# bernardomig/torch_semantic_segmentation

Hardware: AMD Instinct MI355X
Metric: images/sec (train step) fastscnn 1024x2048 bs=8 (higher is better)
Workload: dtype bf16; 1 GPU; fastscnn train step (zero_grad+fwd+CE(ignore 255)+bwd+AdamW), 8 x 3 x 1024 x 2048 per GPU, 19 classes, random-init weights; global_batch=8, parallelism=dp1, hip_graph=True, syncbn=False

## Files before the change

### include/tss_hip.h

```cpp
#ifndef TSS_HIP_H
#define TSS_HIP_H

#ifdef __cplusplus
extern "C" {
#endif

#define TSS_OK 0
#define TSS_ERR_DTYPE (-1)
#define TSS_ERR_SHAPE (-2)
#define TSS_ERR_ALIGN (-3)
#define TSS_ERR_HIP (-4)

#define TSS_F32 0
#define TSS_BF16 1

typedef struct tss_bn_bwd_job {
  const double* bstats; double count; const float* invstd; const float* gamma; int training; int accumulate;
  float* dgamma; float* dbeta; float* ga; float* gb; float* gce; int C;
  int xchg_world; int xchg_rank; void* xchg_peers[8]; void* xchg_counters;
} tss_bn_bwd_job;

enum {
  TSS_K_PWCONV_FWD = 0, TSS_K_PWCONV_BWD_DATA, TSS_K_PWCONV_BWD_WEIGHT,
  TSS_K_CONV3X3_FWD, TSS_K_CONV3X3_BWD_DATA, TSS_K_CONV3X3_BWD_WEIGHT,
  TSS_K_STEM_FWD, TSS_K_STEM_BWD_WEIGHT,
  TSS_K_DWCONV_FWD, TSS_K_DWCONV_BWD_DATA, TSS_K_DWCONV_BWD_WEIGHT,
  TSS_K_BN_FINALIZE, TSS_K_BN_BWD_FINALIZE, TSS_K_JOIN_FWD, TSS_K_JOIN_BWD,
  TSS_K_DROPOUT, TSS_K_BIAS_GRAD, TSS_K_ADAMW,
  TSS_K_BILINEAR_FWD, TSS_K_BILINEAR_BWD, TSS_K_BILINEAR_BWD_COLS, TSS_K_BILINEAR_PLANAR_FWD,
  TSS_K_UPSAMPLE_HEAD_FWD, TSS_K_UPSAMPLE_HEAD_BWD_ROWS, TSS_K_UPSAMPLE_HEAD_BWD_COLS,
  TSS_K_POOL_FWD, TSS_K_POOL_BWD, TSS_K_COPY,
  TSS_K_CE_FWD, TSS_K_CE_BWD, TSS_K_ARGMAX, TSS_K_UPSAMPLE_CE_FWD, TSS_K_UPSAMPLE_CE_BWD,
  TSS_K_RESIZE_FLIP_PLANAR, TSS_K_MULTISCALE_ARGMAX,
  TSS_K_SGD, TSS_K_GRAD_NORM,
  TSS_K_WIDE_CE_FWD, TSS_K_WIDE_CE_BWD, TSS_K_WIDE_ARGMAX, TSS_K_WIDE_MULTISCALE_ARGMAX,
  TSS_K_COUNT
};

int tss_version(void);
int tss_memset_zero(void* p, long bytes, void* stream);
const char* tss_last_error(void);
const char* tss_arch(void);
#define TSS_OPT_DISABLE_FAST_PATHS 1
int tss_set_option(int key, int value);
int tss_get_option(int key);

int tss_prof_enable(int on);
int tss_prof_reset(void);
int tss_prof_collect(void);
int tss_prof_get(int kernel_id, long* launches, double* total_ms, double* alg_bytes, double* flops);
long tss_prof_records(int* kernel_ids, double* ms, double* alg_bytes, long max_records);
const char* tss_prof_name(int kernel_id);
const char* tss_prof_symbol(int kernel_id);

int tss_pwconv_fwd(const void* x, long ldx, const float* in_mean, const float* in_scale, const float* in_bias, int in_relu,
                   const float* w, const void* w_bf16, const float* bias, void* y, long ldy, double* stats,
                   long P, int K, int N, int dtype, void* stream);
int tss_pwconv_fwd_joined(const void* x, long ldx, const float* in_mean, const float* in_scale, const float* in_bias, int in_relu,
                          const float* w, const void* w_bf16, const float* bias,
                          const float* out_mean, const float* out_scale, const float* out_beta,
                          const void* residual, long ldr, int out_relu, void* y, long ldy,
                          long P, int K, int N, int dtype, void* stream);
int tss_bneck_eval_supported(int Cin, int Cmid, int Cout, int stride, int residual, int dtype);
int tss_bneck_eval_fwd(const void* x, long ldx, const float* w1, const void* w1_bf16, const float* mean1, const float* scale1,
                       const float* beta1, const float* wdw, const float* mean2, const float* scale2, const float* beta2,
                       const float* w3, const void* w3_bf16, const float* mean3, const float* scale3, const float* beta3,
                       int residual, void* y, long ldy, int B, int H, int W, int Cin, int Cmid, int Cout, int stride, int dtype,
                       void* stream);
long tss_bn_xchg_bytes(void);
int tss_bn_xchg_counters(void);
int tss_ipc_alloc(long bytes, void** ptr_out, void* handle_out);
int tss_ipc_open(const void* handle, void** ptr_out);
int tss_ipc_close(void* ptr);
int tss_ipc_free(void* ptr);
int tss_bn_xchg_error(const void* mailbox, long* out);
int tss_bn_finalize_xchg(const double* sums, double count, const void* const* peers, int rank, int world, void* counters,
                         const float* gamma, float eps, float momentum, float* running_mean, float* running_var,
                         long long* num_batches_tracked, float* mean_out, float* invstd_out, float* scale, int C, void* stream);
int tss_bn_bwd_finalize_xchg(const double* bstats, double count, const void* const* peers, int rank, int world, void* counters,
                             const float* invstd, const float* gamma, int accumulate, float* dgamma, float* dbeta,
                             float* ga, float* gb, float* gce, int C, void* stream);
int tss_pwconv_bwd_data(const void* e, long lde, const void* yraw, long ldyr,
                        const float* ga, const float* gb, const float* gce, const float* gmu, const float* w, const void* wT_bf16,
                        const void* xraw, long ldx, const float* in_mean, const float* in_scale, const float* in_bias, int in_relu,
                        void* e_in, long ldei, double* bstats, const float* wg_ws, float* wg_dw, long wg_P, int wg_K, int wg_N,
                        long P, int K, int N, int dtype, void* stream);
int tss_pwconv_bwd_weight(const void* e, long lde, const void* yraw, long ldyr,
                          const float* ga, const float* gb, const float* gce, const float* gmu,
                          const void* xraw, long ldx, const float* in_mean, const float* in_scale, const float* in_bias, int in_relu,
                          float* dw, float* ws, int defer_reduce, long P, int K, int N, int dtype, const tss_bn_bwd_job* fin,
                          void* stream);
long tss_pwconv_bwd_weight_ws(long P, int K, int N, int dtype);
int tss_pwconv_fwd_multi(const void* const* srcs, const long* lds, const float* const* means, const float* const* scales,
                         const float* const* biases, int nsrc, int in_relu, const float* w, const void* w_bf16,
                         const float* bias, void* y, long ldy, long P, int N, int dtype, void* stream);
int tss_pwconv_wg_reduce(const float* ws, float* dw, long P, int K, int N, void* stream);

int tss_permute_w3x3(const float* w, float* w_tnc, float* w_tcn, int N, int Cin, void* stream);
int tss_permute_w3x3_bf16(const float* w, void* w_tnc_bf16, void* w_tcn_bf16, int N, int Cin, void* stream);
int tss_conv3x3_fwd(const void* x, long ldx, const float* in_mean, const float* in_scale, const float* in_bias, int in_relu,
                    const float* w_tnc, const void* w_tnc_bf16, void* y, long ldy, double* stats,
                    int B, int Hin, int Win, int Cin, int N, int stride, int dil, int dtype, void* stream);
int tss_conv3x3_bwd_data(const void* e, long lde, const void* yraw, long ldyr,
                         const float* ga, const float* gb, const float* gce, const float* gmu, const float* w_tcn,
                         const void* w_tcn_bf16,
                         const void* xraw, long ldx, const float* in_mean, const float* in_scale, const float* in_bias, int in_relu,
                         void* e_in, long ldei, double* bstats,
                         int B, int H, int W, int Cin, int N, int dil, int dtype, void* stream);
int tss_conv3x3_bwd_weight(const void* e, long lde, const void* yraw, long ldyr,
                           const float* ga, const float* gb, const float* gce, const float* gmu,
                           const void* xraw, long ldx, const float* in_mean, const float* in_scale, const float* in_bias, int in_relu,
                           float* dw, int B, int Hin, int Win, int Cin, int N, int stride, int dil,
                           int dtype, void* stream);
int tss_im2col3x3(const void* x, long ldx, const float* in_mean, const float* in_scale, const float* in_bias, int in_relu,
                  void* col, int B, int H, int W, int C, int dil, int dtype, void* stream);

int tss_permute_wtaps(const float* w , float* w_tnc, float* w_tcn, int N, int Cin, int T, void* stream);
int tss_conv1d3_fwd(const void* x, long ldx, const float* in_mean, const float* in_scale, const float* in_bias, int in_relu,
                    const float* w_tnc, const float* bias, void* y, long ldy, double* stats,
                    int B, int H, int W, int Cin, int N, int axis, int dil, int dtype, void* stream);
int tss_conv1d3_bwd_data(const void* e, long lde, const void* yraw, long ldyr,
                         const float* ga, const float* gb, const float* gce, const float* gmu, const float* w_tcn,
                         const void* xraw, long ldx, const float* in_mean, const float* in_scale, const float* in_bias, int in_relu,
                         void* e_in, long ldei, double* bstats,
                         int B, int H, int W, int Cin, int N, int axis, int dil, int dtype, void* stream);
int tss_conv1d3_bwd_weight(const void* e, long lde, const void* yraw, long ldyr,
                           const float* ga, const float* gb, const float* gce, const float* gmu,
                           const void* xraw, long ldx, const float* in_mean, const float* in_scale, const float* in_bias, int in_relu,
                           float* dw, int B, int H, int W, int Cin, int N, int axis, int dil, int dtype, void* stream);
int tss_conv1d3_lean_supported(int Cin, int N, int dtype);
int tss_conv1d3_fwd_w(const void* x, long ldx, const float* in_mean, const float* in_scale, const float* in_bias, int in_relu,
                      const float* w, const float* bias, void* y, long ldy, double* stats,
                      int B, int H, int W, int Cin, int N, int axis, int dil, int dtype, void* stream);
int tss_conv1d3_bwd_data_w(const void* e, long lde, const void* yraw, long ldyr,
                           const float* ga, const float* gb, const float* gce, const float* gmu, const float* w,
                           const void* xraw, long ldx, const float* in_mean, const float* in_scale, const float* in_bias, int in_relu,
                           void* e_in, long ldei, double* bstats,
                           int B, int H, int W, int Cin, int N, int axis, int dil, int dtype, void* stream);
int tss_conv1d3_bwd_weight_rows(long P, int Cin, int N, int dtype);
int tss_conv1d3_bwd_weight_sweep(const void* e, long lde, const void* yraw, long ldyr,
                                 const float* ga, const float* gb, const float* gce, const float* gmu,
                                 const void* xraw, long ldx, const float* in_mean, const float* in_scale, const float* in_bias,
                                 int in_relu, float* ws, int B, int H, int W, int Cin, int N, int axis, int dil, int dtype, void* stream);
int tss_convtap_bwd_weight_rows(long P, int Cin, int N, int T, int dtype);
int tss_convtap_bwd_weight_sweep(const void* e, long lde, const void* yraw, long ldyr,
                                 const float* ga, const float* gb, const float* gce, const float* gmu,
                                 const void* xraw, long ldx, const float* in_mean, const float* in_scale, const float* in_bias,
                                 int in_relu, float* ws, int B, int H, int W, int Cin, int N, int T, int axis, int dil, int dtype, void* stream);
int tss_sconv_bwd_weight_rows(int B, int Hin, int Win, int Cin, int N, int dtype);
int tss_sconv_bwd_weight_sweep(const void* e, long lde, const void* yraw, long ldyr,
                               const float* ga, const float* gb, const float* gce, const float* gmu,
                               const void* xraw, long ldx, const float* in_mean, const float* in_scale, const float* in_bias,
                               int in_relu, float* ws, int B, int Hin, int Win, int Cin, int N, int dtype, void* stream);
int tss_im2col1d3(const void* x, long ldx, const float* in_mean, const float* in_scale, const float* in_bias, int in_relu,
                  void* col, int B, int H, int W, int C, int axis, int dil, int dtype, void* stream);
int tss_convkxk_fwd(const void* x, long ldx, const float* in_mean, const float* in_scale, const float* in_bias, int in_relu,
                    const float* w_tnc, const float* bias, void* y, long ldy, double* stats,
                    int B, int Hin, int Win, int Cin, int N, int kh, int kw, int stride, int dil, int dtype, void* stream);
int tss_convkxk_bwd_data(const void* e, long lde, const void* yraw, long ldyr,
                         const float* ga, const float* gb, const float* gce, const float* gmu, const float* w_tcn,
                         const void* xraw, long ldx, const float* in_mean, const float* in_scale, const float* in_bias, int in_relu,
                         void* e_in, long ldei, double* bstats,
                         int B, int Hin, int Win, int Cin, int N, int kh, int kw, int stride, int dil, int dtype, void* stream);
int tss_convkxk_bwd_weight(const void* e, long lde, const void* yraw, long ldyr,
                           const float* ga, const float* gb, const float* gce, const float* gmu,
                           const void* xraw, long ldx, const float* in_mean, const float* in_scale, const float* in_bias, int in_relu,
                           float* dw, int B, int Hin, int Win, int Cin, int N, int kh, int kw, int stride, int dil,
                           int dtype, void* stream);

int tss_convkxk_transposed_fwd(const void* x, long ldx, const float* w_tcn, const float* bias, void* y, long ldy,
                               int B, int Hout, int Wout, int Cout, int Cin_t, int kh, int kw, int stride, int dtype, void* stream);

int tss_tensor_stats(const void* z, long ldz, long P, int C, double* stats, int dtype, void* stream);
int tss_bn_bwd_apply(const void* e, long lde, const void* z, long ldz, const float* ga, const float* gb, const float* gce,
                     const float* gmu, void* dz, long lddz, long P, int C, int dtype, void* stream);
int tss_pool_concat_fwd(const void* y1, long ld1, const float* bias, int N1, const void* x, int x_f32, long sxb, long sxc, long sxh,
                        long sxw, int Cin, void* z, long ldz, int B, int Hin, int Win, int dtype, void* stream);
int tss_pool_concat_bwd(const void* dz, long lddz, int N1, const void* x, int x_f32, long sxb, long sxc, long sxh, long sxw, int Cin,
                        void* dx, long lddx, int B, int Hin, int Win, int dtype, void* stream);
int tss_rows_slices(int B, long HW);
int tss_mul_addrows_fwd(const void* u, long ldu, const void* a, long lda, const void* r, long ldr, void* out, long ldo, int B, long HW,
                        int C, int dtype, void* stream);
int tss_mul_addrows_bwd(const void* g, long ldg, const void* u, long ldu, const void* a, long lda, void* du, long lddu, void* da,
                        long ldda, void* dr, long lddr, float* ws, int B, long HW, int C, int dtype, void* stream);
int tss_scale_rows(const void* x, long ldx, const float* m, void* out, long ldo, int B, long HW, int C, int dtype, void* stream);
int tss_cat2_add(const void* gl, long ldl, const void* gr, long ldr, const void* gs, long lds, void* out, long ldo, long P, int half,
                 int dtype, void* stream);
int tss_pad_channels(const void* g, long ldg, int C, void* out, long ldo, int CP, long P, int dtype, void* stream);
int tss_ssnbt_tail_fwd(const void* left, long ldl, const float* mean_l, const float* scale_l, const float* shift_l,
                       const void* right, long ldr, const float* mean_r, const float* scale_r, const float* shift_r,
                       const void* x, long ldx, const float* m, void* out, long ldo, int B, long HW, int C, int dtype, void* stream);
int tss_ssnbt_tail_bwd(const void* dout, long lddo, const void* out, long ldo,
                       const void* left, long ldl, const float* mean_l, const void* right, long ldr, const float* mean_r,
                       const float* m, void* e, long lde, void* gs, long ldgs, double* stats_l, double* stats_r,
                       int B, long HW, int C, int dtype, void* stream);

int tss_channel_shuffle(const void* x, long ldx, void* y, long ldy, long P, int C, int groups, int dtype, void* stream);

int tss_stem3x3_fwd(const void* x_nchw, int x_is_f32, const float* w, void* y, long ldy, double* stats,
                    int B, int Cin, int Hin, int Win, int N, int stride, int dtype, void* stream);
int tss_stem3x3_bwd_weight(const void* e, long lde, const void* yraw, long ldyr,
                           const float* ga, const float* gb, const float* gce, const float* gmu,
                           const void* x_nchw, int x_is_f32, float* dw,
                           float* ws ,
                           int B, int Cin, int Hin, int Win, int N, int stride, int dtype, void* stream);

int tss_dwconv3x3_fwd(const void* x, long ldx, const float* in_mean, const float* in_scale, const float* in_bias, int in_relu,
                      const float* w, void* y, long ldy, double* stats,
                      int B, int Hin, int Win, int C, int stride, int dil, int dtype, void* stream);
int tss_dwconv3x3_bwd_data(const void* e, long lde, const void* yraw, long ldyr,
                           const float* ga, const float* gb, const float* gce, const float* gmu, const float* w,
                           const void* xraw, long ldx, const float* in_mean, const float* in_scale, const float* in_bias, int in_relu,
                           void* e_in, long ldei, double* bstats, const float* wg_ws, float* wg_dw,
                           int B, int Hin, int Win, int C, int stride, int dil, int dtype, void* stream);
int tss_pwconv_bwd_data_radd_supported(long P, int K, int N, int dtype);
int tss_pwconv_bwd_data_joined(const void* e, long lde, const void* yraw, long ldyr,
                               const float* ga, const float* gb, const float* gce, const float* gmu, const float* w, const void* wT_bf16,
                               void* e_in, long ldei, const float* wg_ws, float* wg_dw, long wg_P, int wg_K, int wg_N,
                               const void* radd, long ldr, const void* join_out, long ldjo, const void* join_y, long ldjy,
                               const float* join_mean, double* join_bstats, long P, int K, int N, int dtype, void* stream);
int tss_pwconv_bwd_data_radd(const void* e, long lde, const void* yraw, long ldyr,
                             const float* ga, const float* gb, const float* gce, const float* gmu, const float* w, const void* wT_bf16,
                             void* e_in, long ldei, const float* wg_ws, float* wg_dw, long wg_P, int wg_K, int wg_N,
                             const void* radd, long ldr, long P, int K, int N, int dtype, void* stream);
int tss_pwconv_bwd_fused_preferred(long P, int Cin, int Cout, int dtype);
int tss_pwconv_bwd_fused_rows(long P, int Cin, int Cout);
int tss_pwconv_bwd_fused(const void* e, long lde, const void* yraw, long ldyr, const float* ga, const float* gb, const float* gce,
                         const float* gmu, const float* w, const void* wT_bf16, const void* x, long ldx, const float* in_mean,
                         const float* in_scale, const float* in_bias, int in_relu, int x_pending, void* e_in, long ldei,
                         double* bstats, float* ws, float* bias_ws, long P, int Cin, int Cout, int dtype, void* stream);
int tss_pwconv_bwd_sweep_preferred(long P, int Cin, int Cout, int x_pending, int dtype);
int tss_pwconv_bwd_sweep_rows(long P, int Cin, int Cout);
int tss_pwconv_bwd_sweep(const void* e, long lde, const void* yraw, long ldyr, const float* ga, const float* gb, const float* gce,
                         const float* gmu, const void* wT_bf16, const void* x, long ldx, const float* in_mean,
                         const float* in_scale, const float* in_bias, int in_relu, int x_pending, const void* radd, long ldr,
                         void* e_in, long ldei, double* bstats, float* ws, long P, int Cin, int Cout, int dtype, void* stream);
int tss_dwconv3x3_bwd_fused_supported(int C, int stride, int dil, int dtype);
int tss_dwconv3x3_bwd_fused_sweep(const void* e, long lde, const void* yraw, long ldyr,
                                  const float* ga, const float* gb, const float* gce, const float* gmu, const float* w,
                                  const void* x, long ldx, const float* in_mean, const float* in_scale, const float* in_bias, int in_relu,
                                  int x_pending, void* e_in, long ldei, double* bstats, float* ws,
                                  int B, int Hin, int Win, int C, int stride, int dil, int dtype, void* stream, int* rows_out);
int tss_dw_reduce_many(int njobs, const float* const* ws, float* const* dw, const int* n, const int* rows, void* stream);
int tss_dwconv3x3_bwd_fused_preferred(int C, int stride, int dil, int dtype);
int tss_dwconv3x3_bwd_fused(const void* e, long lde, const void* yraw, long ldyr,
                            const float* ga, const float* gb, const float* gce, const float* gmu, const float* w,
                            const void* x, long ldx, const float* in_mean, const float* in_scale, const float* in_bias, int in_relu,
                            int x_pending, void* e_in, long ldei, double* bstats, float* ws, float* dw,
                            int B, int Hin, int Win, int C, int stride, int dil, int dtype, void* stream);
int tss_dwconv3x3_bwd_weight(const void* e, long lde, const void* yraw, long ldyr,
                             const float* ga, const float* gb, const float* gce, const float* gmu,
                             const void* xraw, long ldx, const float* in_mean, const float* in_scale, const float* in_bias, int in_relu,
                             float* dw, float* ws , int defer_reduce,
                             int B, int Hin, int Win, int C, int stride, int dil, int dtype, void* stream);

int tss_updw_supported(int B, int Hs, int Ws, int Ho, int Wo, int C, int dil, int dtype);
int tss_updw_ws_rows(int B, int Hs, int Ws, int Ho, int Wo, int C, int dil, int dtype);
int tss_updw_fwd(const void* x, long ldx, int Hs, int Ws, const float* w, void* y, long ldy, double* stats,
                 int B, int Ho, int Wo, int C, int dil, int dtype, void* stream);
int tss_updw_bwd(const void* e, long lde, const void* yraw, long ldyr, const float* ga, const float* gb, const float* gce,
                 const float* gmu, const float* w, const void* x, long ldx, int Hs, int Ws, void* e_up, long ldeu, float* ws,
                 int B, int Ho, int Wo, int C, int dil, int dtype, void* stream, int* rows_out);

int tss_stat_slabs(void);

int tss_bn_finalize(const double* sums, double count, const float* gamma, float eps,
                    float momentum, float* running_mean, float* running_var, long long* num_batches_tracked,
                    float* mean_out, float* invstd_out, float* scale, int C, void* stream);
int tss_bn_eval_affine(const float* gamma, const float* running_mean, const float* running_var,
                       float eps, float* mean_out, float* invstd_out, float* scale, int C, void* stream);
int tss_bn_eval_affine_batched(const long long* table, int njobs, int max_channels, void* stream);
int tss_bn_bwd_finalize(const double* bstats, double count, const float* invstd,
                        const float* gamma, int training, int accumulate, float* dgamma, float* dbeta,
                        float* ga, float* gb, float* gce, int C, void* stream);

int tss_slab_reduce(const double* slabs, double count, double* out, int C, void* stream);
int tss_bn_finalize_sync(const double* gsums, const float* gamma, float eps, float momentum, float* running_mean,
                         float* running_var, long long* num_batches_tracked, float* mean_out, float* invstd_out,
                         float* scale, int C, void* stream);
int tss_bn_bwd_finalize_sync(const double* bstats, const double* gsums, const float* invstd, const float* gamma,
                             int accumulate, float* dgamma, float* dbeta, float* ga, float* gb, float* gce, int C,
                             void* stream);

int tss_join_fwd(const void* a, long lda, const float* ma, const float* sa, const float* ba,
                 const void* b, long ldb, const float* mb, const float* sb, const float* bb,
                 void* out, long ldo, int relu, float drop_p, const unsigned long long* seed_slot,
                 long P, int C, int dtype, void* stream);
int tss_join_bwd(const void* dout, long lddo, const void* out, long ldo, int relu,
                 const void* a_raw, long lda, const float* mean_a, double* stats_a,
                 const void* b_raw, long ldb, const float* mean_b, double* stats_b,
                 void* e, long lde, float dout_scale, long P, int C, int dtype, void* stream);

int tss_dropout_tick(unsigned long long* counter, unsigned long long* seed_slot, void* stream);
int tss_dropout(const void* x, long ldx, void* y, long ldy, long P, int C, float p,
                const unsigned long long* seed_slot, int dtype, void* stream);
int tss_bias_grad(const void* e, long lde, long P, int N, float* dbias, int dtype, void* stream);
int tss_dropout_mask(const unsigned long long* counter, void* mask, long P, int C, float p, void* stream);
int tss_pwconv_drop_supported(long P, int K, int N, int dtype);
int tss_pwconv_fwd_drop(const void* x, long ldx, const float* in_mean, const float* in_scale, const float* in_bias, int in_relu,
                        const float* w, const void* w_bf16, const float* bias, void* y, long ldy,
                        const void* mask, float drop_p, unsigned long long* counter,
                        long P, int K, int N, int dtype, void* stream);
int tss_pwconv_bwd_fused_drop_supported(long P, int Cin, int Cout, int dtype);
int tss_pwconv_bwd_fused_drop_rows(long P);
int tss_pwconv_bwd_fused_drop(const void* e, long lde, const void* yraw, long ldyr, const float* ga, const float* gb, const float* gce,
                              const float* gmu, const float* w, const void* x, long ldx, const float* in_mean,
                              const float* in_scale, const float* in_bias, int in_relu, int x_pending, const void* mask, float drop_p,
                              void* e_in, long ldei, double* bstats, float* ws, float* bias_ws, long P, int Cin, int Cout, int dtype,
                              void* stream);
int tss_cast_weights(const long long* table, int njobs, int blocks_per_job, float* zero, long zero_n, void* stream);
int tss_adamw_step(float* params, const float* grads, float* exp_avg, float* exp_avg_sq, long n,
                   const float* lr, float beta1, float beta2, float eps, float weight_decay,
                   float* state, float grad_scale, float lr_host, long step_host, void* stream);

#define TSS_OPT_MAX_GROUPS 8
#define TSS_OPT_NESTEROV 1
typedef struct tss_optgroup { long begin; long end; float lr; float weight_decay; float beta1; float beta2; float eps; int flags; } tss_optgroup;
int tss_adamw_step_groups(float* params, const float* grads, float* exp_avg, float* exp_avg_sq, long n,
                          const tss_optgroup* groups, int ngroups, const float* lr, float* state, const float* scale,
                          float grad_scale, long step_host, void* stream);
int tss_sgd_step_groups(float* params, const float* grads, float* momentum_buf, long n, const tss_optgroup* groups, int ngroups,
                        const float* lr, float* state, const float* scale, float grad_scale, long step_host, void* stream);
long tss_grad_sqnorm_workspace_bytes(long n);
int tss_grad_sqnorm(const float* grads, long n, double* workspace, float grad_scale, float max_norm, float* out, void* stream);

int tss_bilinear_nhwc_fwd(const void* x, long ldx, void* y, long ldy, int B, int Hin, int Win, int Hout, int Wout,
                          int C, int dtype, void* stream);
int tss_bilinear_nhwc_bwd(const void* dy, long lddy, void* dx, long lddx, float* tmp ,
                          int B, int Hin, int Win, int Hout, int Wout, int C, int dtype, void* stream);
int tss_bilinear_planar_fwd(const void* x, int x_dtype, void* y, int y_dtype, long planes, int Hin, int Win,
                            int Hout, int Wout, void* stream);
int tss_upsample_head_fwd(const void* low, long ldl, void* y, int B, int N, int h, int w, int H, int W,
                          int dtype, void* stream);
int tss_upsample_head_bwd(const void* dy, const float* gscale, float* tmp, void* dlow, long ldl,
                          int B, int N, int h, int w, int H, int W, int dtype, void* stream);
int tss_adaptive_pool_fwd(const void* x, long ldx, void* y, long ldy, int B, int H, int W, int C, int bins,
                          int dtype, void* stream);
int tss_adaptive_pool_bwd(const void* dy, long lddy, void* dx, long lddx, int B, int H, int W, int C, int bins,
                          int dtype, void* stream);
int tss_ppm_pool_slices(int B, int ncells);
int tss_ppm_pool_fwd(const void* x, long ldx, void* const* y, const long* ldy, const int* bins, int narms,
                     float* ws ,
                     int B, int H, int W, int C, int dtype, void* stream);
int tss_ppm_pool_bwd(const void* const* dy, const long* lddy, const int* bins, int narms, void* dx, long lddx,
                     const void* radd, long ldr, int B, int H, int W, int C, int dtype, void* stream);
int tss_ppm_concat_fwd(const void* x, long ldx, const void* const* raw, const long* ldr, const int* bins,
                       const float* const* mean, const float* const* scale, const float* const* beta, const int* relu,
                       int narms, void* out, long ldo, int B, int H, int W, int C, int ca, int dtype, void* stream);
int tss_ppm_concat_bwd(const void* dout, long lddo, const void* const* raw, const long* ldr, const int* bins,
                       const float* const* mean, const float* const* scale, const float* const* beta, const int* relu,
                       double* const* bstats, void* const* e, const long* lde, int narms,
                       int B, int H, int W, int C, int ca, int dtype, void* stream);
int tss_ppm_arms_supported(int narms, int C, int Ca, const int* P, int dtype);
int tss_ppm_arms_fwd(const void* const* x, const long* ldx, const float* const* w, const float* const* gamma, float* const* running_mean,
                     float* const* running_var, long long* const* num_batches_tracked, void* const* y, const long* ldy, float* const* vec,
                     const int* P, int narms, int C, int Ca, int training, float eps, float momentum, int dtype, void* stream);
int tss_ppm_arms_bwd(const void* const* e, const long* lde, const void* const* y, const long* ldy, const void* const* x, const long* ldx,
                     const float* const* w, const float* const* gamma, float* const* vec, float* const* dw, float* const* dgamma,
                     float* const* dbeta, int accumulate, void* const* e_in, const long* ldei, const int* P, int narms, int C, int Ca,
                     int training, int dtype, void* stream);
int tss_copy_nhwc(const void* x, long ldx, void* y, long ldy, long P, int C, int dtype, void* stream);

int tss_gate_slices(int B, long HW);
int tss_gate_fwd(const void* x, long ldx, const void* a, long lda, void* out, long ldo, int B, long HW, int C, float add_one,
                 int dtype, void* stream);
int tss_gate_bwd(const void* g, long ldg, const void* x, long ldx, const void* a, long lda, void* dx, long lddx, void* da, long ldda,
                 float* ws, int B, long HW, int C, float add_one, int dtype, void* stream);

int tss_cross_entropy_fwd(const void* logits, const long long* target, float* lse, double* acc,
                          float* loss, float* inv_count, long B, int C, long HW, int ignore_index,
                          int dtype, void* stream);
int tss_cross_entropy_bwd(const void* logits, const long long* target, const float* lse, const float* inv_count,
                          const float* grad_out, void* dlogits, long B, int C, long HW, int ignore_index,
                          int dtype, void* stream);
long tss_cross_entropy_ex_rows(long B, long HW);
int tss_cross_entropy_fwd_ex(const void* logits, const long long* target, const float* weight, float label_smoothing,
                             float* lse, double* rows, float* loss, float* inv_count, long B, int C, long HW, int ignore_index,
                             int dtype, void* stream);
int tss_cross_entropy_bwd_ex(const void* logits, const long long* target, const float* weight, float label_smoothing,
                             const float* lse, const float* inv_count, const float* grad_out, void* dlogits, long B, int C, long HW,
                             int ignore_index, int dtype, void* stream);
long tss_ohem_workspace_bytes(void);
int tss_ohem_select(const float* pixel_loss, void* workspace, float* loss, float* params, long n, float thresh_loss, long n_top,
                    void* stream);
int tss_ohem_fwd(const void* logits, const long long* target, float* lse, float* pixel_loss, void* workspace,
                 float* loss, float* params, long B, int C, long HW, int ignore_index, float thresh_loss,
                 long n_top, int dtype, void* stream);
int tss_ohem_bwd(const void* logits, const long long* target, const float* lse, const float* pixel_loss,
                 const float* params, const float* grad_out, void* dlogits, long B, int C, long HW, int ignore_index,
                 int dtype, void* stream);
long tss_lovasz_workspace_bytes(long n_pixels, int C, int chunk_classes);
int tss_lovasz_fwd(const void* logits, const long long* target, void* workspace, float* loss, float* n_present,
                   long B, int C, long HW, int ignore_index, int has_ignore, int variant, int chunk_classes, int dtype,
                   void* stream);
int tss_lovasz_bwd(const void* logits, const long long* target, const void* workspace, const float* n_present,
                   const float* grad_out, void* dlogits, long B, int C, long HW, int chunk_classes, int dtype, void* stream);
long tss_focal_workspace_bytes(long B, long HW, int max_blocks);
int tss_focal_fwd(const void* logits, const long long* target, float* lse, float* pixel_coef, void* workspace, float* loss,
                  float* scale, long B, int C, long HW, int ignore_index, int has_ignore, float alpha, float gamma, int variant,
                  int max_blocks, int dtype, void* stream);
int tss_focal_bwd(const void* logits, const long long* target, const float* lse, const float* pixel_coef, const float* scale,
                  const float* grad_out, void* dlogits, long B, int C, long HW, int max_blocks, int dtype, void* stream);
long tss_dice_workspace_bytes(long B, int C, long HW, int max_blocks);
int tss_dice_fwd(const void* logits, const long long* target, float* lse, void* workspace, float* loss, long B, int C, long HW,
                 int ignore_index, int has_ignore, float smooth, int max_blocks, int dtype, void* stream);
int tss_dice_bwd(const void* logits, const long long* target, const float* lse, const void* workspace, const float* grad_out,
                 void* dlogits, long B, int C, long HW, int ignore_index, int has_ignore, int max_blocks, int dtype, void* stream);
// ... 91 lines not shown
```

### torch_semantic_segmentation_amd/_native.py

```python
import ctypes
import os

import torch

_HERE = os.path.dirname(os.path.abspath(__file__))
LIB_PATH = os.environ.get('TSS_HIP_LIB') or os.path.join(_HERE, 'libtss_hip.so')

TSS_F32, TSS_BF16 = 0, 1
ERRORS = {-1: 'TSS_ERR_DTYPE (unsupported dtype)', -2: 'TSS_ERR_SHAPE (unsupported shape or pitch)',
          -3: 'TSS_ERR_ALIGN (pointer not 16-byte aligned)', -4: 'TSS_ERR_HIP (HIP launch error)'}

_P, _L, _I, _F, _D = ctypes.c_void_p, ctypes.c_long, ctypes.c_int, ctypes.c_float, ctypes.c_double

HEADER_PATH = os.path.join(os.path.dirname(_HERE), 'include', 'tss_hip.h')


def parse_header(path=HEADER_PATH):
    import re
    text = open(path).read()
    text = re.sub(r'/\*.*?\*/', ' ', text, flags=re.S)
    scalars = {'int': _I, 'long': _L, 'float': _F, 'double': _D}
    decls = {}
    for m in re.finditer(r'\b(int|long|const\s+char\s*\*)\s*(tss_\w+)\s*\(([^)]*)\)\s*;', text):
        ret, name, params = m.group(1), m.group(2), m.group(3).strip()
        types = []
        if params and params != 'void':
            for prm in params.split(','):
                prm = prm.strip()
                if '*' in prm:
                    types.append(_P)
                else:
                    words = prm.split()[:-1]
                    types.append(scalars[' '.join(w for w in words if w != 'const')])
        decls[name] = (scalars.get(ret, ctypes.c_char_p), types)
    return decls


_lib = None


def lib():
    global _lib
    if _lib is None:
        if not os.path.exists(LIB_PATH):
            raise RuntimeError(
                'libtss_hip.so is not built (%s). Run `python -m torch_semantic_segmentation_amd.build`; '
                'this package has no non-HIP fallback.' % LIB_PATH)
        handle = ctypes.CDLL(LIB_PATH)
        for name, (restype, argtypes) in parse_header().items():
            fn = getattr(handle, name)
            fn.argtypes = argtypes
            fn.restype = restype
        _lib = handle
    return _lib


def call(name, *args):
    rc = getattr(lib(), name)(*args)
    if rc != 0:
        detail = lib().tss_last_error().decode() if rc == -4 else ''
        raise RuntimeError('%s failed: %s %s' % (name, ERRORS.get(rc, rc), detail))


def fast_paths_disabled():
    return lib().tss_get_option(1) == 1


def ptr(t):
    return None if t is None else t.data_ptr()


def stream():
    return torch.cuda.current_stream().cuda_stream


_slabs = None


def stat_slabs():
    global _slabs
    if _slabs is None:
        _slabs = lib().tss_stat_slabs()
    return _slabs


def dtype_code(dtype):
    if dtype == torch.float32:
        return TSS_F32
    if dtype == torch.bfloat16:
        return TSS_BF16
    raise TypeError('the HIP path computes in float32 or bfloat16 activations, got %s' % dtype)



K_COUNT = 41


def prof_enable(on=True):
    call('tss_prof_enable', 1 if on else 0)


def prof_reset():
    call('tss_prof_reset')


def prof_records(limit=100000):
    h = lib()
    ids = (ctypes.c_int * limit)()
    ms = (ctypes.c_double * limit)()
    by = (ctypes.c_double * limit)()
    n = min(h.tss_prof_records(ids, ms, by, limit), limit)
    return [(h.tss_prof_name(ids[i]).decode(), ms[i], by[i]) for i in range(n)]


def prof_table():
    call('tss_prof_collect')
    out = {}
    h = lib()
    for k in range(K_COUNT):
        n, ms, by, fl = ctypes.c_long(), ctypes.c_double(), ctypes.c_double(), ctypes.c_double()
        h.tss_prof_get(k, ctypes.byref(n), ctypes.byref(ms), ctypes.byref(by), ctypes.byref(fl))
        if n.value:
            out[h.tss_prof_name(k).decode()] = dict(symbol=h.tss_prof_symbol(k).decode(), launches=n.value,
                                                    ms=ms.value, bytes=by.value, flops=fl.value)
    return out
```

### torch_semantic_segmentation_amd/build.py

```python
import os
import subprocess
import sys
from concurrent.futures import ThreadPoolExecutor

HERE = os.path.dirname(os.path.abspath(__file__))
CSRC = os.path.join(HERE, 'csrc')
INCLUDE = os.path.join(os.path.dirname(HERE), 'include')
LIB = os.path.join(HERE, 'libtss_hip.so')
SOURCES = ['convgemm.hip', 'pwfast.hip', 'pwbwd.hip', 'pwsweep.hip', 'bneck.hip', 'conv3x3.hip', 'fc1d.hip', 'fcg.hip', 'sconv.hip', 'atrous.hip', 'wstat.hip', 'stem.hip', 'wgrad.hip', 'dwconv.hip', 'dwroll.hip', 'updw.hip', 'pointwise.hip', 'optim.hip', 'xchg.hip', 'resample.hip', 'ppm.hip', 'loss.hip', 'ohem.hip', 'lovasz.hip', 'softloss.hip', 'distill.hip', 'labelhist.hip', 'hostio.hip', 'augment.hip', 'msflip.hip', 'widehead.hip', 'softhead.hip', 'gate.hip', 'zoo.hip', 'ssnbt.hip', 'prof.cpp']
HIPCC = os.environ.get('HIPCC', '/opt/rocm/bin/hipcc')
FLAGS = ['--offload-arch=gfx950', '-O3', '-fPIC', '-std=c++17', '-Wall', '-Wno-unused-function',
         '-I' + INCLUDE, '-I' + CSRC]


def _deps_mtime():
    files = [os.path.join(CSRC, f) for f in os.listdir(CSRC) if f.endswith('.h')]
    files.append(os.path.join(INCLUDE, 'tss_hip.h'))
    return max(os.path.getmtime(f) for f in files)


def _compile(src, force):
    path = os.path.join(CSRC, src)
    timing = os.environ.get('TSS_TIMING') == '1'
    obj = os.path.join(CSRC, os.path.splitext(src)[0] + ('.timing.o' if timing else '.o'))
    if (not force and os.path.exists(obj)
            and os.path.getmtime(obj) >= max(os.path.getmtime(path), _deps_mtime())):
        return obj, False
    extra = ['-DTSS_TIMING'] if timing else []
    cmd = [HIPCC] + FLAGS + extra + (['-x', 'hip'] if src.endswith('.cpp') else []) + ['-c', path, '-o', obj]
    res = subprocess.run(cmd, capture_output=True, text=True)
    if res.returncode != 0:
        raise RuntimeError('hipcc failed for %s:\n%s\n%s' % (src, res.stdout, res.stderr))
    if res.stderr.strip():
        sys.stderr.write(res.stderr)
    return obj, True


def build(force=False, verbose=True):
    with ThreadPoolExecutor(max_workers=4) as pool:
        results = list(pool.map(lambda s: _compile(s, force), SOURCES))
    objs = [o for o, _ in results]
    variant = 'timing' if os.environ.get('TSS_TIMING') == '1' else 'release'
    stamp = os.path.join(CSRC, '.variant')
    same = os.path.exists(stamp) and open(stamp).read().strip() == variant
    if any(changed for _, changed in results) or not os.path.exists(LIB) or not same:
        cmd = [HIPCC, '--offload-arch=gfx950', '-shared', '-fPIC', '-o', LIB] + objs
        res = subprocess.run(cmd, capture_output=True, text=True)
        if res.returncode != 0:
            raise RuntimeError('link failed:\n%s\n%s' % (res.stdout, res.stderr))
        open(stamp, 'w').write(variant)
        if verbose:
            print('built', LIB, '(%s)' % variant)
    elif verbose:
        print('up to date', LIB)
    return LIB


if __name__ == '__main__':
    build(force='--force' in sys.argv)
```

### torch_semantic_segmentation_amd/csrc/dwroll.hip

```cpp
#include "dwroll.h"

#include <cstdlib>

#include "common.h"

namespace {

constexpr int NT = 256;
constexpr int ENT = NT + 16;

struct RollArgs {
  const bf16_t* x; long ldx; const float* xm; const float* xs; const float* xb; int x_relu;
  const float* w; bf16_t* y; long ldy; double* stats;
  int B, Hin, Win, C, CV, Hout, Wout;
  int CVS, PXL, nsl, nstrips, RS, nseg, rows_used;
  int dseg, dstrip, db;
  long units;
};

struct Cursor { int it, b, strip, seg, x0, o0; };

__device__ __forceinline__ void advance(Cursor& c, const RollArgs& g, int n_iter) {
  if (++c.it == n_iter) {
    c.it = 0;
    c.seg += g.dseg;
    int carry = c.seg >= g.nseg ? 1 : 0;
    c.seg -= carry * g.nseg;
    c.strip += g.dstrip + carry;
    carry = c.strip >= g.nstrips ? 1 : 0;
    c.strip -= carry * g.nstrips;
    c.b += g.db + carry;
    c.x0 = c.strip * g.PXL;
    c.o0 = c.seg * g.RS;
  }
}

__device__ __forceinline__ int clampi(int v, int lo, int hi) { return v < lo ? lo : (v > hi ? hi : v); }

typedef unsigned int u32x4 __attribute__((ext_vector_type(4)));
__device__ __forceinline__ void request(u32x4& dst, const bf16_t* uniform_base, int elem_offset) {
  asm volatile("global_load_dwordx4 %0, %1, %2" : "=v"(dst) : "v"(elem_offset * 2), "s"(uniform_base));
}
template <int N> __device__ __forceinline__ void arrived(u32x4& a, u32x4& b) {
  asm volatile("s_waitcnt vmcnt(%2)" : "+v"(a), "+v"(b) : "n"(N));
}
template <int N> __device__ __forceinline__ void arrived(u32x4& a, u32x4& b, u32x4& c, u32x4& d, u32x4& e, u32x4& f) {
  asm volatile("s_waitcnt vmcnt(%6)" : "+v"(a), "+v"(b), "+v"(c), "+v"(d), "+v"(e), "+v"(f) : "n"(N));
}

__device__ __forceinline__ void park(float4* lo4, float4* hi4, int e, const u32x4& raw, bool valid, const float sc[8],
                                     const float sh[8], float relu_lo) {
  float v[8];
  V8<bf16_t>::unpack(make_uint4(raw[0], raw[1], raw[2], raw[3]), v);
  const float lo = valid ? relu_lo : 0.f, hi = valid ? TSS_INF : 0.f;
#pragma unroll
  for (int j = 0; j < 8; ++j) v[j] = clamp3(v[j] * sc[j] + sh[j], lo, hi);
  lo4[e] = make_float4(v[0], v[1], v[2], v[3]);
  hi4[e] = make_float4(v[4], v[5], v[6], v[7]);
}
__device__ __forceinline__ void fetch(const float4* lo4, const float4* hi4, int e, float v[8]) {
  const float4 a = lo4[e], b = hi4[e];
  v[0] = a.x; v[1] = a.y; v[2] = a.z; v[3] = a.w; v[4] = b.x; v[5] = b.y; v[6] = b.z; v[7] = b.w;
}

template <int NC>
__device__ __forceinline__ void flush_slab(const float (&s1)[NC], const float (&s2)[NC], double* stats, int C, int CVS, int PXL,
                                           int sl, int brow, int rows_used, int p, int cg, bool lane_on, float* red) {
  const int tid = threadIdx.x;
  const int cw = CVS * NC;
  __syncthreads();
  if (p < PXL) {
#pragma unroll
    for (int j = 0; j < NC; ++j) {
      red[(p * 2 + 0) * cw + cg * NC + j] = lane_on ? s1[j] : 0.f;
      red[(p * 2 + 1) * cw + cg * NC + j] = lane_on ? s2[j] : 0.f;
    }
  }
  __syncthreads();
  const int ncol = 2 * cw, share = NT / ncol;
  float part = 0.f;
  const int col = tid % ncol, sub = tid / ncol;
  if (sub < share) {
#pragma unroll 8
    for (int q = sub; q < PXL; q += share) part += red[(q * 2 + col / cw) * cw + col % cw];
  }
  float* part_s = red + NT * 16;
  if (sub < share) part_s[sub * ncol + col] = part;
  __syncthreads();
  if (tid < ncol) {
    const int which = tid / cw, c = tid - which * cw;
    const int ch = sl * 64 + c;
    if (ch < C) {
      double a = 0.0;
      for (int q = 0; q < share; ++q) a += (double)part_s[q * ncol + tid];
      stats[(long)brow * 2 * C + which * C + ch] = a;
      for (int r = brow + rows_used; r < TSS_STAT_SLABS; r += rows_used) stats[(long)r * 2 * C + which * C + ch] = 0.0;
    }
  }
}

template <int S> struct RollCfg;
#ifndef TSS_ROLL_PF1
#define TSS_ROLL_PF1 6
#endif
#ifndef TSS_ROLL_PF2
#define TSS_ROLL_PF2 2
#endif
#ifndef TSS_ROLL_BPF1
#define TSS_ROLL_BPF1 4
#endif
#ifndef TSS_ROLL_BPF2
#define TSS_ROLL_BPF2 2
#endif
template <> struct RollCfg<1> { static constexpr int PF = TSS_ROLL_PF1, NRAW = 2, ROWS = 1, ARRS = 1; };
template <> struct RollCfg<2> { static constexpr int PF = TSS_ROLL_PF2, NRAW = 6, ROWS = 2, ARRS = 2; };

template <int S>
__global__ __launch_bounds__(NT, 2) void dw_fwd_roll_kernel(const RollArgs g) {
  typedef RollCfg<S> K;
  constexpr int PF = K::PF;
  extern __shared__ __align__(16) unsigned char dyn_smem[];
  typedef float4 (*Ring)[K::ROWS][K::ARRS][2][ENT];
  Ring ring = reinterpret_cast<Ring>(dyn_smem);
  const int tid = threadIdx.x;
  const int p = tid / g.CVS, cg = tid - p * g.CVS;
  const int sl = (int)blockIdx.x % g.nsl, brow = (int)blockIdx.x / g.nsl;
  const int cv = sl * 8 + cg;
  const bool lane_on = p < g.PXL && cv < g.CV;
  const int c0 = lane_on ? cv * 8 : 0;
  const bool halo_l = lane_on && p == 0, halo_r = lane_on && p == g.PXL - 1;
  const int ldx = (int)g.ldx;

  const int n_iter = (S == 1) ? g.RS + 2 : g.RS + 1;
  Cursor ci, cc;
  ci.it = 0;
  ci.seg = brow % g.nseg;
  ci.strip = (brow / g.nseg) % g.nstrips;
  ci.b = brow / (g.nseg * g.nstrips);
  ci.x0 = ci.strip * g.PXL;
  ci.o0 = ci.seg * g.RS;
  cc = ci;

  u32x4 raw[PF][K::NRAW];
  const int halo_dx = halo_l ? -1 : (halo_r ? g.PXL : p);
  auto issue = [&](const Cursor& c, u32x4 (&r)[K::NRAW]) {
    const int b = c.b < g.B ? c.b : g.B - 1;
    if (S == 1) {
      const int iy = clampi(c.o0 - 1 + c.it, 0, g.Hin - 1);
      const bf16_t* row = g.x + ((long)b * g.Hin + iy) * g.Win * g.ldx;
      request(r[0], row, clampi(c.x0 + p, 0, g.Win - 1) * ldx + c0);
      request(r[1], row, clampi(c.x0 + halo_dx, 0, g.Win - 1) * ldx + c0);
    } else {
#pragma unroll
      for (int ry = 0; ry < 2; ++ry) {
        const int iy = clampi(2 * (c.o0 + c.it) - 1 + ry, 0, g.Hin - 1);
        const bf16_t* row = g.x + ((long)b * g.Hin + iy) * g.Win * g.ldx;
        const int ix = 2 * (c.x0 + p);
        request(r[3 * ry + 0], row, clampi(ix, 0, g.Win - 1) * ldx + c0);
        request(r[3 * ry + 1], row, clampi(ix + 1, 0, g.Win - 1) * ldx + c0);
        request(r[3 * ry + 2], row, clampi(halo_l ? 2 * c.x0 - 1 : ix, 0, g.Win - 1) * ldx + c0);
      }
    }
  };
#pragma unroll
  for (int k = 0; k < PF; ++k) {
    issue(ci, raw[k]);
    advance(ci, g, n_iter);
  }

  float sc[8], sh[8];
  {
    float mu[8];
    const bool has = g.xs != nullptr, has_b = has && g.xb != nullptr, has_m = has && g.xm != nullptr;
    const float* safe = g.w;
#pragma unroll
    for (int h = 0; h < 2; ++h) {
      float a[4], b[4], m[4];
      V4<float>::load(has ? g.xs + c0 + 4 * h : safe, a);
      V4<float>::load(has_b ? g.xb + c0 + 4 * h : safe, b);
      V4<float>::load(has_m ? g.xm + c0 + 4 * h : safe, m);
#pragma unroll
      for (int j = 0; j < 4; ++j) {
        sc[4 * h + j] = has ? a[j] : 1.f;
        sh[4 * h + j] = has_b ? b[j] : 0.f;
        mu[4 * h + j] = has_m ? m[j] : 0.f;
      }
    }
#pragma unroll
    for (int j = 0; j < 8; ++j) sh[j] = __builtin_fmaf(-mu[j], sc[j], sh[j]);
  }
  float wr[9][8];
  {
    float wf[72];
#pragma unroll
    for (int q = 0; q < 18; ++q) V4<float>::load(g.w + (long)c0 * 9 + 4 * q, wf + 4 * q);
#pragma unroll
    for (int j = 0; j < 8; ++j)
#pragma unroll
      for (int t = 0; t < 9; ++t) wr[t][j] = wf[j * 9 + t];
  }
  const float relu_lo = g.x_relu ? 0.f : -TSS_INF;
  float s1[8], s2[8];
#pragma unroll
  for (int j = 0; j < 8; ++j) { s1[j] = 0.f; s2[j] = 0.f; }

  auto write = [&](const Cursor& c, const u32x4 (&r)[K::NRAW], int slot) {
    if (S == 1) {
      const int iy = c.o0 - 1 + c.it;
      const bool vy = iy >= 0 && iy < g.Hin;
      float4* lo4 = ring[slot][0][0][0];
      float4* hi4 = ring[slot][0][0][1];
      if (p < g.PXL) park(lo4, hi4, tid + g.CVS, r[0], vy && c.x0 + p < g.Win, sc, sh, relu_lo);
      if (halo_l) park(lo4, hi4, tid, r[1], vy && c.x0 - 1 >= 0, sc, sh, relu_lo);
      if (halo_r) park(lo4, hi4, tid + 2 * g.CVS, r[1], vy && c.x0 + g.PXL < g.Win, sc, sh, relu_lo);
    } else {
#pragma unroll
      for (int ry = 0; ry < 2; ++ry) {
        const int iy = 2 * (c.o0 + c.it) - 1 + ry;
        const bool vy = iy >= 0 && iy < g.Hin;
        const int ix = 2 * (c.x0 + p);
        if (p < g.PXL) {
          park(ring[slot][ry][1][0], ring[slot][ry][1][1], tid, r[3 * ry + 0], vy && ix < g.Win, sc, sh, relu_lo);
          park(ring[slot][ry][0][0], ring[slot][ry][0][1], tid + g.CVS, r[3 * ry + 1], vy && ix + 1 < g.Win, sc, sh, relu_lo);
        }
        if (halo_l) park(ring[slot][ry][0][0], ring[slot][ry][0][1], tid, r[3 * ry + 2], vy && 2 * c.x0 - 1 >= 0, sc, sh, relu_lo);
      }
    }
  };

  float accA[8], accB[8];
#pragma unroll
  for (int j = 0; j < 8; ++j) { accA[j] = 0.f; accB[j] = 0.f; }

  auto emit = [&](const Cursor& c, int orow, float (&acc)[8]) {
    if (lane_on && orow < g.Hout && c.x0 + p < g.Wout) {
#pragma unroll
      for (int j = 0; j < 8; ++j) {
        acc[j] = V8<bf16_t>::round(acc[j]);
        s1[j] += acc[j];
        s2[j] += acc[j] * acc[j];
      }
      V8<bf16_t>::store(g.y + ((long)c.b * g.Hout + orow) * g.Wout * g.ldy + ((c.x0 + p) * (int)g.ldy + c0), acc);
    }
  };
  auto compute = [&](const Cursor& c, int slot) {
    if (!lane_on) return;
    if (S == 1) {
      float accC[8];
      if (c.it == 0) {
#pragma unroll
        for (int j = 0; j < 8; ++j) { accA[j] = 0.f; accB[j] = 0.f; }
      }
#pragma unroll
      for (int kx = 0; kx < 3; ++kx) {
        float a[8];
        fetch(ring[slot][0][0][0], ring[slot][0][0][1], tid + kx * g.CVS, a);
#pragma unroll
        for (int j = 0; j < 8; ++j) {
          accA[j] += a[j] * wr[6 + kx][j];
          accB[j] += a[j] * wr[3 + kx][j];
          accC[j] = kx == 0 ? a[j] * wr[0][j] : accC[j] + a[j] * wr[kx][j];
        }
      }
      if (c.it >= 2) emit(c, c.o0 + c.it - 2, accA);
#pragma unroll
      for (int j = 0; j < 8; ++j) { accA[j] = accB[j]; accB[j] = accC[j]; }
    } else {
      if (c.it == 0) {
#pragma unroll
        for (int j = 0; j < 8; ++j) accA[j] = 0.f;
      }
#pragma unroll
      for (int kx = 0; kx < 3; ++kx) {
        float a[8];
        fetch(ring[slot][0][kx & 1][0], ring[slot][0][kx & 1][1], tid + (kx >> 1) * g.CVS, a);
#pragma unroll
        for (int j = 0; j < 8; ++j) {
          accA[j] += a[j] * wr[6 + kx][j];
          accB[j] = kx == 0 ? a[j] * wr[0][j] : accB[j] + a[j] * wr[kx][j];
        }
      }
      if (c.it >= 1) emit(c, c.o0 + c.it - 1, accA);
#pragma unroll
      for (int kx = 0; kx < 3; ++kx) {
        float a[8];
        fetch(ring[slot][1][kx & 1][0], ring[slot][1][kx & 1][1], tid + (kx >> 1) * g.CVS, a);
#pragma unroll
        for (int j = 0; j < 8; ++j) accB[j] += a[j] * wr[3 + kx][j];
      }
#pragma unroll
      for (int j = 0; j < 8; ++j) accA[j] = accB[j];
    }
  };

  int slot = 0;
  while (cc.b < g.B) {
#pragma unroll
    for (int k = 0; k < PF; ++k) {
      if (cc.b >= g.B) break;
      if (S == 1) arrived<K::NRAW * (PF - 1)>(raw[k][0], raw[k][1]);
      else arrived<K::NRAW * (PF - 1)>(raw[k][0], raw[k][1], raw[k][2], raw[k][3 % K::NRAW], raw[k][4 % K::NRAW], raw[k][5 % K::NRAW]);
      write(cc, raw[k], slot);
      asm volatile("" ::: "memory");
      issue(ci, raw[k]);
      advance(ci, g, n_iter);
      __syncthreads();
      compute(cc, slot);
      advance(cc, g, n_iter);
      slot ^= 1;
    }
  }
#pragma unroll
  for (int k = 0; k < PF; ++k) {
    if (S == 1) arrived<0>(raw[k][0], raw[k][1]);
    else arrived<0>(raw[k][0], raw[k][1], raw[k][2], raw[k][3 % K::NRAW], raw[k][4 % K::NRAW], raw[k][5 % K::NRAW]);
  }

  if (g.stats) flush_slab<8>(s1, s2, g.stats, g.C, g.CVS, g.PXL, sl, brow, g.rows_used, p, cg, lane_on, reinterpret_cast<float*>(dyn_smem));
}

void plan(RollArgs& g, int S) {
  g.CV = g.C / 8;
  g.nsl = (g.CV + 7) / 8;
  g.CVS = g.CV < 8 ? g.CV : 8;
  g.PXL = NT / g.CVS;
  g.nstrips = (g.Wout + g.PXL - 1) / g.PXL;
  const int cap = TSS_STAT_SLABS / g.nsl > 0 ? TSS_STAT_SLABS / g.nsl : 1;
  const int halo = S == 1 ? 2 : 1;
  long best_cost = -1;
  for (int nseg = 1; nseg <= g.Hout; ++nseg) {
    const int RS = (g.Hout + nseg - 1) / nseg;
    if (RS < 4 && nseg > 1) break;
    const int segs = (g.Hout + RS - 1) / RS;
    const long units = (long)g.B * g.nstrips * segs;
    const long k = (units + cap - 1) / cap;
    const long cost = k * (RS + halo) + 6;
    if (best_cost < 0 || cost < best_cost) {
      best_cost = cost;
      g.RS = RS; g.nseg = segs; g.units = units;
      g.rows_used = (int)((units + k - 1) / k);
    }
  }
  g.dseg = g.rows_used % g.nseg;
  g.dstrip = (g.rows_used / g.nseg) % g.nstrips;
  g.db = g.rows_used / (g.nseg * g.nstrips);
}


typedef unsigned int u32x2 __attribute__((ext_vector_type(2)));
__device__ __forceinline__ void request2(u32x2& dst, const bf16_t* uniform_base, int elem_offset) {
  asm volatile("global_load_dwordx2 %0, %1, %2" : "=v"(dst) : "v"(elem_offset * 2), "s"(uniform_base));
}
template <int N> __device__ __forceinline__ void arrived2(u32x2& a, u32x2& b, u32x2& c, u32x2& d, u32x2& e, u32x2& f) {
  asm volatile("s_waitcnt vmcnt(%6)" : "+v"(a), "+v"(b), "+v"(c), "+v"(d), "+v"(e), "+v"(f) : "n"(N));
}
__device__ __forceinline__ void settle(float (&a)[4]) { asm volatile("" : "+v"(a[0]), "+v"(a[1]), "+v"(a[2]), "+v"(a[3])); }
__device__ __forceinline__ void settle(float4& a) { asm volatile("" : "+v"(a.x), "+v"(a.y), "+v"(a.z), "+v"(a.w)); }
__device__ __forceinline__ u32x2 keep2(const u32x2& r) {
  u32x2 o;
  asm volatile("v_mov_b32 %0, %2\n\tv_mov_b32 %1, %3" : "=&v"(o[0]), "=&v"(o[1]) : "v"(r[0]), "v"(r[1]));
  return o;
}
__device__ __forceinline__ void unpack4(const u32x2& r, float v[4]) {
  v[0] = __uint_as_float(r[0] << 16); v[1] = __uint_as_float(r[0] & 0xffff0000u);
  v[2] = __uint_as_float(r[1] << 16); v[3] = __uint_as_float(r[1] & 0xffff0000u);
}
__device__ __forceinline__ float4 ld4(const float* p) { return *reinterpret_cast<const float4*>(p); }

struct RollBwdArgs {
  const bf16_t* e; long lde; const bf16_t* yr; long ldyr; const float* ga; const float* gb; const float* gce; const float* gmu;
  const float* w;
  const bf16_t* x; long ldx; const float* xm; const float* xs; const float* xb; int x_relu, x_mask;
  bf16_t* ein; long ldei; double* stats; float* ws;
  int B, H, W, C;
  int CVS, PXL, nsl, nstrips, RS, nseg, rows_used, dseg, dstrip, db;
};
#ifdef TSS_ROLL_TIMING
__device__ unsigned long long g_roll_timing[8];
#define TSS_RT(var) unsigned long long var; asm volatile("s_memtime %0\n s_waitcnt lgkmcnt(0)" : "=s"(var) :: "memory")
#else
#define TSS_RT(var)
#endif
constexpr int BENT = NT + 32;
constexpr int BPF = TSS_ROLL_BPF1;

struct BCursor { int it, b, strip, seg, x0, o0; };
__device__ __forceinline__ void advance(BCursor& c, const RollBwdArgs& g, int n_iter) {
  if (++c.it == n_iter) {
    c.it = 0;
    c.seg += g.dseg;
    int carry = c.seg >= g.nseg ? 1 : 0;
    c.seg -= carry * g.nseg;
    c.strip += g.dstrip + carry;
    carry = c.strip >= g.nstrips ? 1 : 0;
    c.strip -= carry * g.nstrips;
    c.b += g.db + carry;
    c.x0 = c.strip * g.PXL;
    c.o0 = c.seg * g.RS;
  }
}

template <int RPJ>
__global__ __launch_bounds__(NT, 2) void dw_bwd_roll_s1_kernel(const RollBwdArgs g) {
  constexpr int PFB = RPJ == 1 ? BPF : 2;
  TSS_RT(rt_begin);
#ifdef TSS_ROLL_TIMING
  unsigned long long rt_ph[4] = {0, 0, 0, 0}, rt_ph4 = 0;
#endif
  __shared__ __align__(16) float4 rows_s[4 * RPJ][BENT];
  auto Gs = [&](int slot_, int jr) -> float4* { return rows_s[slot_ * RPJ + jr]; };
  auto As = [&](int slot_, int jr) -> float4* { return rows_s[2 * RPJ + slot_ * RPJ + jr]; };
  static_assert(sizeof(float4) * 4 * BENT >= sizeof(float) * (NT * 16 + NT), "flush_slab scratch");
  const int tid = threadIdx.x;
  const int p = tid / g.CVS, cg = tid - p * g.CVS;
  const int sl = (int)blockIdx.x % g.nsl, brow = (int)blockIdx.x / g.nsl;
  const int ch = sl * 64 + cg * 4;
  const bool lane_on = p < g.PXL && ch < g.C;
  const int c0 = lane_on ? ch : 0;
  const bool halo_l = lane_on && p == 0, halo_r = lane_on && p == g.PXL - 1;
  const int halo_dx = halo_l ? -1 : (halo_r ? g.PXL : p);
  const int lde = (int)g.lde, ldy = (int)g.ldyr, ldx = (int)g.ldx;
  const bf16_t* ysrc = g.yr ? g.yr : g.e;

  const int n_iter = (g.RS + 2 + RPJ - 1) / RPJ;
  BCursor ci, cc;
  ci.it = 0;
  ci.seg = brow % g.nseg;
  ci.strip = (brow / g.nseg) % g.nstrips;
  ci.b = brow / (g.nseg * g.nstrips);
  ci.x0 = ci.strip * g.PXL;
  ci.o0 = ci.seg * g.RS;
  cc = ci;

  u32x2 raw[PFB][6 * RPJ];
  auto issue = [&](const BCursor& c, u32x2 (&r)[6 * RPJ]) {
    const int b = c.b < g.B ? c.b : g.B - 1;
#pragma unroll
   for (int jr = 0; jr < RPJ; ++jr) {
    const int iy = clampi(c.o0 - 1 + c.it * RPJ + jr, 0, g.H - 1);
    const long rowpix = ((long)b * g.H + iy) * g.W;
    const int xm_ = clampi(c.x0 + p, 0, g.W - 1), xh_ = clampi(c.x0 + halo_dx, 0, g.W - 1);
    const bf16_t* re = g.e + rowpix * g.lde;
    const bf16_t* ry = ysrc + rowpix * (g.yr ? g.ldyr : g.lde);
    const bf16_t* rx = g.x + rowpix * g.ldx;
    const int ldyy = g.yr ? ldy : lde;
    request2(r[6 * jr + 0], re, xm_ * lde + c0);
    request2(r[6 * jr + 1], ry, xm_ * ldyy + c0);
    request2(r[6 * jr + 2], rx, xm_ * ldx + c0);
    request2(r[6 * jr + 3], re, xh_ * lde + c0);
    request2(r[6 * jr + 4], ry, xh_ * ldyy + c0);
    request2(r[6 * jr + 5], rx, xh_ * ldx + c0);
   }
  };
#pragma unroll
  for (int k = 0; k < PFB; ++k) {
    issue(ci, raw[k]);
    advance(ci, g, n_iter);
  }

  float ca[4], cb[4], kd[4], sc[4], sh[4], mu[4];
  {
    const float* safe = g.w;
    float t0[4], t1[4], t2[4], t3[4];
    V4<float>::load(g.ga ? g.ga + c0 : safe, t0);
    V4<float>::load(g.yr ? g.gb + c0 : safe, t1);
    V4<float>::load(g.yr ? g.gce + c0 : safe, t2);
    V4<float>::load(g.yr ? g.gmu + c0 : safe, t3);
#pragma unroll
    for (int j = 0; j < 4; ++j) {
      ca[j] = g.ga ? t0[j] : 1.f;
      cb[j] = g.yr ? t1[j] : 0.f;
      kd[j] = g.yr ? -(ca[j] * t2[j]) - cb[j] * t3[j] : 0.f;
    }
    const bool has = g.xs != nullptr;
    V4<float>::load(has ? g.xs + c0 : safe, t0);
    V4<float>::load(has && g.xb ? g.xb + c0 : safe, t1);
    V4<float>::load(g.xm ? g.xm + c0 : safe, t2);
#pragma unroll
    for (int j = 0; j < 4; ++j) {
      sc[j] = has ? t0[j] : 1.f;
      mu[j] = g.xm ? t2[j] : 0.f;
      sh[j] = __builtin_fmaf(-(has ? mu[j] : 0.f), sc[j], (has && g.xb) ? t1[j] : 0.f);
    }
  }
  float wr[9][4];
  {
    float wf[36];
#pragma unroll
    for (int q = 0; q < 9; ++q) V4<float>::load(g.w + (long)c0 * 9 + 4 * q, wf + 4 * q);
#pragma unroll
    for (int j = 0; j < 4; ++j)
#pragma unroll
      for (int t = 0; t < 9; ++t) wr[t][j] = wf[j * 9 + t];
  }
  const float relu_lo = g.x_relu ? 0.f : -TSS_INF;
  float dwa[9][4], accA[4], accB[4], gprev[4], aprev[3][4], s1[4], s2[4];
#pragma unroll
  for (int j = 0; j < 4; ++j) {
    accA[j] = accB[j] = gprev[j] = s1[j] = s2[j] = 0.f;
#pragma unroll
    for (int t = 0; t < 9; ++t) dwa[t][j] = 0.f;
#pragma unroll
    for (int t = 0; t < 3; ++t) aprev[t][j] = 0.f;
  }
  u32x2 xprev = {0u, 0u};

  auto ga_of = [&](const u32x2& re, const u32x2& ry, const u32x2& rx, bool valid, float4& gv, float4& av) {
    float ev[4], yv[4], xv[4], go[4], ao[4];
    unpack4(re, ev); unpack4(ry, yv); unpack4(rx, xv);
    const float lo = valid ? relu_lo : 0.f, hi = valid ? TSS_INF : 0.f;
#pragma unroll
    for (int j = 0; j < 4; ++j) {
      const float gj = ca[j] * ev[j] + (cb[j] * yv[j] + kd[j]);
      go[j] = valid ? gj : 0.f;
      ao[j] = clamp3(xv[j] * sc[j] + sh[j], lo, hi);
    }
    gv = make_float4(go[0], go[1], go[2], go[3]);
    av = make_float4(ao[0], ao[1], ao[2], ao[3]);
  };

  TSS_RT(rt_loop);
  int slot = 0;
  while (cc.b < g.B) {
#pragma unroll
    for (int k = 0; k < PFB; ++k) {
      if (cc.b >= g.B) break;
      TSS_RT(rt0);
#pragma unroll
      for (int jr = 0; jr < RPJ; ++jr)
        arrived2<6 * RPJ * (PFB - 1)>(raw[k][6 * jr], raw[k][6 * jr + 1], raw[k][6 * jr + 2], raw[k][6 * jr + 3], raw[k][6 * jr + 4], raw[k][6 * jr + 5]);
      TSS_RT(rt1);
      float4 gown[RPJ], aown[RPJ];
      u32x2 xcur[RPJ];
#pragma unroll
      for (int jr = 0; jr < RPJ; ++jr) {
        const int r = cc.o0 - 1 + cc.it * RPJ + jr;
        const bool vy = r >= 0 && r < g.H;
        ga_of(raw[k][6 * jr], raw[k][6 * jr + 1], raw[k][6 * jr + 2], vy && cc.x0 + p < g.W, gown[jr], aown[jr]);
        if (p < g.PXL) { Gs(slot, jr)[tid + g.CVS] = gown[jr]; As(slot, jr)[tid + g.CVS] = aown[jr]; }
        if (halo_l || halo_r) {
          float4 gh, ah;
          ga_of(raw[k][6 * jr + 3], raw[k][6 * jr + 4], raw[k][6 * jr + 5], vy && (halo_l ? cc.x0 - 1 >= 0 : cc.x0 + g.PXL < g.W), gh, ah);
          const int eh = halo_l ? tid : tid + 2 * g.CVS;
          Gs(slot, jr)[eh] = gh; As(slot, jr)[eh] = ah;
        }
        xcur[jr] = keep2(raw[k][6 * jr + 2]);
        settle(gown[jr]); settle(aown[jr]);
      }
      asm volatile("" ::: "memory");
      TSS_RT(rt1a);
      issue(ci, raw[k]);
      advance(ci, g, n_iter);
      TSS_RT(rt2);
      __syncthreads();
      TSS_RT(rt3);
      if (lane_on) {
#pragma unroll
       for (int jr = 0; jr < RPJ; ++jr) {
        const int idx = cc.it * RPJ + jr;
        float G[3][4], A[3][4];
#pragma unroll
        for (int q = 0; q < 3; ++q) {
          const float4 gq = Gs(slot, jr)[tid + q * g.CVS], aq = As(slot, jr)[tid + q * g.CVS];
          G[q][0] = gq.x; G[q][1] = gq.y; G[q][2] = gq.z; G[q][3] = gq.w;
          A[q][0] = aq.x; A[q][1] = aq.y; A[q][2] = aq.z; A[q][3] = aq.w;
        }
        if (idx == 0) {
#pragma unroll
          for (int j = 0; j < 4; ++j) { accA[j] = 0.f; accB[j] = 0.f; }
        }
        float accC[4];
#pragma unroll
        for (int j = 0; j < 4; ++j) {
          accA[j] += wr[0][j] * G[2][j]; accA[j] += wr[1][j] * G[1][j]; accA[j] += wr[2][j] * G[0][j];
          accB[j] += wr[3][j] * G[2][j]; accB[j] += wr[4][j] * G[1][j]; accB[j] += wr[5][j] * G[0][j];
          accC[j] = wr[6][j] * G[2][j]; accC[j] += wr[7][j] * G[1][j]; accC[j] += wr[8][j] * G[0][j];
        }
        const int q = cc.o0 + idx - 2;
        const bool prev_owned = idx >= 2 && idx <= g.RS + 1;
        if (prev_owned && q < g.H && cc.x0 + p < g.W) {
          float out[4];
          if (g.x_mask) {
            float xv[4];
            unpack4(jr == 0 ? xprev : xcur[jr > 0 ? jr - 1 : 0], xv);
#pragma unroll
            for (int j = 0; j < 4; ++j) {
              const bool dead = g.x_relu && !(xv[j] * sc[j] + sh[j] > 0.f);
              out[j] = V8<bf16_t>::round(dead ? 0.f : accA[j]);
              s1[j] += out[j];
              s2[j] += out[j] * (xv[j] - mu[j]);
            }
          } else {
#pragma unroll
            for (int j = 0; j < 4; ++j) out[j] = accA[j];
          }
          V4<bf16_t>::store(g.ein + ((long)cc.b * g.H + q) * g.W * g.ldei + ((cc.x0 + p) * (int)g.ldei + c0), out);
        }
        const bool own_cur = idx >= 1 && idx <= g.RS;
#pragma unroll
        for (int j = 0; j < 4; ++j) {
          const float gc = own_cur ? G[1][j] : 0.f, gp = gprev[j];
#pragma unroll
          for (int kx = 0; kx < 3; ++kx) {
            dwa[6 + kx][j] += gp * A[kx][j];
            dwa[3 + kx][j] += gc * A[kx][j];
            dwa[0 + kx][j] += gc * aprev[kx][j];
          }
          gprev[j] = gc;
#pragma unroll
          for (int kx = 0; kx < 3; ++kx) aprev[kx][j] = A[kx][j];
          accA[j] = accB[j]; accB[j] = accC[j];
        }
       }
        xprev = xcur[RPJ - 1];
      }
#ifdef TSS_ROLL_TIMING
      asm volatile("s_waitcnt vmcnt(%0)" :: "n"(6 * RPJ * PFB));
      TSS_RT(rt4);
      rt_ph[0] += rt1 - rt0; rt_ph[1] += rt2 - rt1a; rt_ph[2] += rt3 - rt2; rt_ph[3] += rt4 - rt3; rt_ph4 += rt1a - rt1;
#endif
      advance(cc, g, n_iter);
      slot ^= 1;
    }
  }
  TSS_RT(rt_tail);
#pragma unroll
  for (int k = 0; k < PFB; ++k)
#pragma unroll
    for (int jr = 0; jr < RPJ; ++jr)
      arrived2<0>(raw[k][6 * jr], raw[k][6 * jr + 1], raw[k][6 * jr + 2], raw[k][6 * jr + 3], raw[k][6 * jr + 4], raw[k][6 * jr + 5]);

  float* red = reinterpret_cast<float*>(&rows_s[0][0]);
  if (g.stats) flush_slab<4>(s1, s2, g.stats, g.C, g.CVS, g.PXL, sl, brow, g.rows_used, p, cg, lane_on, red);
  float* wrow = g.ws + (long)brow * g.C * 9;
  const int cw = g.CVS * 4;
#pragma unroll
  for (int t0 = 0; t0 < 9; t0 += 3) {
    __syncthreads();
#pragma unroll
    for (int tt = 0; tt < 3; ++tt)
      *reinterpret_cast<float4*>(red + tid * 12 + tt * 4) =
          lane_on ? make_float4(dwa[t0 + tt][0], dwa[t0 + tt][1], dwa[t0 + tt][2], dwa[t0 + tt][3]) : make_float4(0.f, 0.f, 0.f, 0.f);
    __syncthreads();
    for (int i = tid; i < cw * 3; i += NT) {
      const int c = i / 3, tt = i - c * 3;
      const int cgc = c >> 2, j = c & 3;
      if (sl * 64 + c < g.C) {
        float sum = 0.f;
        for (int q = 0; q < g.PXL; ++q) sum += red[(q * g.CVS + cgc) * 12 + tt * 4 + j];
        wrow[(long)(sl * 64 + c) * 9 + t0 + tt] = sum;
      }
    }
  }
#ifdef TSS_ROLL_TIMING
  asm volatile("s_waitcnt vmcnt(0)" ::: "memory");
  TSS_RT(rt_end);
  if (threadIdx.x == 0) {
    for (int q = 0; q < 4; ++q) atomicAdd(&g_roll_timing[q], rt_ph[q]);
    atomicAdd(&g_roll_timing[4], rt_loop - rt_begin);
    atomicAdd(&g_roll_timing[5], rt_end - rt_tail);
    atomicAdd(&g_roll_timing[6], rt_ph4);
    atomicAdd(&g_roll_timing[7], 1ull);
  }
#endif
}

constexpr int B2PF = TSS_ROLL_BPF2;

struct B2Cursor { int it, b, strip, seg, x0, o0; };
__device__ __forceinline__ void advance(B2Cursor& c, const RollBwdArgs& g, int n_iter) {
  if (++c.it == n_iter) {
    c.it = 0;
    c.seg += g.dseg;
    int carry = c.seg >= g.nseg ? 1 : 0;
    c.seg -= carry * g.nseg;
    c.strip += g.dstrip + carry;
    carry = c.strip >= g.nstrips ? 1 : 0;
    c.strip -= carry * g.nstrips;
    c.b += g.db + carry;
    c.x0 = c.strip * g.PXL;
    c.o0 = c.seg * g.RS;
  }
}
template <int N>
__device__ __forceinline__ void arrived10(u32x2 (&r)[10]) {
  asm volatile("s_waitcnt vmcnt(%10)"
               : "+v"(r[0]), "+v"(r[1]), "+v"(r[2]), "+v"(r[3]), "+v"(r[4]), "+v"(r[5]), "+v"(r[6]), "+v"(r[7]), "+v"(r[8]), "+v"(r[9])
               : "n"(N));
}

__global__ __launch_bounds__(NT, 2) void dw_bwd_roll_s2_kernel(const RollBwdArgs g, const int Ho, const int Wo) {
  __shared__ __align__(16) float4 rows_s[6][BENT];
  static_assert(sizeof(float4) * 6 * BENT >= sizeof(float) * (NT * 16 + NT), "flush_slab scratch");
  const int tid = threadIdx.x;
  const int p = tid / g.CVS, cg = tid - p * g.CVS;
  const int sl = (int)blockIdx.x % g.nsl, brow = (int)blockIdx.x / g.nsl;
  const int ch = sl * 64 + cg * 4;
  const bool lane_on = p < g.PXL && ch < g.C;
  const int c0 = lane_on ? ch : 0;
  const bool halo_l = lane_on && p == 0, halo_r = lane_on && p == g.PXL - 1;
  const int lde = (int)g.lde, ldx = (int)g.ldx;
  const bf16_t* ysrc = g.yr ? g.yr : g.e;
  const int ldyy = g.yr ? (int)g.ldyr : lde;
  const long ldyl = g.yr ? g.ldyr : g.lde;

  const int n_iter = g.RS + 1;
  B2Cursor ci, cc;
  ci.it = 0;
  ci.seg = brow % g.nseg;
  ci.strip = (brow / g.nseg) % g.nstrips;
  ci.b = brow / (g.nseg * g.nstrips);
  ci.x0 = ci.strip * g.PXL;
  ci.o0 = ci.seg * g.RS;
  cc = ci;

  u32x2 raw[B2PF][10];
  auto issue = [&](const B2Cursor& c, u32x2 (&r)[10]) {
    const int b = c.b < g.B ? c.b : g.B - 1;
    const int o = c.o0 + c.it;
    const long orow = ((long)b * Ho + clampi(o, 0, Ho - 1)) * Wo;
    const bf16_t* re = g.e + orow * g.lde;
    const bf16_t* ry = ysrc + orow * ldyl;
    const int po = clampi(c.x0 + p, 0, Wo - 1), pr = clampi(c.x0 + (halo_r ? p + 1 : p), 0, Wo - 1);
    request2(r[0], re, po * lde + c0);
    request2(r[1], ry, po * ldyy + c0);
    request2(r[2], re, pr * lde + c0);
    request2(r[3], ry, pr * ldyy + c0);
    const int ix = 2 * (c.x0 + p);
    const int x0c = clampi(ix, 0, g.W - 1), x1c = clampi(ix + 1, 0, g.W - 1), xlc = clampi(halo_l ? ix - 1 : ix, 0, g.W - 1);
#pragma unroll
    for (int ry2 = 0; ry2 < 2; ++ry2) {
      const int iy = clampi(2 * o - 1 + ry2, 0, g.H - 1);
      const bf16_t* rx = g.x + ((long)b * g.H + iy) * g.W * g.ldx;
      request2(r[4 + 3 * ry2], rx, x0c * ldx + c0);
      request2(r[5 + 3 * ry2], rx, x1c * ldx + c0);
      request2(r[6 + 3 * ry2], rx, xlc * ldx + c0);
    }
  };
#pragma unroll
  for (int k = 0; k < B2PF; ++k) {
    issue(ci, raw[k]);
    advance(ci, g, n_iter);
  }

  float ca[4], cb[4], kd[4], sc[4], sh[4], mu[4];
  {
    const float* safe = g.w;
    float t0[4], t1[4], t2[4], t3[4];
    V4<float>::load(g.ga ? g.ga + c0 : safe, t0);
    V4<float>::load(g.yr ? g.gb + c0 : safe, t1);
    V4<float>::load(g.yr ? g.gce + c0 : safe, t2);
    V4<float>::load(g.yr ? g.gmu + c0 : safe, t3);
#pragma unroll
    for (int j = 0; j < 4; ++j) {
      ca[j] = g.ga ? t0[j] : 1.f;
      cb[j] = g.yr ? t1[j] : 0.f;
      kd[j] = g.yr ? -(ca[j] * t2[j]) - cb[j] * t3[j] : 0.f;
    }
    const bool has = g.xs != nullptr;
    V4<float>::load(has ? g.xs + c0 : safe, t0);
    V4<float>::load(has && g.xb ? g.xb + c0 : safe, t1);
    V4<float>::load(g.xm ? g.xm + c0 : safe, t2);
#pragma unroll
    for (int j = 0; j < 4; ++j) {
      sc[j] = has ? t0[j] : 1.f;
      mu[j] = g.xm ? t2[j] : 0.f;
      sh[j] = __builtin_fmaf(-(has ? mu[j] : 0.f), sc[j], (has && g.xb) ? t1[j] : 0.f);
    }
  }
  float wr[9][4];
  {
    float wf[36];
#pragma unroll
    for (int q = 0; q < 9; ++q) V4<float>::load(g.w + (long)c0 * 9 + 4 * q, wf + 4 * q);
#pragma unroll
    for (int j = 0; j < 4; ++j)
#pragma unroll
      for (int t = 0; t < 9; ++t) wr[t][j] = wf[j * 9 + t];
  }
  const float relu_lo = g.x_relu ? 0.f : -TSS_INF;
  float dwa[9][4], gprev[4], gprev_r[4], s1[4], s2[4];
#pragma unroll
  for (int j = 0; j < 4; ++j) {
    gprev[j] = gprev_r[j] = s1[j] = s2[j] = 0.f;
#pragma unroll
    for (int t = 0; t < 9; ++t) dwa[t][j] = 0.f;
  }

  auto g_of = [&](const u32x2& re, const u32x2& ry, bool valid, float (&go)[4]) {
    float ev[4], yv[4];
    unpack4(re, ev); unpack4(ry, yv);
#pragma unroll
    for (int j = 0; j < 4; ++j) go[j] = valid ? ca[j] * ev[j] + (cb[j] * yv[j] + kd[j]) : 0.f;
  };
  auto a_of = [&](const u32x2& rx, bool valid, float (&ao)[4]) {
    float xv[4];
    unpack4(rx, xv);
    const float lo = valid ? relu_lo : 0.f, hi = valid ? TSS_INF : 0.f;
#pragma unroll
    for (int j = 0; j < 4; ++j) ao[j] = clamp3(xv[j] * sc[j] + sh[j], lo, hi);
  };
  auto put4 = [&](float4* row, int e, const float (&v)[4]) { row[e] = make_float4(v[0], v[1], v[2], v[3]); };
  auto get4 = [&](const float4* row, int e, float (&v)[4]) { const float4 t = row[e]; v[0] = t.x; v[1] = t.y; v[2] = t.z; v[3] = t.w; };
  auto emit = [&](const B2Cursor& c, int q, int px, const u32x2& xraw, float (&acc)[4]) {
    if (q >= 0 && q < g.H && px < g.W) {
      float out[4];
      if (g.x_mask) {
        float xv[4];
        unpack4(xraw, xv);
#pragma unroll
        for (int j = 0; j < 4; ++j) {
          const bool dead = g.x_relu && !(xv[j] * sc[j] + sh[j] > 0.f);
          out[j] = V8<bf16_t>::round(dead ? 0.f : acc[j]);
          s1[j] += out[j];
          s2[j] += out[j] * (xv[j] - mu[j]);
        }
      } else {
#pragma unroll
        for (int j = 0; j < 4; ++j) out[j] = acc[j];
      }
      V4<bf16_t>::store(g.ein + ((long)c.b * g.H + q) * g.W * g.ldei + (px * (int)g.ldei + c0), out);
    }
  };

  int slot = 0;
  while (cc.b < g.B) {
#pragma unroll
    for (int k = 0; k < B2PF; ++k) {
      if (cc.b >= g.B) break;
      arrived10<10 * (B2PF - 1)>(raw[k]);
      const int o = cc.o0 + cc.it;
      const bool vo = o < Ho;
      const int r0 = 2 * o - 1, r1 = 2 * o;
      const bool v0 = r0 >= 0 && r0 < g.H, v1 = r1 < g.H;
      const int ix = 2 * (cc.x0 + p);
      float gown[4], a00[4], a01[4], a10[4], a11[4];
      g_of(raw[k][0], raw[k][1], vo && cc.x0 + p < Wo, gown);
      a_of(raw[k][4], v0 && ix < g.W, a00);
      a_of(raw[k][5], v0 && ix + 1 < g.W, a01);
      a_of(raw[k][7], v1 && ix < g.W, a10);
      a_of(raw[k][8], v1 && ix + 1 < g.W, a11);
      float4* Gs = rows_s[slot];
      float4* A0 = rows_s[2 + 2 * slot];
      float4* A1 = rows_s[3 + 2 * slot];
      if (p < g.PXL) { put4(Gs, tid, gown); put4(A0, tid + g.CVS, a01); put4(A1, tid + g.CVS, a11); }
      if (halo_r) {
        float gh[4];
        g_of(raw[k][2], raw[k][3], vo && cc.x0 + g.PXL < Wo, gh);
        put4(Gs, tid + g.CVS, gh);
      }
      if (halo_l) {
        float ah[4];
        a_of(raw[k][6], v0 && ix - 1 >= 0, ah);
        put4(A0, tid, ah);
        a_of(raw[k][9], v1 && ix - 1 >= 0, ah);
        put4(A1, tid, ah);
      }
      const u32x2 x00 = keep2(raw[k][4]), x01 = keep2(raw[k][5]), x10 = keep2(raw[k][7]), x11 = keep2(raw[k][8]);
      settle(gown); settle(a00); settle(a01); settle(a10); settle(a11);
      asm volatile("" ::: "memory");
      issue(ci, raw[k]);
      advance(ci, g, n_iter);
      __syncthreads();
      if (lane_on) {
        float gr[4], al0[4], al1[4];
        get4(Gs, tid + g.CVS, gr);
        get4(A0, tid, al0);
        get4(A1, tid, al1);
        const bool first = cc.it == 0, last = cc.it == g.RS;
        float e0[4], e1[4];
        if (!first) {
#pragma unroll
          for (int j = 0; j < 4; ++j) {
            e0[j] = wr[7][j] * gprev[j]; e0[j] += wr[1][j] * gown[j];
            e1[j] = wr[8][j] * gprev[j]; e1[j] += wr[6][j] * gprev_r[j]; e1[j] += wr[2][j] * gown[j]; e1[j] += wr[0][j] * gr[j];
          }
          emit(cc, r0, ix, x00, e0);
          emit(cc, r0, ix + 1, x01, e1);
        }
        if (!last) {
#pragma unroll
          for (int j = 0; j < 4; ++j) {
            e0[j] = wr[4][j] * gown[j];
            e1[j] = wr[5][j] * gown[j]; e1[j] += wr[3][j] * gr[j];
          }
          emit(cc, r1, ix, x10, e0);
          emit(cc, r1, ix + 1, x11, e1);
        }
#pragma unroll
        for (int j = 0; j < 4; ++j) {
          const float gc = last ? 0.f : gown[j], gp = first ? 0.f : gprev[j];
          dwa[0][j] += gc * al0[j]; dwa[1][j] += gc * a00[j]; dwa[2][j] += gc * a01[j];
          dwa[3][j] += gc * al1[j]; dwa[4][j] += gc * a10[j]; dwa[5][j] += gc * a11[j];
          dwa[6][j] += gp * al0[j]; dwa[7][j] += gp * a00[j]; dwa[8][j] += gp * a01[j];
          gprev[j] = gown[j]; gprev_r[j] = gr[j];
        }
      }
      advance(cc, g, n_iter);
      slot ^= 1;
    }
  }
#pragma unroll
  for (int k = 0; k < B2PF; ++k) arrived10<0>(raw[k]);

  float* red = reinterpret_cast<float*>(&rows_s[0][0]);
  if (g.stats) flush_slab<4>(s1, s2, g.stats, g.C, g.CVS, g.PXL, sl, brow, g.rows_used, p, cg, lane_on, red);
  float* wrow = g.ws + (long)brow * g.C * 9;
  const int cw = g.CVS * 4;
#pragma unroll
  for (int t0 = 0; t0 < 9; t0 += 3) {
    __syncthreads();
#pragma unroll
    for (int tt = 0; tt < 3; ++tt)
      *reinterpret_cast<float4*>(red + tid * 12 + tt * 4) =
          lane_on ? make_float4(dwa[t0 + tt][0], dwa[t0 + tt][1], dwa[t0 + tt][2], dwa[t0 + tt][3]) : make_float4(0.f, 0.f, 0.f, 0.f);
    __syncthreads();
    for (int i = tid; i < cw * 3; i += NT) {
      const int c = i / 3, tt = i - c * 3;
      const int cgc = c >> 2, j = c & 3;
      if (sl * 64 + c < g.C) {
        float sum = 0.f;
        for (int q = 0; q < g.PXL; ++q) sum += red[(q * g.CVS + cgc) * 12 + tt * 4 + j];
        wrow[(long)(sl * 64 + c) * 9 + t0 + tt] = sum;
      }
    }
  }
}

void plan_bwd(RollBwdArgs& g, int S, int Ho, int Wo, int rpj = 1) {
  const int cv4 = g.C / 4;
  g.nsl = (g.C + 63) / 64;
  g.CVS = cv4 < 16 ? cv4 : 16;
  g.PXL = NT / g.CVS;
  g.nstrips = (Wo + g.PXL - 1) / g.PXL;
  const int cap = TSS_STAT_SLABS / g.nsl > 0 ? TSS_STAT_SLABS / g.nsl : 1;
  const int halo = S == 1 ? 2 : 1;
  long best_cost = -1;
  for (int nseg = 1; nseg <= Ho; ++nseg) {
    const int RS = (Ho + nseg - 1) / nseg;
    if (RS < 4 && nseg > 1) break;
    const int segs = (Ho + RS - 1) / RS;
    const long units = (long)g.B * g.nstrips * segs;
    const long k = (units + cap - 1) / cap;
    const long cost = k * ((RS + halo + rpj - 1) / rpj) * rpj + 6;
    if (best_cost < 0 || cost < best_cost) {
      best_cost = cost;
      g.RS = RS; g.nseg = segs;
      g.rows_used = (int)((units + k - 1) / k);
    }
  }
  g.dseg = g.rows_used % g.nseg;
  g.dstrip = (g.rows_used / g.nseg) % g.nstrips;
  g.db = g.rows_used / (g.nseg * g.nstrips);
}

inline size_t ring_bytes(int S) { return (size_t)2 * S * S * 2 * ENT * sizeof(float4); }

}

namespace tss {

bool dwroll_supported(int C, int stride, int dil, int dtype) {
  const char* sw = getenv("TSS_DW_ROLL");
  const bool on = !(sw && atoi(sw) == 0);
  return on && dtype == TSS_BF16 && dil == 1 && (stride == 1 || stride == 2) && C >= 8 && (C % 8) == 0 && C <= 768;
}

void dwroll_fwd(const void* x, long ldx, const float* in_mean, const float* in_scale, const float* in_bias, int in_relu,
                const float* w, void* y, long ldy, double* stats,
                int B, int Hin, int Win, int C, int stride, hipStream_t stream) {
  RollArgs g = {};
  g.x = (const bf16_t*)x; g.ldx = ldx; g.xm = in_mean; g.xs = in_scale; g.xb = in_bias; g.x_relu = in_relu;
  g.w = w; g.y = (bf16_t*)y; g.ldy = ldy; g.stats = stats;
  g.B = B; g.Hin = Hin; g.Win = Win; g.C = C;
  g.Hout = (Hin - 1) / stride + 1; g.Wout = (Win - 1) / stride + 1;
  plan(g, stride);
  const int grid = g.nsl * g.rows_used;
  static tss::DevOnce once;
  if (once.first())
    (void)hipFuncSetAttribute(reinterpret_cast<const void*>(dw_fwd_roll_kernel<2>), hipFuncAttributeMaxDynamicSharedMemorySize, (int)ring_bytes(2));
  if (stride == 1) hipLaunchKernelGGL(dw_fwd_roll_kernel<1>, dim3(grid), dim3(NT), ring_bytes(1), stream, g);
  else hipLaunchKernelGGL(dw_fwd_roll_kernel<2>, dim3(grid), dim3(NT), ring_bytes(2), stream, g);
}


bool dwroll_bwd_fused_supported(int C, int stride, int dil, int dtype) {
  const char* sw = getenv("TSS_DW_ROLL_BWD");
  const bool on = !(sw && atoi(sw) == 0);
  return on && dtype == TSS_BF16 && dil == 1 && (stride == 1 || stride == 2) && C >= 8 && (C % 8) == 0 && C <= 768;
}

int dwroll_bwd_fused(const void* e, long lde, const void* yraw, long ldyr, const float* ga, const float* gb, const float* gce,
                     const float* gmu, const float* w, const void* x, long ldx, const float* in_mean, const float* in_scale,
                     const float* in_bias, int in_relu, int x_pending, void* e_in, long ldei, double* bstats, float* ws,
                     int B, int H, int W, int C, int stride, hipStream_t stream) {
  RollBwdArgs g = {};
  g.e = (const bf16_t*)e; g.lde = lde; g.yr = (const bf16_t*)yraw; g.ldyr = ldyr; g.ga = ga; g.gb = gb; g.gce = gce; g.gmu = gmu;
  g.w = w; g.x = (const bf16_t*)x; g.ldx = ldx; g.xm = in_mean; g.xs = in_scale; g.xb = in_bias; g.x_relu = in_relu;
  g.x_mask = x_pending; g.ein = (bf16_t*)e_in; g.ldei = ldei; g.stats = bstats; g.ws = ws;
  g.B = B; g.H = H; g.W = W; g.C = C;
  const int Ho = (H - 1) / stride + 1, Wo = (W - 1) / stride + 1;
  const char* sw = getenv("TSS_ROLL_RPJ");
  const int rpj = (stride == 1 && !(sw && atoi(sw) == 1)) ? 2 : 1;
  plan_bwd(g, stride, Ho, Wo, rpj);
  if (stride == 1 && rpj == 2) hipLaunchKernelGGL(dw_bwd_roll_s1_kernel<2>, dim3(g.nsl * g.rows_used), dim3(NT), 0, stream, g);
  else if (stride == 1) hipLaunchKernelGGL(dw_bwd_roll_s1_kernel<1>, dim3(g.nsl * g.rows_used), dim3(NT), 0, stream, g);
  else hipLaunchKernelGGL(dw_bwd_roll_s2_kernel, dim3(g.nsl * g.rows_used), dim3(NT), 0, stream, g, Ho, Wo);
  return g.rows_used;
}

}

#ifdef TSS_ROLL_TIMING
extern "C" int tss_debug_roll_timing(unsigned long long* out8, int reset) {
  if (hipMemcpyFromSymbol(out8, HIP_SYMBOL(g_roll_timing), sizeof(unsigned long long) * 8) != hipSuccess) return -1;
  if (reset) { unsigned long long z[8] = {0}; (void)hipMemcpyToSymbol(HIP_SYMBOL(g_roll_timing), z, sizeof(z)); }
  return 0;
}
#endif
```

### torch_semantic_segmentation_amd/csrc/prof.cpp

```cpp
#include <mutex>
#include <vector>

#include "common.h"

namespace {

struct KernelInfo { const char* name; const char* symbol; };
const KernelInfo kInfo[TSS_K_COUNT] = {
    {"pwconv_fwd", "pwfast_kernel<false>|pwfast_mc_kernel<false>|convgemm_kernel"},
    {"pwconv_bwd_data", "pwfast_kernel<true>|pwfast_mc_kernel<true>|pwbwd_kernel|pwsweep_kernel|convgemm_kernel"},
    {"pwconv_bwd_weight", "wgfast_kernel|wgrad_kernel"},
    {"conv3x3_fwd", "conv3x3_wstat_kernel|conv3x3_stream_kernel|conv3x3_lean_kernel<false>|fc1d_kernel|convgemm_kernel<fwd>"}, {"conv3x3_bwd_data", "conv3x3_lean_kernel<true>|fc1d_kernel|convgemm_kernel<bwd>"}, {"conv3x3_bwd_weight", "fc1d_wgrad_kernel|wgrad_kernel"},
    {"stem3x3_fwd", "stem_fwd_mfma_kernel|convgemm_kernel"}, {"stem3x3_bwd_weight", "stem_wgrad_mfma_kernel|stem_wgrad_kernel"},
    {"dwconv3x3_fwd", "dw_fwd_roll_kernel|dw_fwd_strip_kernel"}, {"dwconv3x3_bwd_data", "dw_bwd_roll_s1_kernel|dw_bwd_roll_s2_kernel|dw_bwd_data_strip_kernel"},
    {"dwconv3x3_bwd_weight", "dw_bwd_weight_strip_kernel"},
    {"bn_finalize", "bn_finalize_kernel"}, {"bn_bwd_finalize", "bn_bwd_finalize_kernel"},
    {"join_fwd", "join_fwd_kernel"}, {"join_bwd", "join_bwd_kernel"},
    {"dropout", "dropout_kernel"}, {"bias_grad", "colsum_kernel"}, {"adamw", "adamw_kernel"},
    {"bilinear_nhwc_fwd", "bilinear_nhwc_fwd_kernel|ppm_concat_fwd_kernel"}, {"bilinear_nhwc_bwd_rows", "bilinear_nhwc_bwd_rows_kernel|ppm_concat_bwd_kernel"},
    {"bilinear_nhwc_bwd_cols", "bilinear_nhwc_bwd_cols_kernel"},
    {"bilinear_planar_fwd", "bilinear_planar_fwd_kernel"},
    {"upsample_head_fwd", "upsample_head_fwd_kernel"}, {"upsample_head_bwd_rows", "upsample_head_bwd_rows_kernel"},
    {"upsample_head_bwd_cols", "upsample_head_bwd_cols_kernel"},
    {"adaptive_pool_fwd", "adaptive_pool_fwd_kernel|ppm_pool_fwd_kernel"}, {"adaptive_pool_bwd", "adaptive_pool_bwd_kernel|ppm_pool_bwd_kernel"},
    {"copy_nhwc", "copy_nhwc_kernel"},
    {"cross_entropy_fwd", "ce_fwd_kernel"}, {"cross_entropy_bwd", "ce_bwd_kernel"}, {"argmax_confusion", "argmax_confusion_kernel"},
    {"upsample_ce_fwd", "upsample_ce_onepass_kernel"}, {"upsample_ce_bwd", "upsample_ce_gather_kernel"},
    {"resize_flip_planar", "resize_flip_planar_kernel"}, {"multiscale_argmax_confusion", "multiscale_argmax_kernel"},
    {"sgd", "sgd_kernel"}, {"grad_norm", "grad_sqnorm_kernel|grad_sqnorm_final_kernel"},
    {"upsample_ce_wide_fwd", "wide_ce_kernel"}, {"upsample_ce_wide_bwd", "wide_ce_gather_kernel"},
    {"argmax_confusion_wide", "wide_upsample_argmax_kernel|wide_planar_argmax_kernel"},
    {"multiscale_argmax_confusion_wide", "wide_multiscale_argmax_kernel"},
};

struct Rec { int kid; hipEvent_t a, b; double bytes, flops; };
struct Total { long launches; double ms, bytes, flops; };
struct Done { int kid; double ms, bytes; };
std::vector<Done> g_done;

std::mutex g_mu;
bool g_enabled = false;
std::vector<Rec> g_recs;
std::vector<hipEvent_t> g_pool;
Total g_tot[TSS_K_COUNT];
thread_local char g_err[256] = "";

hipEvent_t get_event() {
  if (!g_pool.empty()) { hipEvent_t e = g_pool.back(); g_pool.pop_back(); return e; }
  hipEvent_t e;
  (void)hipEventCreate(&e);
  return e;
}

}

namespace tss {

int check_last(const char* what) {
  const hipError_t err = hipGetLastError();
  if (err == hipSuccess) return TSS_OK;
  snprintf(g_err, sizeof(g_err), "%s: %s", what, hipGetErrorString(err));
  return TSS_ERR_HIP;
}

ProfScope::ProfScope(int kernel_id, hipStream_t s, double alg_bytes, double flops) : slot(-1), stream(s) {
  if (!g_enabled) return;
  std::lock_guard<std::mutex> lk(g_mu);
  Rec r;
  r.kid = kernel_id; r.bytes = alg_bytes; r.flops = flops;
  r.a = get_event(); r.b = get_event();
  (void)hipEventRecord(r.a, stream);
  g_recs.push_back(r);
  slot = (int)g_recs.size() - 1;
}

ProfScope::~ProfScope() {
  if (slot < 0) return;
  std::lock_guard<std::mutex> lk(g_mu);
  (void)hipEventRecord(g_recs[slot].b, stream);
}

}

extern "C" {

int tss_version(void) { return 1; }

int tss_memset_zero(void* p, long bytes, void* stream) {
  if (!p || bytes <= 0) return TSS_OK;
  if (hipMemsetAsync(p, 0, (size_t)bytes, (hipStream_t)stream) != hipSuccess) return TSS_ERR_HIP;
  return tss::check_last("memset_zero");
}
const char* tss_last_error(void) { return g_err; }
const char* tss_arch(void) { return "gfx950"; }

int tss_prof_enable(int on) {
  std::lock_guard<std::mutex> lk(g_mu);
  g_enabled = on != 0;
  return TSS_OK;
}

int tss_prof_reset(void) {
  std::lock_guard<std::mutex> lk(g_mu);
  for (Rec& r : g_recs) { g_pool.push_back(r.a); g_pool.push_back(r.b); }
  g_recs.clear();
  for (int i = 0; i < TSS_K_COUNT; ++i) g_tot[i] = Total{0, 0.0, 0.0, 0.0};
  g_done.clear();
  return TSS_OK;
}

int tss_prof_collect(void) {
  std::lock_guard<std::mutex> lk(g_mu);
  for (Rec& r : g_recs) {
    if (hipEventSynchronize(r.b) != hipSuccess) return TSS_ERR_HIP;
    float ms = 0.f;
    if (hipEventElapsedTime(&ms, r.a, r.b) != hipSuccess) return TSS_ERR_HIP;
    Total& t = g_tot[r.kid];
    t.launches += 1; t.ms += ms; t.bytes += r.bytes; t.flops += r.flops;
    g_done.push_back(Done{r.kid, (double)ms, r.bytes});
    g_pool.push_back(r.a); g_pool.push_back(r.b);
  }
  g_recs.clear();
  return TSS_OK;
}

int tss_prof_get(int kernel_id, long* launches, double* total_ms, double* alg_bytes, double* flops) {
  if (kernel_id < 0 || kernel_id >= TSS_K_COUNT) return TSS_ERR_SHAPE;
  std::lock_guard<std::mutex> lk(g_mu);
  const Total& t = g_tot[kernel_id];
  if (launches) *launches = t.launches;
  if (total_ms) *total_ms = t.ms;
  if (alg_bytes) *alg_bytes = t.bytes;
  if (flops) *flops = t.flops;
  return TSS_OK;
}

long tss_prof_records(int* kernel_ids, double* ms, double* alg_bytes, long max_records) {
  std::lock_guard<std::mutex> lk(g_mu);
  long n = (long)g_done.size() < max_records ? (long)g_done.size() : max_records;
  for (long i = 0; i < n; ++i) { kernel_ids[i] = g_done[i].kid; ms[i] = g_done[i].ms; alg_bytes[i] = g_done[i].bytes; }
  return (long)g_done.size();
}

const char* tss_prof_name(int kernel_id) {
  return (kernel_id >= 0 && kernel_id < TSS_K_COUNT) ? kInfo[kernel_id].name : "";
}
const char* tss_prof_symbol(int kernel_id) {
  return (kernel_id >= 0 && kernel_id < TSS_K_COUNT) ? kInfo[kernel_id].symbol : "";
}

}
```

### torch_semantic_segmentation_amd/csrc/stem.hip

```cpp
#include "common.h"

namespace {

constexpr int NT = 256;

struct StemArgs {
  const void* x; int x_f32;
  const float* w; void* y; long ldy; double* stats;
  int B, Cin, Hin, Win, Hout, Wout, N, stride;
};

struct __attribute__((packed, aligned(4))) F4u { float x, y, z, w; };
template <typename TX>
__device__ __forceinline__ void stem_taps(const TX* x, long b, int oy, int ox, bool in, int Cin, int Hin, int Win,
                                          int stride, long plane, float v[27]) {
  if (sizeof(TX) == 4 && stride == 2 && Win >= 4) {
    const int ix0 = 2 * ox - 1;
    const int base = ix0 < 0 ? 0 : (ix0 > Win - 4 ? Win - 4 : ix0);
    const int sh = ix0 - base;
#pragma unroll
    for (int c = 0; c < 3; ++c)
#pragma unroll
      for (int ky = 0; ky < 3; ++ky) {
        const int iy = 2 * oy + ky - 1;
        const bool vy = in && c < Cin && iy >= 0 && iy < Hin;
        const float* row = reinterpret_cast<const float*>(x) + (b * Cin + (c < Cin ? c : 0)) * plane + (long)(vy ? iy : 0) * Win + base;
        const F4u f = *reinterpret_cast<const F4u*>(row);
#pragma unroll
        for (int kx = 0; kx < 3; ++kx) {
          const int idx = kx + sh;
          const float t = idx <= 0 ? f.x : (idx == 1 ? f.y : (idx == 2 ? f.z : f.w));
          v[c * 9 + ky * 3 + kx] = (vy && idx >= 0 && ix0 + kx < Win) ? t : 0.f;
        }
      }
    return;
  }
#pragma unroll
  for (int c = 0; c < 3; ++c)
#pragma unroll
    for (int ky = 0; ky < 3; ++ky) {
      const int iy = oy * stride + ky - 1;
      const bool vy = iy >= 0 && iy < Hin;
#pragma unroll
      for (int kx = 0; kx < 3; ++kx) {
        const int ix = ox * stride + kx - 1;
        const bool ok = in && c < Cin && vy && ix >= 0 && ix < Win;
        const long off = (b * Cin + (c < Cin ? c : 0)) * plane + (vy ? iy : 0) * (long)Win + (ix < 0 ? 0 : (ix >= Win ? Win - 1 : ix));
        const float t = (float)x[off];
        v[c * 9 + ky * 3 + kx] = ok ? t : 0.f;
      }
    }
}

template <typename TX>
__global__ __launch_bounds__(NT, 2) void stem_fwd_mfma_kernel(const StemArgs g) {
  typedef bf16_t T;
  constexpr int N = 32, TP = 256, PITCH = 40;
  __shared__ __align__(16) T Xp[TP * PITCH];
  __shared__ float red[NT / 64][2][N];
  const int tid = threadIdx.x, lane = tid & 63, wave = tid >> 6;
  const int fr = lane & 15, fq = lane >> 4;
  const int K = g.Cin * 9;
  bf16x8 wf[2];
#pragma unroll
  for (int i = 0; i < 2; ++i)
#pragma unroll
    for (int j = 0; j < 8; ++j) {
      const int k = fq * 8 + j;
      wf[i][j] = (T)(g.w[(i * 16 + fr) * K + (k < K ? k : 0)] * (k < K ? 1.f : 0.f));
    }
  const TX* x = reinterpret_cast<const TX*>(g.x);
  T* y = reinterpret_cast<T*>(g.y);
  float st1[2][4], st2[2][4];
#pragma unroll
  for (int i = 0; i < 2; ++i)
#pragma unroll
    for (int q = 0; q < 4; ++q) { st1[i][q] = 0.f; st2[i][q] = 0.f; }
  const long P = (long)g.B * g.Hout * g.Wout;
  const long HWo = (long)g.Hout * g.Wout;
  const long plane = (long)g.Hin * g.Win;
  const long ntiles = (P + TP - 1) / TP;
  for (long tile = blockIdx.x; tile < ntiles; tile += gridDim.x) {
    const long p0 = tile * TP;
    {
      const long p = p0 + tid;
      const bool in = p < P;
      const long pc = in ? p : 0;
      const long b = pc / HWo; const long rem = pc - b * HWo;
      const int oy = (int)(rem / g.Wout), ox = (int)(rem - (long)oy * g.Wout);
      float v[32];
      stem_taps<TX>(x, b, oy, ox, in, g.Cin, g.Hin, g.Win, g.stride, plane, v);
#pragma unroll
      for (int k = 27; k < 32; ++k) v[k] = 0.f;
      __syncthreads();
#pragma unroll
      for (int h = 0; h < 4; ++h) V8<T>::store(Xp + tid * PITCH + h * 8, v + h * 8);
    }
    __syncthreads();
#pragma unroll
    for (int m = 0; m < 4; ++m) {
      const int prow = wave * 64 + m * 16 + fr;
      const bf16x8 xf = *reinterpret_cast<const bf16x8*>(Xp + prow * PITCH + fq * 8);
      const long p = p0 + prow;
#pragma unroll
      for (int i = 0; i < 2; ++i) {
        const f32x4 d = __builtin_amdgcn_mfma_f32_16x16x32_bf16(wf[i], xf, (f32x4){0.f, 0.f, 0.f, 0.f}, 0, 0, 0);
        if (p < P) {
          bf16x4 o;
#pragma unroll
          for (int q = 0; q < 4; ++q) o[q] = (T)d[q];
#pragma unroll
          for (int q = 0; q < 4; ++q) { const float rq = (float)o[q]; st1[i][q] += rq; st2[i][q] += rq * rq; }
          *reinterpret_cast<bf16x4*>(y + p * g.ldy + i * 16 + fq * 4) = o;
        }
      }
    }
  }
  if (g.stats) {
#pragma unroll
    for (int i = 0; i < 2; ++i)
#pragma unroll
      for (int q = 0; q < 4; ++q) {
        const float a = row16_sum(st1[i][q]), b = row16_sum(st2[i][q]);
        if (fr == 0) { red[wave][0][i * 16 + fq * 4 + q] = a; red[wave][1][i * 16 + fq * 4 + q] = b; }
      }
    __syncthreads();
    for (int i = tid; i < 2 * N; i += NT) {
      const int which = i / N, n = i - which * N;
      double s = 0.0;
      for (int wv = 0; wv < NT / 64; ++wv) s += (double)red[wv][which][n];
      g.stats[(long)blockIdx.x * 2 * N + i] = s;
      for (int r = blockIdx.x + gridDim.x; r < TSS_STAT_SLABS; r += gridDim.x) g.stats[(long)r * 2 * N + i] = 0.0;
    }
  }
}

struct StemWgradArgs {
  const void* e; long lde; const void* yraw; long ldyr; const float* ga; const float* gb; const float* gce; const float* gmu;
  const void* x; float* ws; float* dw;
  int B, Cin, Hin, Win, Hout, Wout, stride;
};

template <typename T, typename TX>
__global__ __launch_bounds__(NT, 2) void stem_wgrad_kernel(const StemWgradArgs g) {
  constexpr int N = 32, TP = 256, KP = 28;
  __shared__ __align__(16) float Gs[TP * N];
  __shared__ __align__(16) float Xs[TP * KP];
  const int tid = threadIdx.x;
  const T* e = reinterpret_cast<const T*>(g.e);
  const T* yr = reinterpret_cast<const T*>(g.yraw);
  const TX* x = reinterpret_cast<const TX*>(g.x);
  const int K = g.Cin * 9;
  const long P = (long)g.B * g.Hout * g.Wout;
  const long HWo = (long)g.Hout * g.Wout;
  const long plane = (long)g.Hin * g.Win;
  const long ntiles = (P + TP - 1) / TP;
  const int gcv = tid & 3;
  float ca[8], cb[8], cc[8], cm[8];
#pragma unroll
  for (int j = 0; j < 8; ++j) {
    ca[j] = g.ga ? g.ga[gcv * 8 + j] : 1.f;
    cb[j] = g.yraw ? g.gb[gcv * 8 + j] : 0.f;
    cc[j] = g.yraw ? g.gce[gcv * 8 + j] : 0.f;
    cm[j] = g.yraw ? g.gmu[gcv * 8 + j] : 0.f;
  }
  const int n = tid & 31, jg = tid >> 5;
  float acc[4] = {0.f, 0.f, 0.f, 0.f};
  for (long tile = blockIdx.x; tile < ntiles; tile += gridDim.x) {
    const long p0 = tile * TP;
    __syncthreads();
    {
      const long p = p0 + tid;
      const bool in = p < P;
      const long pc = in ? p : 0;
      const long b = pc / HWo; const long rem = pc - b * HWo;
      const int oy = (int)(rem / g.Wout), ox = (int)(rem - (long)oy * g.Wout);
      float* xr = Xs + tid * KP;
#pragma unroll
      for (int c = 0; c < 3; ++c) {
#pragma unroll
        for (int ky = 0; ky < 3; ++ky) {
          const int iy = oy * g.stride + ky - 1;
          const bool vy = iy >= 0 && iy < g.Hin;
#pragma unroll
          for (int kx = 0; kx < 3; ++kx) {
            const int ix = ox * g.stride + kx - 1;
            const bool ok = in && c < g.Cin && vy && ix >= 0 && ix < g.Win;
            const long off = (b * g.Cin + (c < g.Cin ? c : 0)) * plane + (vy ? iy : 0) * (long)g.Win +
                             (ix < 0 ? 0 : (ix >= g.Win ? g.Win - 1 : ix));
            const float v = (float)x[off];
            xr[c * 9 + ky * 3 + kx] = ok ? v : 0.f;
          }
        }
      }
      xr[27] = 0.f;
    }
#pragma unroll
    for (int i = 0; i < 4; ++i) {
      const int px = (tid >> 2) + 64 * i;
      const long p = p0 + px;
      const bool in = p < P;
      const long pc = in ? p : 0;
      float ev[8], gv[8];
      V8<T>::load(e + pc * g.lde + gcv * 8, ev);
      if (yr) {
// ... 197 lines not shown
```

### torch_semantic_segmentation_amd/ops.py

```python
import collections
import ctypes
import math
import os
import threading

import torch
from torch.autograd import Function
from torch.nn.modules.batchnorm import _BatchNorm

from . import _native as N

call, ptr, stream = N.call, N.ptr, N.stream



_DIRECT = [False]


class direct_grads:

    def __init__(self, enabled=True):
        self.enabled = bool(enabled)

    def __enter__(self):
# ... 390 lines not shown
class Dense3x3Shadows(_Scoped):
    _table = _W3X3

    def __init__(self, module):
        self.items = []
        for m in module.modules():
            if (isinstance(m, torch.nn.Conv2d) and m.kernel_size == (3, 3) and m.groups == 1 and m.weight.is_cuda
                    and m.weight.dtype == torch.float32 and m.in_channels % 8 == 0 and m.out_channels % 8 == 0):
                w = m.weight
                self.items.append((w, w.data_ptr(), torch.empty((9, m.out_channels, m.in_channels), dtype=torch.bfloat16, device=w.device)))
        self.entries = {p: t for _, p, t in self.items}

    def refresh(self):
        for w, p, t in self.items:
            if w.data_ptr() != p:
                raise RuntimeError('Dense3x3Shadows: a parameter was reallocated; rebuild the shadows')
            call('tss_permute_w3x3_bf16', ptr(w), ptr(t), None, w.shape[0], w.shape[1], stream())


_EVAL_AFFINES = {}


class EvalAffines(_Scoped):
    _table = _EVAL_AFFINES

    def __init__(self, module):
        import struct
        bns = [m for m in module.modules() if isinstance(m, torch.nn.modules.batchnorm._BatchNorm)
               and m.running_mean is not None and m.running_var is not None and m.running_mean.is_cuda
               and m.running_mean.dtype == torch.float32 and (m.weight is None or m.weight.dtype == torch.float32)]
        self.bns, self.table, self.entries = bns, None, {}
        if not bns:
            return
        dev = bns[0].running_mean.device
        total = sum(3 * m.num_features for m in bns)
        self.flat = torch.empty(total, dtype=torch.float32, device=dev)
        rows, off = [], 0
        for m in bns:
            C = m.num_features
            out = self.flat[off:off + 3 * C].view(3, C)
            off += 3 * C
            self.entries[id(m)] = out
            eps_bits = struct.unpack('<i', struct.pack('<f', float(m.eps)))[0]
            rows.append([m.weight.data_ptr() if m.weight is not None else 0, m.running_mean.data_ptr(),
                         m.running_var.data_ptr(), out.data_ptr(), C, eps_bits])
        self.ptrs = [(r[0], r[1], r[2]) for r in rows]
        self.table = torch.tensor(rows, dtype=torch.int64, device=dev)
        self.max_c = max(m.num_features for m in bns)

    def refresh(self):
        if self.table is None:
            return
        for m, (g, rm, rv) in zip(self.bns, self.ptrs):
            if (m.weight.data_ptr() if m.weight is not None else 0) != g or m.running_mean.data_ptr() != rm \
                    or m.running_var.data_ptr() != rv:
                raise RuntimeError('EvalAffines: a BatchNorm tensor was reallocated; rebuild the affines')
        call('tss_bn_eval_affine_batched', ptr(self.table), self.table.shape[0], self.max_c, stream())


conv3x3_lean_max_dilation = int(os.environ.get('TSS_CONV3X3_LEAN_MAXDIL', '1'))


def _conv3x3_lean(dtype, k, n, stride, dil):
    return (dtype == torch.bfloat16 and stride == 1 and 1 <= dil <= conv3x3_lean_max_dilation and k in (32, 64, 128) and n % 16 == 0 and 16 <= n <= 128
            and not N.fast_paths_disabled())


conv3x3_stream = os.environ.get('TSS_CONV3X3_STREAM', '1') != '0'


def _conv3x3_stream(dtype, k, n, stride, in_link, in_relu):
    return (conv3x3_stream and dtype == torch.bfloat16 and stride == 1 and in_link is None and not in_relu and k % 32 == 0
            and 32 <= k <= 128 and n % 16 == 0 and 16 <= n <= 128 and not N.fast_paths_disabled())


def _shadow(weight, which):
    ent = _SHADOWS.get(weight.data_ptr()) if _SHADOWS else None
    return ptr(ent[which]) if ent is not None else None


def _aff(link):
    if link is None:
        return None, None, None
    return ptr(link.mean), ptr(link.scale), ptr(link.beta)


def _direct_target(param):
    g = param.grad if (param is not None and param.is_leaf) else None
    if _DIRECT[0] and g is not None and g.dtype == torch.float32 and g.is_contiguous() and g.is_cuda:
        return g
    return None


def _grad_target(param, like, shape=None):
    g = _direct_target(param)
    if g is not None:
        return g, None
    g = torch.zeros_like(like) if shape is None else torch.zeros(shape, dtype=torch.float32, device=like.device)
    return g, g



def round_up(v, m):
    return (v + m - 1) // m * m


def new_nhwc(b, c, h, w, dtype, device, ld=None):
    ld = round_up(c, 8) if ld is None else ld
    base = torch.empty((b, h, w, ld), dtype=dtype, device=device)
    t = base.permute(0, 3, 1, 2)
    return t if ld == c else t[:, :c]


def is_nhwc(t):
    if t.dim() != 4 or not t.is_cuda:
        return False
    b, c, h, w = t.shape
    ld = t.stride(3)
    return (t.stride() == (h * w * ld, 1, w * ld, ld) and ld % 8 == 0 and ld >= c
            and t.data_ptr() % 16 == 0)


def to_nhwc(t):
    if is_nhwc(t):
        return t
    _check_device(t)
    out = new_nhwc(*t.shape, t.dtype, t.device)
    out.copy_(t)
    return out


def _check_device(t):
    if not t.is_cuda:
        raise RuntimeError('torch_semantic_segmentation_amd runs on the MI355X HIP path only: got a %s tensor. '
                           'There is no CPU fallback (the CPU oracle lives in oracle/, for tests).' % t.device)
    if t.device.index is not None and t.device.index != torch.cuda.current_device():
        raise RuntimeError('tensor lives on cuda:%d but the current device is cuda:%d; wrap the call in '
                           'torch.cuda.device(%d) (one process per GPU is the supported layout)'
                           % (t.device.index, torch.cuda.current_device(), t.device.index))
    N.lib()


def ld(t):
    return t.stride(3)


def npix(t):
    return t.shape[0] * t.shape[2] * t.shape[3]



class BNLink:
    __slots__ = ('C', 'count', 'training', 'gamma', 'beta', 'vec', 'scale', 'mean', 'invstd',
                 'ga', 'gb', 'gce', 'stats', 'bstats', 'consumed', 'sync')

    def __init__(self, C, count, training, gamma, beta, device, slabs=True):
        self.C, self.count, self.training, self.gamma, self.beta = C, count, training, gamma, beta
        self.vec = torch.empty((6, C), dtype=torch.float32, device=device)
        self.mean, self.invstd, self.scale, self.ga, self.gb, self.gce = self.vec.unbind(0)
        if slabs:
            both = torch.empty((2, N.stat_slabs(), 2 * C), dtype=torch.float64, device=device)
            self.stats, self.bstats = both[0], both[1]
        else:
            self.stats = self.bstats = None
        self.consumed = False
        self.sync = None


class Deferred:
    __slots__ = ('raw', 'link', 'relu')

    def __init__(self, raw, link=None, relu=False):
        self.raw, self.link, self.relu = raw, link, relu

    @property
    def shape(self):
        return self.raw.shape


    def take(self):
        if self.link is not None:
            if self.link.consumed:
                raise RuntimeError('a deferred BatchNorm output may feed exactly one consumer; materialize it first')
            self.link.consumed = True
        return self


class SyncBatchNorm(torch.nn.BatchNorm2d):
    process_group = None


def convert_syncbn_model(module, process_group=None):
    for m in module.modules():
        if isinstance(m, torch.nn.BatchNorm2d) and not isinstance(m, SyncBatchNorm):
            m.__class__ = SyncBatchNorm
            m.process_group = process_group
    return module


def _sync_group(bn, any_mode=False):
    import torch.distributed as dist
    if not isinstance(bn, (SyncBatchNorm, torch.nn.SyncBatchNorm)) or not (bn.training or any_mode):
        return None
    if not (dist.is_available() and dist.is_initialized()):
        return None
    group = getattr(bn, 'process_group', None) or dist.group.WORLD
    return group if (dist.get_world_size(group) > 1 or os.environ.get('TSS_SYNCBN_FORCE') == '1') else None


syncbn_ipc = os.environ.get('TSS_SYNCBN_IPC', '1') != '0'
_XCHG = {}


class _Exchange:

    def __init__(self, group, device):
        import socket
        import torch.distributed as dist
        self.rank, self.world = dist.get_rank(group), dist.get_world_size(group)
        self.device = device
        if self.world > 8:
            raise RuntimeError('more than 8 ranks')
        nbytes = N.lib().tss_bn_xchg_bytes()
        own, handle = ctypes.c_void_p(), (ctypes.c_char * 64)()
        with torch.cuda.device(device):
            call('tss_ipc_alloc', nbytes, ctypes.byref(own), handle)
            self.own = own.value
            me = (socket.gethostname(), os.getpid(), bytes(handle.raw))
            everyone = [None] * self.world
            if self.world > 1:
                dist.all_gather_object(everyone, me, group=group)
            else:
                everyone[0] = me
            if len({h for h, _, _ in everyone}) != 1:
                call('tss_ipc_free', self.own)
                raise RuntimeError('the ranks of the group are not on one node')
            self.mapped = []
            ptrs = []
            for r, (_, pid, hb) in enumerate(everyone):
                if r == self.rank:
                    ptrs.append(self.own)
                    continue
                if pid == os.getpid():
                    raise RuntimeError('two ranks in one process')
                p_ = ctypes.c_void_p()
                call('tss_ipc_open', ctypes.create_string_buffer(hb, 64), ctypes.byref(p_))
                self.mapped.append(p_.value)
                ptrs.append(p_.value)
        self.peers = (ctypes.c_void_p * self.world)(*ptrs)
        self.counters = torch.zeros(N.lib().tss_bn_xchg_counters(), dtype=torch.int64, device=device)
        if self.world > 1:
            dist.barrier(group=group)

    def error(self):
        out = ctypes.c_long(0)
        with torch.cuda.device(self.device):
            call('tss_bn_xchg_error', self.own, ctypes.byref(out))
        return out.value


def _exchange(group, device):
    if not syncbn_ipc:
        return None
    key = (group, device.index)
    if key not in _XCHG:
        try:
            _XCHG[key] = _Exchange(group, device)
        except Exception as exc:
            import warnings
            warnings.warn('SyncBatchNorm: HIP IPC exchange unavailable (%s); using dist.all_reduce' % (exc,))
            _XCHG[key] = None
    return _XCHG[key]


def _allreduce_stats(slabs, count, C, group, st):
    import torch.distributed as dist
    vec = torch.empty(2 * C + 1, dtype=torch.float64, device=slabs.device)
    call('tss_slab_reduce', ptr(slabs), float(count), ptr(vec), C, st)
    dist.all_reduce(vec, op=dist.ReduceOp.SUM, group=group)
    return vec


def as_deferred(x):
    if isinstance(x, Deferred):
        return x
    _check_device(x)
    N.dtype_code(x.dtype)
    return Deferred(to_nhwc(x))


def materialize(d, relu_override=None):
    if not isinstance(d, Deferred):
        return d
    if d.link is None and not d.relu:
        return d.raw
    return join(d, None, d.relu)



class UnitCfg:
    __slots__ = ('kind', 'stride', 'dil', 'in_link', 'in_relu', 'bn', 'training', 'out_dtype', 'out_link',
                 'image_f32', 'cin', 'cout', 'params', 'res_fork', 'stash_fork', 'overlapped', 'kh', 'kw', 'drop_p', 'prev_join')


def _classify(conv, x_is_image):
    k = conv.kernel_size
    if tuple(k) in ((1, 3), (3, 1)):
        ax = 0 if tuple(k) == (1, 3) else 1
        d = conv.dilation[1 - ax]
        want_pad, want_dil = ((0, d), (1, d)) if ax == 0 else ((d, 0), (d, 1))
        if (conv.padding_mode != 'zeros' or conv.groups != 1 or tuple(conv.stride) != (1, 1) or tuple(conv.padding) != want_pad
                or tuple(conv.dilation) != want_dil or x_is_image):
            raise NotImplementedError('HIP path: 1x3 / 3x1 convolutions must be dense, stride 1, padding = dilation on the '
                                      'kernel axis: %r' % conv)
        return 'dense1d_w' if ax == 0 else 'dense1d_h', 1, d
    kh, kw = k
    if conv.groups == 1 and not x_is_image and kh % 2 == 1 and kw % 2 == 1 and (kh != kw or kh > 3):
        dd = [conv.dilation[i] for i in (0, 1) if k[i] > 1]
        d = dd[0]
# ... 403 lines not shown

def _res_grad(cfg):
    fork = cfg.res_fork
    return fork, (fork.g2 if fork is not None else None)


def _bwd_stem(c):
    ws = c.tmp((N.stat_slabs(), c.Cout * 28))
    call('tss_stem3x3_bwd_weight', *c.gargs, ptr(c.x), int(c.cfg.image_f32), ptr(c.dw), ptr(ws),
         c.B, c.Cin, c.Hin, c.Win, c.Cout, c.s, c.dt, c.st)
    if c.need_dx:
        raise NotImplementedError('HIP path: gradient with respect to the input image is not implemented')
    return None, _NO_EXTRAS



def _bwd_pw(c):
    P, Cin, Cout, dt = c.P, c.Cin, c.Cout, c.dt
    fused = bool(fuse_pw_backward and c.need_dx and c.side is None and c.e.dtype == torch.bfloat16
                 and not N.fast_paths_disabled() and N.lib().tss_pwconv_bwd_fused_preferred(P, Cin, Cout, dt))
    if c.drop_mask is not None:
        fused = True
    if fused:
        return _bwd_pw_fused(c)
    radd_s = _res_grad(c.cfg)[1]
    sweep = bool(sweep_pw_backward and c.need_dx and c.side is None and c.e.dtype == torch.bfloat16 and c.x.dtype == torch.bfloat16
                 and not N.fast_paths_disabled()
                 and N.lib().tss_pwconv_bwd_sweep_preferred(P, Cin, Cout, int(bool(c.deferred_in)), dt)
                 and (radd_s is None or (not c.deferred_in and radd_s.dtype == c.e.dtype and tuple(radd_s.shape) == tuple(c.x.shape)
                                         and is_nhwc(radd_s))))
    if sweep:
        return _bwd_pw_sweep(c)
    return _bwd_pw_split(c)


def _bwd_pw_fused(c):
    e_in = _new_e_in(c)
    if e_in is None:
        return None, _NO_EXTRAS
    P, Cin, Cout, weight, drop_mask = c.P, c.Cin, c.Cout, c.weight, c.drop_mask
    rows = (N.lib().tss_pwconv_bwd_fused_drop_rows(P) if drop_mask is not None
            else N.lib().tss_pwconv_bwd_fused_rows(P, Cin, Cout))
    ws = c.tmp((rows, Cout * Cin))
    bws = dbias = dbias_ret = None
    if c.has_bias:
        bws = c.tmp((rows, Cout))
        dbias, dbias_ret = _grad_target(c.p_bias, weight, Cout)
    if drop_mask is not None:
        call('tss_pwconv_bwd_fused_drop', *c.gargs, ptr(weight), *c.xargs, int(bool(c.deferred_in)), ptr(drop_mask),
             c.cfg.drop_p, ptr(e_in), ld(e_in), c.bst, ptr(ws), ptr(bws), P, Cin, Cout, c.dt, c.st)
    else:
        call('tss_pwconv_bwd_fused', *c.gargs, ptr(weight), _shadow(weight, 1), *c.xargs, int(bool(c.deferred_in)),
             ptr(e_in), ld(e_in), c.bst, ptr(ws), ptr(bws), P, Cin, Cout, c.dt, c.st)
    returned = c.dw_ret if c.dw_ret is not None else dbias_ret
    _add_rows(ws, c.dw, Cout * Cin, rows, c.p_weight, returned)
    if bws is not None:
        _add_rows(bws, dbias, Cout, rows, c.p_bias, returned)
    return e_in, (None, True, dbias_ret)


def _bwd_pw_sweep(c):
    e_in = _new_e_in(c)
    if e_in is None:
        return None, _NO_EXTRAS
    P, Cin, Cout, weight = c.P, c.Cin, c.Cout, c.weight
    fork, radd_s = _res_grad(c.cfg)
    rows = N.lib().tss_pwconv_bwd_sweep_rows(P, Cin, Cout)
    ws = c.tmp((rows, Cout * Cin))
    wT = _shadow(weight, 1)
    hold_wT = None
    if wT is None:
        hold_wT = weight.detach().reshape(Cout, Cin).t().contiguous().to(torch.bfloat16)
        wT = ptr(hold_wT)
    call('tss_pwconv_bwd_sweep', *c.gargs, wT, *c.xargs, int(bool(c.deferred_in)), ptr(radd_s),
         ld(radd_s) if radd_s is not None else 0, ptr(e_in), ld(e_in), c.bst, ptr(ws), P, Cin, Cout, c.dt, c.st)
    del hold_wT
    if radd_s is not None:
        fork.consumed = True
    _add_rows(ws, c.dw, Cout * Cin, rows, c.p_weight, c.dw_ret)
    return e_in, _NO_EXTRAS


def _bwd_pw_split(c):
    P, Cin, Cout, dt = c.P, c.Cin, c.Cout, c.dt
    nws = N.lib().tss_pwconv_bwd_weight_ws(P, Cin, Cout, dt) if c.y is not None else 0
    ws = c.tmp(nws) if nws else None
    defer = 1 if (ws is not None and c.need_dx and c.side is None) else 0
    postponed = bool(defer and postpone_wgrad and c.dw_ret is None and not c.cfg.overlapped
                     and _backward_task() != -1 and not _param_observed(c.p_weight))
    if not postponed:
        _flush_wg(c.st)
        _flush_red(c.st)
        call('tss_pwconv_bwd_weight', *c.gargs, *c.xargs, ptr(c.dw), ptr(ws), defer, P, Cin, Cout, dt, None, c.wst)
    e_in = _new_e_in(c)
    if e_in is None:
        return None, _NO_EXTRAS
    if postponed:
        red, hold = _take_red(c.dev)
    else:
        red, hold = ((ptr(ws), ptr(c.dw), 0, 0, 0) if defer else (None, None, 0, 0, 0)), None
    _pw_data_grad(c, e_in, red)
    del hold
    if postponed:
        _postpone_pw_wgrad(c, ws)
    return e_in, _NO_EXTRAS


def _pw_data_grad(c, e_in, red):
    e, x, y, weight, P, Cin, Cout, dt, st = c.e, c.x, c.y, c.weight, c.P, c.Cin, c.Cout, c.dt, c.st
    deferred_in = c.deferred_in
    fork, radd = _res_grad(c.cfg)
    radd_ok = (radd is not None and not deferred_in and y is not None and e.dtype == torch.bfloat16 and radd.dtype == e.dtype
               and tuple(radd.shape) == tuple(e_in.shape) and N.lib().tss_pwconv_bwd_data_radd_supported(P, Cin, Cout, dt))
    pj = c.cfg.prev_join
    if (pj is not None and (radd is None or radd_ok) and not deferred_in and y is not None and e.dtype == torch.bfloat16
            and P * Cin <= fuse_join_backward_max
            and pj.j_a is not None and tuple(pj.j_a.shape) == tuple(x.shape)
            and is_nhwc(pj.j_a) and N.lib().tss_pwconv_bwd_data_radd_supported(P, Cin, Cout, dt)):
        jl = pj.a_link
        call('tss_pwconv_bwd_data_joined', *c.gargs, ptr(weight), _shadow(weight, 1), ptr(e_in), ld(e_in), *red,
             ptr(radd), ld(radd) if radd is not None else 0, ptr(x), ld(x), ptr(pj.j_a), ld(pj.j_a), ptr(jl.mean),
             ptr(jl.bstats), P, Cin, Cout, dt, st)
        pj.fused_e = e_in
        if radd is not None:
            fork.consumed = True
    elif radd_ok:
        call('tss_pwconv_bwd_data_radd', *c.gargs, ptr(weight), _shadow(weight, 1), ptr(e_in), ld(e_in),
             *red, ptr(radd), ld(radd), P, Cin, Cout, dt, st)
        fork.consumed = True
    else:
        call('tss_pwconv_bwd_data', *c.gargs, ptr(weight), _shadow(weight, 1), *c.margs, ptr(e_in), ld(e_in), c.bst,
             *red, P, Cin, Cout, dt, st)


def _postpone_pw_wgrad(c, ws):
    st = c.st
    _flush_wg(st)
    own = torch.cuda.current_stream(c.dev)
    ps = _cur_pass()

    def launch_wg(fin, _keep=(c.e, c.y, c.x, c.link, c.il, ws, c.dw), _args=(c.gargs, c.xargs, ptr(c.dw), ptr(ws), c.P, c.Cin, c.Cout, c.dt),
                  _sid=st, _own=own, _ps=ps):
        ga_, xa_, dwp, wsp, P_, K_, N_, dt_ = _args
        call('tss_pwconv_bwd_weight', *ga_, *xa_, dwp, wsp, 1, P_, K_, N_, dt_,
             ctypes.byref(fin) if fin is not None else None, _sid)
        _flush_red(_sid, _ps)
        with _lock:
            _ps.red[_sid] = (_keep[5], _keep[6], P_, K_, N_, _keep[0].device, _own)
    with _lock:
        ps.wg[st] = (launch_wg, c.dev, own)



def _bwd_dw(c):
    weight, B, Hin, Win, Cout, s, d, dt, st = c.weight, c.B, c.Hin, c.Win, c.Cout, c.s, c.d, c.dt, c.st
    ws = c.tmp((N.stat_slabs(), Cout * 9))
    defer = 1 if (c.need_dx and c.side is None) else 0
    fused = bool(defer and ((fuse_dw_backward and N.lib().tss_dwconv3x3_bwd_fused_supported(Cout, s, d, dt))
                            or N.lib().tss_dwconv3x3_bwd_fused_preferred(Cout, s, d, dt)))
    if not fused:
        call('tss_dwconv3x3_bwd_weight', *c.gargs, *c.xargs, ptr(c.dw), ptr(ws), defer, B, Hin, Win, Cout, s, d, dt, c.wst)
    e_in = _new_e_in(c)
    if e_in is None:
        return None, _NO_EXTRAS
    if fused and c.dw_ret is None and batch_dw_reductions:
        rows = ctypes.c_int(0)
        call('tss_dwconv3x3_bwd_fused_sweep', *c.gargs, ptr(weight), *c.xargs, int(bool(c.deferred_in)), ptr(e_in), ld(e_in),
             c.bst, ptr(ws), B, Hin, Win, Cout, s, d, dt, st, ctypes.byref(rows))
        _add_rows(ws, c.dw, Cout * 9, rows.value, c.p_weight, c.dw_ret)
    elif fused:
        call('tss_dwconv3x3_bwd_fused', *c.gargs, ptr(weight), *c.xargs, int(bool(c.deferred_in)), ptr(e_in), ld(e_in),
             c.bst, ptr(ws), ptr(c.dw), B, Hin, Win, Cout, s, d, dt, st)
    else:
        call('tss_dwconv3x3_bwd_data', *c.gargs, ptr(weight), *c.margs, ptr(e_in), ld(e_in), c.bst,
             ptr(ws) if defer else None, ptr(c.dw) if defer else None, B, Hin, Win, Cout, s, d, dt, st)
    return e_in, _NO_EXTRAS


def _tap_sweep_wgrad(c, entry, rows, taps, *geom):
    ncols = c.Cout * c.Cin * taps
    ws = c.tmp((rows, ncols))
    call(entry, *c.gargs, *c.xargs, ptr(ws), c.B, c.Hin, c.Win, c.Cin, c.Cout, *geom, c.dt, c.wst)
    return ws, rows, ncols


def _pw_wgrad_of_columns(c, gargs, col, K):
    nws = N.lib().tss_pwconv_bwd_weight_ws(c.P, K, c.Cout, c.dt)
    ws = c.tmp(nws) if nws else None
    call('tss_pwconv_bwd_weight', *gargs, ptr(col), K, None, None, None, 0, ptr(c.dw), ptr(ws), 0,
         c.P, K, c.Cout, c.dt, None, c.wst)


def _dense1d_wgrad(c, axis):
    e, y, P, Cin, Cout, d, dt = c.e, c.y, c.P, c.Cin, c.Cout, c.d, c.dt
    rows = N.lib().tss_conv1d3_bwd_weight_rows(P, Cin, Cout, dt)
    rows_w = 0 if rows else N.lib().tss_convtap_bwd_weight_rows(P, Cin, Cout, 3, dt)
    if rows_w:
        return _tap_sweep_wgrad(c, 'tss_convtap_bwd_weight_sweep', rows_w, 3, 3, axis, d)
    if rows:
        return _tap_sweep_wgrad(c, 'tss_conv1d3_bwd_weight_sweep', rows, 3, axis, d)
    if (e.dtype == torch.bfloat16 and Cin % 8 == 0 and Cout % 8 == 0 and unfold_1d_wgrad and not N.fast_paths_disabled()):
        col = c.tmp((P, Cin * 3), torch.bfloat16)
        call('tss_im2col1d3', *c.xargs, ptr(col), c.B, c.Hin, c.Win, Cin, axis, d, dt, c.wst)
        g_ = c.gargs
        if y is None:
            one, zero = _const_rows(c.dev, Cout)
            g_ = (ptr(e), ld(e), ptr(e), ld(e), ptr(c.ga) if c.ga is not None else ptr(one), ptr(zero), ptr(zero), ptr(zero))
        _pw_wgrad_of_columns(c, g_, col, Cin * 3)
    else:
        call('tss_conv1d3_bwd_weight', *c.gargs, *c.xargs, ptr(c.dw), c.B, c.Hin, c.Win, Cin, Cout, axis, d, dt, c.wst)
    return None


def _bwd_dense1d(c):
    weight, B, Hin, Win, Cin, Cout, d, dt, st = c.weight, c.B, c.Hin, c.Win, c.Cin, c.Cout, c.d, c.dt, c.st
    axis = 0 if c.cfg.kind == 'dense1d_w' else 1
    extras = (_dense1d_wgrad(c, axis), False, None)
    e_in = _new_e_in(c)
    if e_in is None:
        return None, extras
    if N.lib().tss_conv1d3_lean_supported(Cin, Cout, dt):
        call('tss_conv1d3_bwd_data_w', *c.gargs, ptr(weight), *c.margs, ptr(e_in), ld(e_in), c.bst,
             B, Hin, Win, Cin, Cout, axis, d, dt, st)
    else:
        w_tcn = c.tmp((3, Cin, Cout))
        call('tss_permute_wtaps', ptr(weight), None, ptr(w_tcn), Cout, Cin, 3, st)
        call('tss_conv1d3_bwd_data', *c.gargs, ptr(w_tcn), *c.margs, ptr(e_in), ld(e_in), c.bst,
             B, Hin, Win, Cin, Cout, axis, d, dt, st)
    return e_in, extras


def _kxk_data_grad(c, e_in):
    cfg, Cin, Cout, st = c.cfg, c.Cin, c.Cout, c.st
    nt = cfg.kh * cfg.kw
    w_tcn = c.tmp((nt, Cin, Cout))
    call('tss_permute_wtaps', ptr(c.weight), None, ptr(w_tcn), Cout, Cin, nt, st)
    call('tss_convkxk_bwd_data', *c.gargs, ptr(w_tcn), *c.margs, ptr(e_in), ld(e_in), c.bst,
         c.B, c.Hin, c.Win, Cin, Cout, cfg.kh, cfg.kw, c.s, c.d, c.dt, st)


def _bwd_ckk(c):
    cfg, P, Cin, Cout, s, d, dt = c.cfg, c.P, c.Cin, c.Cout, c.s, c.d, c.dt
    rows_after_join = None
    if (s == 1 and (cfg.kh, cfg.kw) in ((1, 5), (5, 1)) and N.lib().tss_convtap_bwd_weight_rows(P, Cin, Cout, 5, dt)):
        rows = N.lib().tss_convtap_bwd_weight_rows(P, Cin, Cout, 5, dt)
        rows_after_join = _tap_sweep_wgrad(c, 'tss_convtap_bwd_weight_sweep', rows, 5, 5, 0 if cfg.kh == 1 else 1, d)
    else:
        call('tss_convkxk_bwd_weight', *c.gargs, *c.xargs, ptr(c.dw), c.B, c.Hin, c.Win, Cin, Cout, cfg.kh, cfg.kw, s, d, dt, c.wst)
    e_in = _new_e_in(c)
    if e_in is not None:
        _kxk_data_grad(c, e_in)
    return e_in, (rows_after_join, False, None)


def _dense_wgrad(c):
    e, B, Hin, Win, P, Cin, Cout, s, d, dt = c.e, c.B, c.Hin, c.Win, c.P, c.Cin, c.Cout, c.s, c.d, c.dt
    if (s == 2 and d == 1 and N.lib().tss_sconv_bwd_weight_rows(B, Hin, Win, Cin, Cout, dt)):
        rows = N.lib().tss_sconv_bwd_weight_rows(B, Hin, Win, Cin, Cout, dt)
        return _tap_sweep_wgrad(c, 'tss_sconv_bwd_weight_sweep', rows, 9)
    if (e.dtype == torch.bfloat16 and s == 1 and c.y is not None and (Cin * 9) % 8 == 0 and Cout % 8 == 0
            and not N.fast_paths_disabled()):
        col = c.tmp((P, Cin * 9), torch.bfloat16)
        call('tss_im2col3x3', *c.xargs, ptr(col), B, Hin, Win, Cin, d, dt, c.wst)
        _pw_wgrad_of_columns(c, c.gargs, col, Cin * 9)
    else:
        call('tss_conv3x3_bwd_weight', *c.gargs, *c.xargs, ptr(c.dw), B, Hin, Win, Cin, Cout, s, d, dt, c.wst)
    return None


def _bwd_dense(c):
    weight, Cin, Cout, d, st = c.weight, c.Cin, c.Cout, c.d, c.st
    extras = (_dense_wgrad(c), False, None)
    e_in = _new_e_in(c)
    if e_in is None:
        return None, extras
    if c.s != 1:
        _kxk_data_grad(c, e_in)
        return e_in, extras
    w_tcn = w_tcn16 = None
    if _conv3x3_lean(c.e.dtype, Cout, Cin, 1, d):
        w_tcn16 = c.tmp((9, Cin, Cout), torch.bfloat16)
        call('tss_permute_w3x3_bf16', ptr(weight), None, ptr(w_tcn16), Cout, Cin, st)
    else:
        w_tcn = c.tmp((9, Cin, Cout))
        call('tss_permute_w3x3', ptr(weight), None, ptr(w_tcn), Cout, Cin, st)
    call('tss_conv3x3_bwd_data', *c.gargs, ptr(w_tcn), ptr(w_tcn16), *c.margs, ptr(e_in), ld(e_in), c.bst,
         c.B, c.Hin, c.Win, Cin, Cout, d, c.dt, st)
    return e_in, extras


_BWD = {'stem': _bwd_stem, 'pw': _bwd_pw, 'dw': _bwd_dw, 'ckk': _bwd_ckk, 'dense': _bwd_dense,
        'dense1d_w': _bwd_dense1d, 'dense1d_h': _bwd_dense1d}


def _bias_backward(c):
    e, P, Cout, link = c.e, c.P, c.Cout, c.link
    if link is not None and link.training:
        return _grad_target(c.p_bias, c.weight, Cout)[1]
    if link is not None:
        dbias = _direct_target(c.p_bias)
        tmp = torch.zeros(Cout, dtype=torch.float32, device=c.dev)
        _bias_grad_into(e, P, Cout, tmp, c.dt, c.st)
        if dbias is None:
            return tmp * link.ga
        dbias.addcmul_(tmp, link.ga)
        return None
    dbias, dbias_ret = _grad_target(c.p_bias, c.weight, Cout)
    _bias_grad_into(e, P, Cout, dbias, c.dt, c.st)
    return dbias_ret


class ConvUnitFn(Function):
    @staticmethod
    def forward(ctx, x, weight, gamma, beta, bias, cfg):
        dev = x.device
        B = x.shape[0]
        dt = N.dtype_code(cfg.out_dtype)
        s, d = cfg.stride, cfg.dil
        Hin, Win = x.shape[2], x.shape[3]
        Ho, Wo = (Hin - 1) // s + 1, (Win - 1) // s + 1
        Cout = cfg.cout
        y = new_nhwc(B, Cout, Ho, Wo, cfg.out_dtype, dev)
        P = B * Ho * Wo
        link = None
        if cfg.bn is not None:
            if cfg.training and P <= 1:
                raise ValueError('Expected more than 1 value per channel when training, got input size %s'
                                 % (tuple(y.shape),))
            link = BNLink(Cout, P, cfg.training, gamma, beta, dev)
        stats = ptr(link.stats) if (link is not None and cfg.training) else None
        st = stream()
        mask = _FWD[cfg.kind](_FwdArgs(cfg, x, weight, bias, y, _aff(cfg.in_link), stats, B, Hin, Win, Cout, P, s, d, dt, dev, st))
        if link is not None:
            _finalize_forward(link, cfg.bn, cfg.training, P, Cout, gamma, st)
        cfg.out_link = link
        ctx.cfg = cfg
        ctx.save_for_backward(x, weight, y if link is not None else None, mask)
        ctx.has_bias = bias is not None
        ctx.has_affine = gamma is not None
        return y

    @staticmethod
    def backward(ctx, e):
        cfg = ctx.cfg
        c = _Bwd()
        c.cfg, c.temps = cfg, []
        x, weight, y, drop_mask = ctx.saved_tensors
        c.x, c.weight, c.drop_mask = x, weight, drop_mask
        c.dev = dev = x.device
        c.e = e = to_nhwc(e)
        c.dt = N.dtype_code(e.dtype)
        c.st = st = stream()
        c.link = link = cfg.out_link
        c.B, c.Hin, c.Win = x.shape[0], x.shape[2], x.shape[3]
        c.s, c.d = cfg.stride, cfg.dil
        c.Cout, c.Cin = cfg.cout, cfg.cin
        Cout = c.Cout
        c.P = P = npix(e)
        c.p_weight, p_gamma, p_beta, c.p_bias = cfg.params
        dgamma, dbeta, c.y, c.ga, gb, gce, gmu = _bn_backward_prologue(link, ctx.has_affine, p_gamma, p_beta, Cout, y, dev, st)
        y = c.y
        c.gargs = (ptr(e), ld(e), ptr(y), ld(y) if y is not None else 0, ptr(c.ga), ptr(gb), ptr(gce), ptr(gmu))
        c.il = il = cfg.in_link
        c.xargs = (ptr(x), ld(x), *_aff(il), int(cfg.in_relu))
        c.deferred_in = il is not None or cfg.in_relu
        c.margs = c.xargs if c.deferred_in else (None, 0, None, None, None, 0)
        c.bst = ptr(il.bstats) if il is not None else None
        c.dw, c.dw_ret = _grad_target(c.p_weight, weight)
        c.need_dx = need_dx = ctx.needs_input_grad[0]
        c.has_bias = ctx.has_bias
        main = torch.cuda.current_stream(dev)
        c.side = side = _wgrad_side_stream(cfg, need_dx, drop_mask, P, dev)
        c.wst = st
        if side is not None:
            side.wait_stream(main)
            c.wst = side.cuda_stream
        e_in, (rows_after_join, bias_done, dbias_ret) = _BWD[cfg.kind](c)
        stash = cfg.stash_fork
        if stash is not None and e_in is not None and not c.deferred_in:
            stash.g2 = e_in
        if ctx.has_bias and not bias_done:
            dbias_ret = _bias_backward(c)
        if side is not None:
            main.wait_stream(side)
        if rows_after_join is not None:
            ws, rows, ncols = rows_after_join
            _add_rows(ws, c.dw, ncols, rows, c.p_weight, c.dw_ret)
        return e_in, c.dw_ret, dgamma, dbeta, dbias_ret, None



class JoinCfg:
    __slots__ = ('a_link', 'b_link', 'relu', 'drop_p', 'res_fork', 'j_a', 'fused_e')


class BranchCfg:
    __slots__ = ('links', 'relus', 'res_fork')


class PpmArmsCfg:
    __slots__ = ('convs', 'bns', 'links')


def join(a, b=None, relu=False, dropout_p=0.0, fork=None):
    a = as_deferred(a).take()
    cfg = JoinCfg()
    cfg.relu = bool(relu)
    cfg.drop_p = float(dropout_p)
    if cfg.drop_p and not (relu and 0.0 < cfg.drop_p < 1.0):
        raise RuntimeError('join: dropout can only be folded into a ReLU join, 0 < p < 1')
    if a.relu and (b is not None or not relu):
        raise RuntimeError('join: a pending ReLU can only be folded into a single-input relu join')
    cfg.a_link = a.link
    braw = None
    cfg.b_link = None
    if b is not None:
        b = as_deferred(b).take()
        if b.relu:
            raise RuntimeError('join: operand b carries a pending ReLU; materialize it first')
        if b.raw.shape != a.raw.shape or b.raw.dtype != a.raw.dtype:
            raise RuntimeError('join: operands differ in shape/dtype: %s vs %s' % (a.raw.shape, b.raw.shape))
        braw, cfg.b_link = b.raw, b.link
    cfg.res_fork = fork if b is not None else None
    cfg.j_a = cfg.fused_e = None
    out = JoinFn.apply(a.raw, braw, cfg)
    if (fuse_join_backward and cfg.relu and not cfg.drop_p and cfg.a_link is not None and cfg.b_link is None and out.requires_grad
            and out.dtype == torch.bfloat16 and not N.fast_paths_disabled()):
        cfg.j_a = a.raw
        _hand(out, _JOIN, cfg)
    return out


class JoinFn(Function):
    @staticmethod
    def forward(ctx, a, b, cfg):
        out = new_nhwc(*a.shape, a.dtype, a.device)
        al, bl = cfg.a_link, cfg.b_link
        slot = None
        if cfg.drop_p:
            slot = torch.empty(1, dtype=torch.int64, device=a.device)
            call('tss_dropout_tick', ptr(_dropout_counter(a.device)), ptr(slot), stream())
        call('tss_join_fwd', ptr(a), ld(a), *_aff(al), ptr(b), ld(b) if b is not None else 0, *_aff(bl),
             ptr(out), ld(out), int(cfg.relu), cfg.drop_p, ptr(slot), npix(a), a.shape[1], N.dtype_code(a.dtype), stream())
        ctx.cfg = cfg
        ctx.has_b = b is not None
        ctx.save_for_backward(a if al is not None else None, b if bl is not None else None,
                              out if cfg.relu else None)
        return out

    @staticmethod
    def backward(ctx, dout):
        cfg = ctx.cfg
        a, b, out = ctx.saved_tensors
        fe = cfg.fused_e
        cfg.fused_e = None
        if (fe is not None and dout.data_ptr() == fe.data_ptr() and dout.shape == fe.shape and dout.dtype == fe.dtype
                and dout.stride() == fe.stride()):
            fork = cfg.res_fork
            if fork is not None and ctx.has_b:
                fork.g2 = dout
            return dout, (dout if ctx.has_b else None), None
        del fe
        dout = to_nhwc(dout)
        al, bl = cfg.a_link, cfg.b_link
        e = new_nhwc(*dout.shape, dout.dtype, dout.device) if cfg.relu else None
        if cfg.relu or al is not None or bl is not None:
            call('tss_join_bwd', ptr(dout), ld(dout), ptr(out), ld(out) if out is not None else 0, int(cfg.relu),
                 ptr(a), ld(a) if a is not None else 0, ptr(al.mean) if al else None, ptr(al.bstats) if al else None,
                 ptr(b), ld(b) if b is not None else 0, ptr(bl.mean) if bl else None, ptr(bl.bstats) if bl else None,
                 ptr(e), ld(e) if e is not None else 0, 1.0 / (1.0 - cfg.drop_p) if cfg.drop_p else 1.0,
                 npix(dout), dout.shape[1], N.dtype_code(dout.dtype), stream())
        g = e if e is not None else dout
        fork = cfg.res_fork
        if fork is not None and ctx.has_b:
            fork.g2 = g
        return g, (g if ctx.has_b else None), None



_dropout_counters = {}


def _dropout_counter(device):
    return _per_device(_dropout_counters, device,
                       lambda: torch.tensor([torch.initial_seed() & 0x7FFFFFFFFFFFFFFF], dtype=torch.int64, device=device))


def dropout(x, p, training):
    if not training or p == 0.0:
        return x
    if p >= 1.0:
        raise NotImplementedError('HIP path: dropout with p >= 1')
    return DropoutFn.apply(to_nhwc(x), float(p))


class DropoutFn(Function):
    @staticmethod
# ... 1893 lines not shown
```

Before: 1732 images/sec.

## Fuse stem conv backward into the following depthwise conv backward sweep

```diff
diff --git a/include/tss_hip.h b/include/tss_hip.h
--- a/include/tss_hip.h
+++ b/include/tss_hip.h
@@ -34,6 +34,7 @@
   TSS_K_RESIZE_FLIP_PLANAR, TSS_K_MULTISCALE_ARGMAX,
   TSS_K_SGD, TSS_K_GRAD_NORM,
   TSS_K_WIDE_CE_FWD, TSS_K_WIDE_CE_BWD, TSS_K_WIDE_ARGMAX, TSS_K_WIDE_MULTISCALE_ARGMAX,
+  TSS_K_STEM_TAIL_BWD_SWEEP, TSS_K_STEM_TAIL_BWD_FINISH,
   TSS_K_COUNT
 };
 
@@ -253,6 +254,18 @@
                              const void* xraw, long ldx, const float* in_mean, const float* in_scale, const float* in_bias, int in_relu,
                              float* dw, float* ws , int defer_reduce,
                              int B, int Hin, int Win, int C, int stride, int dil, int dtype, void* stream);
+
+int tss_stem_tail_supported(int C, int Cin, int Hi, int Wi, int dtype);
+int tss_stem_tail_row_floats(void);
+int tss_stem_tail_bwd_sweep(const void* e, long lde, const void* yraw, long ldyr,
+                            const float* ga, const float* gb, const float* gce, const float* gmu, const float* w,
+                            const void* x, long ldx, const float* in_mean, const float* in_scale, const float* in_bias, int in_relu,
+                            const void* image, int image_f32, int Cin, int Hi, int Wi,
+                            double* bstats, float* ws, float* tail_rows,
+                            int B, int C, int dtype, int grid_cap, void* stream, int* rows_out);
+int tss_stem_tail_bwd_finish(const double* bstats, double count, const float* invstd, const float* gamma, int accumulate,
+                             float* dgamma, float* dbeta, float* ga, float* gb, float* gce, const float* mean,
+                             const float* tail_rows, int rows, float* dw, int Cin, int C, void* stream);
 
 int tss_updw_supported(int B, int Hs, int Ws, int Ho, int Wo, int C, int dil, int dtype);
 int tss_updw_ws_rows(int B, int Hs, int Ws, int Ho, int Wo, int C, int dil, int dtype);
diff --git a/torch_semantic_segmentation_amd/_native.py b/torch_semantic_segmentation_amd/_native.py
--- a/torch_semantic_segmentation_amd/_native.py
+++ b/torch_semantic_segmentation_amd/_native.py
@@ -93,7 +93,7 @@
 
 
 
-K_COUNT = 41
+K_COUNT = 43
 
 
 def prof_enable(on=True):
diff --git a/torch_semantic_segmentation_amd/build.py b/torch_semantic_segmentation_amd/build.py
--- a/torch_semantic_segmentation_amd/build.py
+++ b/torch_semantic_segmentation_amd/build.py
@@ -7,7 +7,7 @@
 CSRC = os.path.join(HERE, 'csrc')
 INCLUDE = os.path.join(os.path.dirname(HERE), 'include')
 LIB = os.path.join(HERE, 'libtss_hip.so')
-SOURCES = ['convgemm.hip', 'pwfast.hip', 'pwbwd.hip', 'pwsweep.hip', 'bneck.hip', 'conv3x3.hip', 'fc1d.hip', 'fcg.hip', 'sconv.hip', 'atrous.hip', 'wstat.hip', 'stem.hip', 'wgrad.hip', 'dwconv.hip', 'dwroll.hip', 'updw.hip', 'pointwise.hip', 'optim.hip', 'xchg.hip', 'resample.hip', 'ppm.hip', 'loss.hip', 'ohem.hip', 'lovasz.hip', 'softloss.hip', 'distill.hip', 'labelhist.hip', 'hostio.hip', 'augment.hip', 'msflip.hip', 'widehead.hip', 'softhead.hip', 'gate.hip', 'zoo.hip', 'ssnbt.hip', 'prof.cpp']
+SOURCES = ['convgemm.hip', 'pwfast.hip', 'pwbwd.hip', 'pwsweep.hip', 'bneck.hip', 'conv3x3.hip', 'fc1d.hip', 'fcg.hip', 'sconv.hip', 'atrous.hip', 'wstat.hip', 'stem.hip', 'stemtail.hip', 'wgrad.hip', 'dwconv.hip', 'dwroll.hip', 'updw.hip', 'pointwise.hip', 'optim.hip', 'xchg.hip', 'resample.hip', 'ppm.hip', 'loss.hip', 'ohem.hip', 'lovasz.hip', 'softloss.hip', 'distill.hip', 'labelhist.hip', 'hostio.hip', 'augment.hip', 'msflip.hip', 'widehead.hip', 'softhead.hip', 'gate.hip', 'zoo.hip', 'ssnbt.hip', 'prof.cpp']
 HIPCC = os.environ.get('HIPCC', '/opt/rocm/bin/hipcc')
 FLAGS = ['--offload-arch=gfx950', '-O3', '-fPIC', '-std=c++17', '-Wall', '-Wno-unused-function',
          '-I' + INCLUDE, '-I' + CSRC]
diff --git a/torch_semantic_segmentation_amd/csrc/dwroll.hip b/torch_semantic_segmentation_amd/csrc/dwroll.hip
--- a/torch_semantic_segmentation_amd/csrc/dwroll.hip
+++ b/torch_semantic_segmentation_amd/csrc/dwroll.hip
@@ -3,10 +3,11 @@
 #include <cstdlib>
 
 #include "common.h"
+#include "dwrollbwd.h"
 
 namespace {
 
-constexpr int NT = 256;
+using namespace tss_roll;
 constexpr int ENT = NT + 16;
 
 struct RollArgs {
@@ -35,8 +36,6 @@
   }
 }
 
-__device__ __forceinline__ int clampi(int v, int lo, int hi) { return v < lo ? lo : (v > hi ? hi : v); }
-
 typedef unsigned int u32x4 __attribute__((ext_vector_type(4)));
 __device__ __forceinline__ void request(u32x4& dst, const bf16_t* uniform_base, int elem_offset) {
   asm volatile("global_load_dwordx4 %0, %1, %2" : "=v"(dst) : "v"(elem_offset * 2), "s"(uniform_base));
@@ -61,42 +60,6 @@
 __device__ __forceinline__ void fetch(const float4* lo4, const float4* hi4, int e, float v[8]) {
   const float4 a = lo4[e], b = hi4[e];
   v[0] = a.x; v[1] = a.y; v[2] = a.z; v[3] = a.w; v[4] = b.x; v[5] = b.y; v[6] = b.z; v[7] = b.w;
-}
-
-template <int NC>
-__device__ __forceinline__ void flush_slab(const float (&s1)[NC], const float (&s2)[NC], double* stats, int C, int CVS, int PXL,
-                                           int sl, int brow, int rows_used, int p, int cg, bool lane_on, float* red) {
-  const int tid = threadIdx.x;
-  const int cw = CVS * NC;
-  __syncthreads();
-  if (p < PXL) {
-#pragma unroll
-    for (int j = 0; j < NC; ++j) {
-      red[(p * 2 + 0) * cw + cg * NC + j] = lane_on ? s1[j] : 0.f;
-      red[(p * 2 + 1) * cw + cg * NC + j] = lane_on ? s2[j] : 0.f;
-    }
-  }
-  __syncthreads();
-  const int ncol = 2 * cw, share = NT / ncol;
-  float part = 0.f;
-  const int col = tid % ncol, sub = tid / ncol;
-  if (sub < share) {
-#pragma unroll 8
-    for (int q = sub; q < PXL; q += share) part += red[(q * 2 + col / cw) * cw + col % cw];
-  }
-  float* part_s = red + NT * 16;
-  if (sub < share) part_s[sub * ncol + col] = part;
-  __syncthreads();
-  if (tid < ncol) {
-    const int which = tid / cw, c = tid - which * cw;
-    const int ch = sl * 64 + c;
-    if (ch < C) {
-      double a = 0.0;
-      for (int q = 0; q < share; ++q) a += (double)part_s[q * ncol + tid];
-      stats[(long)brow * 2 * C + which * C + ch] = a;
-      for (int r = brow + rows_used; r < TSS_STAT_SLABS; r += rows_used) stats[(long)r * 2 * C + which * C + ch] = 0.0;
-    }
-  }
 }
 
 template <int S> struct RollCfg;
@@ -347,41 +310,17 @@
 }
 
 
-typedef unsigned int u32x2 __attribute__((ext_vector_type(2)));
-__device__ __forceinline__ void request2(u32x2& dst, const bf16_t* uniform_base, int elem_offset) {
-  asm volatile("global_load_dwordx2 %0, %1, %2" : "=v"(dst) : "v"(elem_offset * 2), "s"(uniform_base));
-}
 template <int N> __device__ __forceinline__ void arrived2(u32x2& a, u32x2& b, u32x2& c, u32x2& d, u32x2& e, u32x2& f) {
   asm volatile("s_waitcnt vmcnt(%6)" : "+v"(a), "+v"(b), "+v"(c), "+v"(d), "+v"(e), "+v"(f) : "n"(N));
 }
-__device__ __forceinline__ void settle(float (&a)[4]) { asm volatile("" : "+v"(a[0]), "+v"(a[1]), "+v"(a[2]), "+v"(a[3])); }
-__device__ __forceinline__ void settle(float4& a) { asm volatile("" : "+v"(a.x), "+v"(a.y), "+v"(a.z), "+v"(a.w)); }
-__device__ __forceinline__ u32x2 keep2(const u32x2& r) {
-  u32x2 o;
-  asm volatile("v_mov_b32 %0, %2\n\tv_mov_b32 %1, %3" : "=&v"(o[0]), "=&v"(o[1]) : "v"(r[0]), "v"(r[1]));
-  return o;
-}
-__device__ __forceinline__ void unpack4(const u32x2& r, float v[4]) {
-  v[0] = __uint_as_float(r[0] << 16); v[1] = __uint_as_float(r[0] & 0xffff0000u);
-  v[2] = __uint_as_float(r[1] << 16); v[3] = __uint_as_float(r[1] & 0xffff0000u);
-}
 __device__ __forceinline__ float4 ld4(const float* p) { return *reinterpret_cast<const float4*>(p); }
 
-struct RollBwdArgs {
-  const bf16_t* e; long lde; const bf16_t* yr; long ldyr; const float* ga; const float* gb; const float* gce; const float* gmu;
-  const float* w;
-  const bf16_t* x; long ldx; const float* xm; const float* xs; const float* xb; int x_relu, x_mask;
-  bf16_t* ein; long ldei; double* stats; float* ws;
-  int B, H, W, C;
-  int CVS, PXL, nsl, nstrips, RS, nseg, rows_used, dseg, dstrip, db;
-};
 #ifdef TSS_ROLL_TIMING
 __device__ unsigned long long g_roll_timing[8];
 #define TSS_RT(var) unsigned long long var; asm volatile("s_memtime %0\n s_waitcnt lgkmcnt(0)" : "=s"(var) :: "memory")
 #else
 #define TSS_RT(var)
 #endif
-constexpr int BENT = NT + 32;
 constexpr int BPF = TSS_ROLL_BPF1;
 
 struct BCursor { int it, b, strip, seg, x0, o0; };
@@ -666,28 +605,6 @@
 }
 
 constexpr int B2PF = TSS_ROLL_BPF2;
-
-struct B2Cursor { int it, b, strip, seg, x0, o0; };
-__device__ __forceinline__ void advance(B2Cursor& c, const RollBwdArgs& g, int n_iter) {
-  if (++c.it == n_iter) {
-    c.it = 0;
-    c.seg += g.dseg;
-    int carry = c.seg >= g.nseg ? 1 : 0;
-    c.seg -= carry * g.nseg;
-    c.strip += g.dstrip + carry;
-    carry = c.strip >= g.nstrips ? 1 : 0;
-    c.strip -= carry * g.nstrips;
-    c.b += g.db + carry;
-    c.x0 = c.strip * g.PXL;
-    c.o0 = c.seg * g.RS;
-  }
-}
-template <int N>
-__device__ __forceinline__ void arrived10(u32x2 (&r)[10]) {
-  asm volatile("s_waitcnt vmcnt(%10)"
-               : "+v"(r[0]), "+v"(r[1]), "+v"(r[2]), "+v"(r[3]), "+v"(r[4]), "+v"(r[5]), "+v"(r[6]), "+v"(r[7]), "+v"(r[8]), "+v"(r[9])
-               : "n"(N));
-}
 
 __global__ __launch_bounds__(NT, 2) void dw_bwd_roll_s2_kernel(const RollBwdArgs g, const int Ho, const int Wo) {
   __shared__ __align__(16) float4 rows_s[6][BENT];
@@ -927,33 +844,6 @@
   }
 }
 
-void plan_bwd(RollBwdArgs& g, int S, int Ho, int Wo, int rpj = 1) {
-  const int cv4 = g.C / 4;
-  g.nsl = (g.C + 63) / 64;
-  g.CVS = cv4 < 16 ? cv4 : 16;
-  g.PXL = NT / g.CVS;
-  g.nstrips = (Wo + g.PXL - 1) / g.PXL;
-  const int cap = TSS_STAT_SLABS / g.nsl > 0 ? TSS_STAT_SLABS / g.nsl : 1;
-  const int halo = S == 1 ? 2 : 1;
-  long best_cost = -1;
-  for (int nseg = 1; nseg <= Ho; ++nseg) {
-    const int RS = (Ho + nseg - 1) / nseg;
-    if (RS < 4 && nseg > 1) break;
-    const int segs = (Ho + RS - 1) / RS;
-    const long units = (long)g.B * g.nstrips * segs;
-    const long k = (units + cap - 1) / cap;
-    const long cost = k * ((RS + halo + rpj - 1) / rpj) * rpj + 6;
-    if (best_cost < 0 || cost < best_cost) {
-      best_cost = cost;
-      g.RS = RS; g.nseg = segs;
-      g.rows_used = (int)((units + k - 1) / k);
-    }
-  }
-  g.dseg = g.rows_used % g.nseg;
-  g.dstrip = (g.rows_used / g.nseg) % g.nstrips;
-  g.db = g.rows_used / (g.nseg * g.nstrips);
-}
-
 inline size_t ring_bytes(int S) { return (size_t)2 * S * S * 2 * ENT * sizeof(float4); }
 
 }
diff --git a/torch_semantic_segmentation_amd/csrc/dwrollbwd.h b/torch_semantic_segmentation_amd/csrc/dwrollbwd.h
--- /dev/null
+++ b/torch_semantic_segmentation_amd/csrc/dwrollbwd.h
@@ -0,0 +1,122 @@
+#pragma once
+#include "common.h"
+
+namespace tss_roll {
+
+constexpr int NT = 256;
+constexpr int BENT = NT + 32;
+
+__device__ __forceinline__ int clampi(int v, int lo, int hi) { return v < lo ? lo : (v > hi ? hi : v); }
+
+template <int NC>
+__device__ __forceinline__ void flush_slab(const float (&s1)[NC], const float (&s2)[NC], double* stats, int C, int CVS, int PXL,
+                                           int sl, int brow, int rows_used, int p, int cg, bool lane_on, float* red) {
+  const int tid = threadIdx.x;
+  const int cw = CVS * NC;
+  __syncthreads();
+  if (p < PXL) {
+#pragma unroll
+    for (int j = 0; j < NC; ++j) {
+      red[(p * 2 + 0) * cw + cg * NC + j] = lane_on ? s1[j] : 0.f;
+      red[(p * 2 + 1) * cw + cg * NC + j] = lane_on ? s2[j] : 0.f;
+    }
+  }
+  __syncthreads();
+  const int ncol = 2 * cw, share = NT / ncol;
+  float part = 0.f;
+  const int col = tid % ncol, sub = tid / ncol;
+  if (sub < share) {
+#pragma unroll 8
+    for (int q = sub; q < PXL; q += share) part += red[(q * 2 + col / cw) * cw + col % cw];
+  }
+  float* part_s = red + NT * 16;
+  if (sub < share) part_s[sub * ncol + col] = part;
+  __syncthreads();
+  if (tid < ncol) {
+    const int which = tid / cw, c = tid - which * cw;
+    const int ch = sl * 64 + c;
+    if (ch < C) {
+      double a = 0.0;
+      for (int q = 0; q < share; ++q) a += (double)part_s[q * ncol + tid];
+      stats[(long)brow * 2 * C + which * C + ch] = a;
+      for (int r = brow + rows_used; r < TSS_STAT_SLABS; r += rows_used) stats[(long)r * 2 * C + which * C + ch] = 0.0;
+    }
+  }
+}
+
+typedef unsigned int u32x2 __attribute__((ext_vector_type(2)));
+__device__ __forceinline__ void request2(u32x2& dst, const bf16_t* uniform_base, int elem_offset) {
+  asm volatile("global_load_dwordx2 %0, %1, %2" : "=v"(dst) : "v"(elem_offset * 2), "s"(uniform_base));
+}
+__device__ __forceinline__ void settle(float (&a)[4]) { asm volatile("" : "+v"(a[0]), "+v"(a[1]), "+v"(a[2]), "+v"(a[3])); }
+__device__ __forceinline__ void settle(float4& a) { asm volatile("" : "+v"(a.x), "+v"(a.y), "+v"(a.z), "+v"(a.w)); }
+__device__ __forceinline__ u32x2 keep2(const u32x2& r) {
+  u32x2 o;
+  asm volatile("v_mov_b32 %0, %2\n\tv_mov_b32 %1, %3" : "=&v"(o[0]), "=&v"(o[1]) : "v"(r[0]), "v"(r[1]));
+  return o;
+}
+__device__ __forceinline__ void unpack4(const u32x2& r, float v[4]) {
+  v[0] = __uint_as_float(r[0] << 16); v[1] = __uint_as_float(r[0] & 0xffff0000u);
+  v[2] = __uint_as_float(r[1] << 16); v[3] = __uint_as_float(r[1] & 0xffff0000u);
+}
+
+struct RollBwdArgs {
+  const bf16_t* e; long lde; const bf16_t* yr; long ldyr; const float* ga; const float* gb; const float* gce; const float* gmu;
+  const float* w;
+  const bf16_t* x; long ldx; const float* xm; const float* xs; const float* xb; int x_relu, x_mask;
+  bf16_t* ein; long ldei; double* stats; float* ws;
+  int B, H, W, C;
+  int CVS, PXL, nsl, nstrips, RS, nseg, rows_used, dseg, dstrip, db;
+};
+
+struct B2Cursor { int it, b, strip, seg, x0, o0; };
+__device__ __forceinline__ void advance(B2Cursor& c, const RollBwdArgs& g, int n_iter) {
+  if (++c.it == n_iter) {
+    c.it = 0;
+    c.seg += g.dseg;
+    int carry = c.seg >= g.nseg ? 1 : 0;
+    c.seg -= carry * g.nseg;
+    c.strip += g.dstrip + carry;
+    carry = c.strip >= g.nstrips ? 1 : 0;
+    c.strip -= carry * g.nstrips;
+    c.b += g.db + carry;
+    c.x0 = c.strip * g.PXL;
+    c.o0 = c.seg * g.RS;
+  }
+}
+template <int N>
+__device__ __forceinline__ void arrived10(u32x2 (&r)[10]) {
+  asm volatile("s_waitcnt vmcnt(%10)"
+               : "+v"(r[0]), "+v"(r[1]), "+v"(r[2]), "+v"(r[3]), "+v"(r[4]), "+v"(r[5]), "+v"(r[6]), "+v"(r[7]), "+v"(r[8]), "+v"(r[9])
+               : "n"(N));
+}
+
+inline void plan_bwd(RollBwdArgs& g, int S, int Ho, int Wo, int rpj = 1, int grid_cap = 0) {
+  const int cv4 = g.C / 4;
+  g.nsl = (g.C + 63) / 64;
+  g.CVS = cv4 < 16 ? cv4 : 16;
+  g.PXL = NT / g.CVS;
+  g.nstrips = (Wo + g.PXL - 1) / g.PXL;
+  int cap = TSS_STAT_SLABS / g.nsl > 0 ? TSS_STAT_SLABS / g.nsl : 1;
+  if (grid_cap > 0 && grid_cap < cap) cap = grid_cap;
+  const int halo = S == 1 ? 2 : 1;
+  long best_cost = -1;
+  for (int nseg = 1; nseg <= Ho; ++nseg) {
+    const int RS = (Ho + nseg - 1) / nseg;
+    if (RS < 4 && nseg > 1) break;
+    const int segs = (Ho + RS - 1) / RS;
+    const long units = (long)g.B * g.nstrips * segs;
+    const long k = (units + cap - 1) / cap;
+    const long cost = k * ((RS + halo + rpj - 1) / rpj) * rpj + 6;
+    if (best_cost < 0 || cost < best_cost) {
+      best_cost = cost;
+      g.RS = RS; g.nseg = segs;
+      g.rows_used = (int)((units + k - 1) / k);
+    }
+  }
+  g.dseg = g.rows_used % g.nseg;
+  g.dstrip = (g.rows_used / g.nseg) % g.nstrips;
+  g.db = g.rows_used / (g.nseg * g.nstrips);
+}
+
+}
diff --git a/torch_semantic_segmentation_amd/csrc/prof.cpp b/torch_semantic_segmentation_amd/csrc/prof.cpp
--- a/torch_semantic_segmentation_amd/csrc/prof.cpp
+++ b/torch_semantic_segmentation_amd/csrc/prof.cpp
@@ -31,6 +31,7 @@
     {"upsample_ce_wide_fwd", "wide_ce_kernel"}, {"upsample_ce_wide_bwd", "wide_ce_gather_kernel"},
     {"argmax_confusion_wide", "wide_upsample_argmax_kernel|wide_planar_argmax_kernel"},
     {"multiscale_argmax_confusion_wide", "wide_multiscale_argmax_kernel"},
+    {"stem_tail_bwd_sweep", "stem_tail_sweep_kernel"}, {"stem_tail_bwd_finish", "stem_tail_finish_kernel"},
 };
 
 struct Rec { int kid; hipEvent_t a, b; double bytes, flops; };
diff --git a/torch_semantic_segmentation_amd/csrc/stem.hip b/torch_semantic_segmentation_amd/csrc/stem.hip
--- a/torch_semantic_segmentation_amd/csrc/stem.hip
+++ b/torch_semantic_segmentation_amd/csrc/stem.hip
@@ -1,4 +1,5 @@
 #include "common.h"
+#include "stemtaps.h"
 
 namespace {
 
@@ -10,47 +11,7 @@
   int B, Cin, Hin, Win, Hout, Wout, N, stride;
 };
 
-struct __attribute__((packed, aligned(4))) F4u { float x, y, z, w; };
-template <typename TX>
-__device__ __forceinline__ void stem_taps(const TX* x, long b, int oy, int ox, bool in, int Cin, int Hin, int Win,
-                                          int stride, long plane, float v[27]) {
-  if (sizeof(TX) == 4 && stride == 2 && Win >= 4) {
-    const int ix0 = 2 * ox - 1;
-    const int base = ix0 < 0 ? 0 : (ix0 > Win - 4 ? Win - 4 : ix0);
-    const int sh = ix0 - base;
-#pragma unroll
-    for (int c = 0; c < 3; ++c)
-#pragma unroll
-      for (int ky = 0; ky < 3; ++ky) {
-        const int iy = 2 * oy + ky - 1;
-        const bool vy = in && c < Cin && iy >= 0 && iy < Hin;
-        const float* row = reinterpret_cast<const float*>(x) + (b * Cin + (c < Cin ? c : 0)) * plane + (long)(vy ? iy : 0) * Win + base;
-        const F4u f = *reinterpret_cast<const F4u*>(row);
-#pragma unroll
-        for (int kx = 0; kx < 3; ++kx) {
-          const int idx = kx + sh;
-          const float t = idx <= 0 ? f.x : (idx == 1 ? f.y : (idx == 2 ? f.z : f.w));
-          v[c * 9 + ky * 3 + kx] = (vy && idx >= 0 && ix0 + kx < Win) ? t : 0.f;
-        }
-      }
-    return;
-  }
-#pragma unroll
-  for (int c = 0; c < 3; ++c)
-#pragma unroll
-    for (int ky = 0; ky < 3; ++ky) {
-      const int iy = oy * stride + ky - 1;
-      const bool vy = iy >= 0 && iy < Hin;
-#pragma unroll
-      for (int kx = 0; kx < 3; ++kx) {
-        const int ix = ox * stride + kx - 1;
-        const bool ok = in && c < Cin && vy && ix >= 0 && ix < Win;
-        const long off = (b * Cin + (c < Cin ? c : 0)) * plane + (vy ? iy : 0) * (long)Win + (ix < 0 ? 0 : (ix >= Win ? Win - 1 : ix));
-        const float t = (float)x[off];
-        v[c * 9 + ky * 3 + kx] = ok ? t : 0.f;
-      }
-    }
-}
+using tss_stem::stem_taps;
 
 template <typename TX>
 __global__ __launch_bounds__(NT, 2) void stem_fwd_mfma_kernel(const StemArgs g) {
diff --git a/torch_semantic_segmentation_amd/csrc/stemtail.hip b/torch_semantic_segmentation_amd/csrc/stemtail.hip
--- /dev/null
+++ b/torch_semantic_segmentation_amd/csrc/stemtail.hip
@@ -0,0 +1,544 @@
+#include <cstdlib>
+
+#include "bnfin.h"
+#include "common.h"
+#include "dwroll.h"
+#include "dwrollbwd.h"
+#include "stemtaps.h"
+
+namespace {
+
+using namespace tss_roll;
+
+constexpr int SPF = 2;
+constexpr int TPX = 128;
+constexpr int TROW = TPX + 8;
+constexpr int NTAP = 5;
+constexpr int N = 32, KP = 28;
+constexpr int ROWF = 2 * N * KP + KP;
+static_assert(ROWF % 4 == 0 && (8 * KP) % 4 == 0, "the finish kernel reads rows 16 bytes at a time");
+
+struct TailArgs { const void* img; int Cin, Hi, Wi; float* rows; };
+
+typedef unsigned int u32x3 __attribute__((ext_vector_type(3)));
+__device__ __forceinline__ void request3(u32x3& dst, const float* uniform_base, int float_offset) {
+  asm volatile("global_load_dwordx3 %0, %1, %2" : "=v"(dst) : "v"(float_offset * 4), "s"(uniform_base));
+}
+template <int N_>
+__device__ __forceinline__ void arrived15(u32x2 (&r)[10], u32x3 (&t)[NTAP]) {
+  asm volatile("s_waitcnt vmcnt(%15)"
+               : "+v"(r[0]), "+v"(r[1]), "+v"(r[2]), "+v"(r[3]), "+v"(r[4]), "+v"(r[5]), "+v"(r[6]), "+v"(r[7]), "+v"(r[8]), "+v"(r[9]),
+                 "+v"(t[0]), "+v"(t[1]), "+v"(t[2]), "+v"(t[3]), "+v"(t[4])
+               : "n"(N_));
+}
+
+__device__ __forceinline__ float mul_then_add(float a, float b, float c) {
+#pragma clang fp contract(off)
+  const float prod = a * b;
+  return prod + c;
+}
+
+constexpr int RING_BYTES = 6 * BENT * (int)sizeof(float4);
+constexpr int TILE_ELEMS = 32 * TROW;
+constexpr int TILE_BYTES = 2 * 3 * TILE_ELEMS * (int)sizeof(bf16_t);
+constexpr int NCONST = 12;
+constexpr int SMEM_BYTES = RING_BYTES + TILE_BYTES + NCONST * 8 * (int)sizeof(float4);
+static_assert(RING_BYTES >= (int)sizeof(float) * (NT * 16 + NT), "flush_slab scratch");
+static_assert(TILE_BYTES >= (int)sizeof(float) * (4 * 32 * 32 + 4 * 32), "tail reduction scratch");
+static_assert(2 * SMEM_BYTES <= 160 * 1024, "two blocks per CU");
+
+template <bool FAST, typename TX>
+__global__ __launch_bounds__(NT, 2) void stem_tail_sweep_kernel(const RollBwdArgs g, const TailArgs t, const int Ho, const int Wo) {
+  extern __shared__ __align__(16) unsigned char tail_smem[];
+  float4 (*rows_s)[BENT] = reinterpret_cast<float4 (*)[BENT]>(tail_smem);
+  bf16_t* tiles = reinterpret_cast<bf16_t*>(tail_smem + RING_BYTES);
+  float4* cl = reinterpret_cast<float4*>(tail_smem + RING_BYTES + TILE_BYTES);
+  const int tid = threadIdx.x, lane = tid & 63;
+  const int wave = __builtin_amdgcn_readfirstlane(tid >> 6);
+  const int fr = lane & 15, fq = lane >> 4;
+  const int p = tid / g.CVS, cg = tid - p * g.CVS;
+  const int brow = (int)blockIdx.x;
+  const int c0 = cg * 4;
+  const bool halo_l = p == 0, halo_r = p == g.PXL - 1;
+  const int lde = (int)g.lde, ldx = (int)g.ldx;
+  const int ldyy = (int)g.ldyr;
+  const int gp = tid & (TPX - 1), grow = gp >> 6, gcol = gp & 63, half = wave >> 1;
+  const long plane = (long)t.Hi * t.Wi;
+
+  const int n_iter = g.RS + 1;
+  B2Cursor ci, cc;
+  ci.it = 0;
+  ci.seg = brow % g.nseg;
+  ci.strip = (brow / g.nseg) % g.nstrips;
+  ci.b = brow / (g.nseg * g.nstrips);
+  ci.x0 = ci.strip * g.PXL;
+  ci.o0 = ci.seg * g.RS;
+  cc = ci;
+
+  u32x2 raw[SPF][10];
+  u32x3 traw[NTAP];
+  auto issue = [&](const B2Cursor& c, u32x2 (&r)[10]) {
+    const int b = c.b < g.B ? c.b : g.B - 1;
+    const int o = c.o0 + c.it;
+    const long orow = ((long)b * Ho + clampi(o, 0, Ho - 1)) * Wo;
+    const bf16_t* re = g.e + orow * g.lde;
+    const bf16_t* ry = g.yr + orow * g.ldyr;
+    const int po = clampi(c.x0 + p, 0, Wo - 1), pr = clampi(c.x0 + (halo_r ? p + 1 : p), 0, Wo - 1);
+    request2(r[0], re, po * lde + c0);
+    request2(r[1], ry, po * ldyy + c0);
+    request2(r[2], re, pr * lde + c0);
+    request2(r[3], ry, pr * ldyy + c0);
+    const int ix = 2 * (c.x0 + p);
+    const int x0c = clampi(ix, 0, g.W - 1), x1c = clampi(ix + 1, 0, g.W - 1), xlc = clampi(halo_l ? ix - 1 : ix, 0, g.W - 1);
+#pragma unroll
+    for (int ry2 = 0; ry2 < 2; ++ry2) {
+      const int iy = clampi(2 * o - 1 + ry2, 0, g.H - 1);
+      const bf16_t* rx = g.x + ((long)b * g.H + iy) * g.W * g.ldx;
+      request2(r[4 + 3 * ry2], rx, x0c * ldx + c0);
+      request2(r[5 + 3 * ry2], rx, x1c * ldx + c0);
+      request2(r[6 + 3 * ry2], rx, xlc * ldx + c0);
+    }
+  };
+  auto win_ch = [&](int i) { const int q = half * NTAP + i < 9 ? half * NTAP + i : 8; return (q * 11) >> 5; };
+  auto win_ky = [&](int i) { const int q = half * NTAP + i < 9 ? half * NTAP + i : 8; return q - 3 * ((q * 11) >> 5); };
+  int t_oy = 0, t_ox = 0;
+  bool t_in = false;
+  auto issue_taps = [&](const B2Cursor& c) {
+    const int o = c.o0 + c.it;
+    const int r = 2 * o - 1 + grow, col = 2 * c.x0 + gcol;
+    t_in = (grow == 0 ? c.it != 0 : c.it != g.RS) && r >= 0 && r < g.H && col < g.W;
+    t_oy = clampi(r, 0, g.H - 1); t_ox = clampi(col, 0, g.W - 1);
+    if constexpr (FAST) {
+      const float* img = reinterpret_cast<const float*>(t.img) + (long)c.b * t.Cin * plane;
+      int shf;
+      const int base = tss_stem::window_base(t_ox, t.Wi, &shf, 3);
+#pragma unroll
+      for (int i = 0; i < NTAP; ++i) {
+        const int ch = win_ch(i), iy = clampi(2 * t_oy + win_ky(i) - 1, 0, t.Hi - 1);
+        request3(traw[i], img, (ch < t.Cin ? ch : t.Cin - 1) * (int)plane + iy * t.Wi + base);
+      }
+    }
+  };
+#pragma unroll
+  for (int i = 0; i < NTAP; ++i) traw[i] = (u32x3){0u, 0u, 0u};
+  static_assert(SPF == 2, "the wait counts below are those of two steps of rows in flight");
+#pragma unroll
+  for (int k = 0; k < SPF; ++k) {
+    issue(ci, raw[k]);
+    advance(ci, g, n_iter);
+  }
+
+  for (int i = tid; i < 2 * 5 * TROW; i += NT) {
+    const int s = i / (5 * TROW);
+    tiles[(s * 3 + 2) * TILE_ELEMS + 27 * TROW + (i - s * 5 * TROW)] = (bf16_t)0.f;
+  }
+  if (tid < NCONST * 8) {
+    const int q = tid >> 3, wc = (tid & 7) * 4;
+    float v[4];
+#pragma unroll
+    for (int j = 0; j < 4; ++j) {
+      const int c = wc + j;
+      const float a = g.ga[c], b = g.gb[c];
+      v[j] = q < 9 ? g.w[c * 9 + q] : (q == 9 ? a : (q == 10 ? b : __builtin_fmaf(-b, g.gmu[c], -(a * g.gce[c]))));
+    }
+    cl[tid] = make_float4(v[0], v[1], v[2], v[3]);
+  }
+  auto const_of = [&](int q, float (&v)[4]) { const float4 f = cl[q * 8 + cg]; v[0] = f.x; v[1] = f.y; v[2] = f.z; v[3] = f.w; };
+
+  float sc[4], sh[4], mu[4];
+  {
+    float t0[4], t1[4], t2[4];
+    V4<float>::load(g.xs + c0, t0);
+    V4<float>::load(g.xb + c0, t1);
+    V4<float>::load(g.xm + c0, t2);
+#pragma unroll
+    for (int j = 0; j < 4; ++j) {
+      sc[j] = t0[j];
+      mu[j] = t2[j];
+      sh[j] = __builtin_fmaf(-mu[j], sc[j], t1[j]);
+    }
+  }
+  const float relu_lo = g.x_relu ? 0.f : -TSS_INF;
+  float dwa[9][4], gprev[4], gprev_r[4], s1[4], s2[4];
+#pragma unroll
+  for (int j = 0; j < 4; ++j) {
+    gprev[j] = gprev_r[j] = s1[j] = s2[j] = 0.f;
+#pragma unroll
+    for (int tp = 0; tp < 9; ++tp) dwa[tp][j] = 0.f;
+  }
+  const int msrc = wave & 1, mkh = wave >> 1;
+  f32x4 acc[2][2], accP[2];
+#pragma unroll
+  for (int i = 0; i < 2; ++i) {
+    accP[i] = (f32x4){0.f, 0.f, 0.f, 0.f};
+#pragma unroll
+    for (int j = 0; j < 2; ++j) acc[i][j] = (f32x4){0.f, 0.f, 0.f, 0.f};
+  }
+  bf16x8 ones;
+#pragma unroll
+  for (int j = 0; j < 8; ++j) ones[j] = (bf16_t)1.f;
+  __syncthreads();
+
+  auto g_of = [&](const u32x2& re, const u32x2& ry, bool valid, float (&go)[4]) {
+    float ev[4], yv[4], ca[4], cb[4], kd[4];
+    unpack4(re, ev); unpack4(ry, yv);
+    const_of(9, ca); const_of(10, cb); const_of(11, kd);
+#pragma unroll
+    for (int j = 0; j < 4; ++j) go[j] = valid ? ca[j] * ev[j] + (cb[j] * yv[j] + kd[j]) : 0.f;
+  };
+  auto a_of = [&](const u32x2& rx, bool valid, float (&ao)[4]) {
+    float xv[4];
+    unpack4(rx, xv);
+    const float lo = valid ? relu_lo : 0.f, hi = valid ? TSS_INF : 0.f;
+#pragma unroll
+    for (int j = 0; j < 4; ++j) ao[j] = clamp3(xv[j] * sc[j] + sh[j], lo, hi);
+  };
+  auto put4 = [&](float4* row, int e, const float (&v)[4]) { row[e] = make_float4(v[0], v[1], v[2], v[3]); };
+  auto get4 = [&](const float4* row, int e, float (&v)[4]) { const float4 q = row[e]; v[0] = q.x; v[1] = q.y; v[2] = q.z; v[3] = q.w; };
+  auto emit = [&](bool owned, int q, int px, const u32x2& xraw, const float (&a)[4], float (&out)[4]) -> bool {
+    const bool in = owned && q >= 0 && q < g.H && px < g.W;
+    if (in) {
+      float xv[4];
+      unpack4(xraw, xv);
+#pragma unroll
+      for (int j = 0; j < 4; ++j) {
+        const bool dead = g.x_relu && !(xv[j] * sc[j] + sh[j] > 0.f);
+        out[j] = V8<bf16_t>::round(dead ? 0.f : a[j]);
+        s1[j] += out[j];
+        const float dx = xv[j] - mu[j];
+        if (j < 2) s2[j] = __builtin_fmaf(out[j], dx, s2[j]);
+        else s2[j] = mul_then_add(out[j], dx, s2[j]);
+      }
+    } else {
+#pragma unroll
+      for (int j = 0; j < 4; ++j) out[j] = 0.f;
+    }
+    return in;
+  };
+  auto park_pair = [&](bf16_t* Gt, bf16_t* Yt, int trow, const float (&o0)[4], const float (&o1)[4], bool in0, bool in1,
+                       const u32x2& xa, const u32x2& xb) {
+    const int col = trow * 64 + 2 * p;
+#pragma unroll
+    for (int j = 0; j < 4; ++j) {
+      const unsigned int gw = (__float_as_uint(o0[j]) >> 16) | (__float_as_uint(o1[j]) & 0xffff0000u);
+      const unsigned int a = in0 ? xa[j >> 1] : 0u, b = in1 ? xb[j >> 1] : 0u;
+      const unsigned int yw = (j & 1) ? ((a >> 16) | (b & 0xffff0000u)) : ((a & 0xffffu) | (b << 16));
+      *reinterpret_cast<unsigned int*>(Gt + (c0 + j) * TROW + col) = gw;
+      *reinterpret_cast<unsigned int*>(Yt + (c0 + j) * TROW + col) = yw;
+    }
+  };
+  auto park_taps = [&](bf16_t* Xt, int b_of_pixel) {
+    if constexpr (FAST) {
+      int shf;
+      (void)tss_stem::window_base(t_ox, t.Wi, &shf, 3);
+#pragma unroll
+      for (int i = 0; i < NTAP; ++i) {
+        const int ch = win_ch(i), ky = win_ky(i);
+        const int iy = 2 * t_oy + ky - 1;
+        float v[3];
+        tss_stem::window_taps(__uint_as_float(traw[i][0]), __uint_as_float(traw[i][1]), __uint_as_float(traw[i][2]), 0.f, shf, t_ox,
+                              t.Wi, t_in && ch < t.Cin && iy >= 0 && iy < t.Hi, v);
+        if (half * NTAP + i < 9) {
+#pragma unroll
+          for (int kx = 0; kx < 3; ++kx) Xt[((half * NTAP + i) * 3 + kx) * TROW + gp] = (bf16_t)v[kx];
+        }
+      }
+    } else if (half == 0) {
+      float v[27];
+      tss_stem::stem_taps<TX>(reinterpret_cast<const TX*>(t.img), (long)b_of_pixel, t_oy, t_ox, t_in, t.Cin, t.Hi, t.Wi, 2, plane, v);
+#pragma unroll
+      for (int i = 0; i < 27; ++i) Xt[i * TROW + gp] = (bf16_t)v[i];
+    }
+  };
+  auto contract = [&](const bf16_t* T) {
+#pragma unroll
+    for (int ks = 0; ks < 2; ++ks) {
+      const int col = mkh * 64 + ks * 32 + fq * 8;
+      bf16x8 sf[2], xf[2];
+#pragma unroll
+      for (int i = 0; i < 2; ++i) {
+        sf[i] = *reinterpret_cast<const bf16x8*>(T + msrc * TILE_ELEMS + (i * 16 + fr) * TROW + col);
+        xf[i] = *reinterpret_cast<const bf16x8*>(T + 2 * TILE_ELEMS + (i * 16 + fr) * TROW + col);
+      }
+#pragma unroll
+      for (int i = 0; i < 2; ++i)
+#pragma unroll
+        for (int j = 0; j < 2; ++j) acc[i][j] = __builtin_amdgcn_mfma_f32_16x16x32_bf16(sf[i], xf[j], acc[i][j], 0, 0, 0);
+      if (ks == msrc) {
+#pragma unroll
+        for (int j = 0; j < 2; ++j) accP[j] = __builtin_amdgcn_mfma_f32_16x16x32_bf16(ones, xf[j], accP[j], 0, 0, 0);
+      }
+    }
+  };
+
+  int slot = 0, t_b = 0;
+  bool have_tile = false;
+  while (cc.b < g.B) {
+#pragma unroll
+    for (int k = 0; k < SPF; ++k) {
+      if (cc.b >= g.B) break;
+      if constexpr (FAST) arrived15<10>(raw[k], traw);
+      else arrived10<10>(raw[k]);
+      const int o = cc.o0 + cc.it;
+      const bool vo = o < Ho;
+      const int r0 = 2 * o - 1, r1 = 2 * o;
+      const bool v0 = r0 >= 0 && r0 < g.H, v1 = r1 < g.H;
+      const int ix = 2 * (cc.x0 + p);
+      const bool first = cc.it == 0, last = cc.it == g.RS;
+      float gown[4], a00[4], a01[4], a10[4], a11[4];
+      g_of(raw[k][0], raw[k][1], vo && cc.x0 + p < Wo, gown);
+      a_of(raw[k][4], v0 && ix < g.W, a00);
+      a_of(raw[k][5], v0 && ix + 1 < g.W, a01);
+      a_of(raw[k][7], v1 && ix < g.W, a10);
+      a_of(raw[k][8], v1 && ix + 1 < g.W, a11);
+      float4* Gs = rows_s[slot];
+      float4* A0 = rows_s[2 + 2 * slot];
+      float4* A1 = rows_s[3 + 2 * slot];
+      put4(Gs, tid, gown); put4(A0, tid + g.CVS, a01); put4(A1, tid + g.CVS, a11);
+      if (halo_r) {
+        float gh[4];
+        g_of(raw[k][2], raw[k][3], vo && cc.x0 + g.PXL < Wo, gh);
+        put4(Gs, tid + g.CVS, gh);
+      }
+      if (halo_l) {
+        float ah[4];
+        a_of(raw[k][6], v0 && ix - 1 >= 0, ah);
+        put4(A0, tid, ah);
+        a_of(raw[k][9], v1 && ix - 1 >= 0, ah);
+        put4(A1, tid, ah);
+      }
+      const u32x2 x00 = keep2(raw[k][4]), x01 = keep2(raw[k][5]), x10 = keep2(raw[k][7]), x11 = keep2(raw[k][8]);
+      settle(gown); settle(a00); settle(a01); settle(a10); settle(a11);
+      if (have_tile) park_taps(tiles + ((slot ^ 1) * 3 + 2) * TILE_ELEMS, t_b);
+      asm volatile("" ::: "memory");
+      issue_taps(cc);
+      t_b = cc.b;
+      issue(ci, raw[k]);
+      advance(ci, g, n_iter);
+      __syncthreads();
+      if (have_tile) contract(tiles + (slot ^ 1) * 3 * TILE_ELEMS);
+      bf16_t* Gt = tiles + slot * 3 * TILE_ELEMS;
+      bf16_t* Yt = Gt + TILE_ELEMS;
+      {
+        float gr[4], al0[4], al1[4];
+        get4(Gs, tid + g.CVS, gr);
+        get4(A0, tid, al0);
+        get4(A1, tid, al1);
+        float e0[4], e1[4], o0[4], o1[4];
+        {
+          float w0[4], w1[4], w2[4], w6[4], w7[4], w8[4];
+          const_of(0, w0); const_of(1, w1); const_of(2, w2); const_of(6, w6); const_of(7, w7); const_of(8, w8);
+#pragma unroll
+          for (int j = 0; j < 4; ++j) {
+            e0[j] = w7[j] * gprev[j]; e0[j] += w1[j] * gown[j];
+            e1[j] = w8[j] * gprev[j]; e1[j] += w6[j] * gprev_r[j]; e1[j] += w2[j] * gown[j]; e1[j] += w0[j] * gr[j];
+          }
+        }
+        {
+          const bool in0 = emit(!first, r0, ix, x00, e0, o0);
+          const bool in1 = emit(!first, r0, ix + 1, x01, e1, o1);
+          park_pair(Gt, Yt, 0, o0, o1, in0, in1, x00, x01);
+        }
+        {
+          float w3[4], w4[4], w5[4];
+          const_of(3, w3); const_of(4, w4); const_of(5, w5);
+#pragma unroll
+          for (int j = 0; j < 4; ++j) {
+            e0[j] = w4[j] * gown[j];
+            e1[j] = w5[j] * gown[j]; e1[j] += w3[j] * gr[j];
+          }
+        }
+        {
+          const bool in0 = emit(!last, r1, ix, x10, e0, o0);
+          const bool in1 = emit(!last, r1, ix + 1, x11, e1, o1);
+          park_pair(Gt, Yt, 1, o0, o1, in0, in1, x10, x11);
+        }
+#pragma unroll
+        for (int j = 0; j < 4; ++j) {
+          const float gc = last ? 0.f : gown[j], gp_ = first ? 0.f : gprev[j];
+          dwa[0][j] = __builtin_fmaf(gc, al0[j], dwa[0][j]); dwa[1][j] = __builtin_fmaf(gc, a00[j], dwa[1][j]);
+          dwa[2][j] = __builtin_fmaf(gc, a01[j], dwa[2][j]);
+          dwa[3][j] = __builtin_fmaf(gc, al1[j], dwa[3][j]); dwa[4][j] = __builtin_fmaf(gc, a10[j], dwa[4][j]);
+          dwa[5][j] = __builtin_fmaf(gc, a11[j], dwa[5][j]);
+          dwa[6][j] = __builtin_fmaf(gp_, al0[j], dwa[6][j]); dwa[7][j] = __builtin_fmaf(gp_, a00[j], dwa[7][j]);
+          dwa[8][j] = __builtin_fmaf(gp_, a01[j], dwa[8][j]);
+          gprev[j] = gown[j]; gprev_r[j] = gr[j];
+        }
+      }
+      have_tile = true;
+      advance(cc, g, n_iter);
+      slot ^= 1;
+    }
+  }
+#pragma unroll
+  for (int k = 0; k < SPF; ++k) {
+    if constexpr (FAST) arrived15<0>(raw[k], traw);
+    else arrived10<0>(raw[k]);
+  }
+  if (have_tile) park_taps(tiles + ((slot ^ 1) * 3 + 2) * TILE_ELEMS, t_b);
+  __syncthreads();
+  if (have_tile) contract(tiles + (slot ^ 1) * 3 * TILE_ELEMS);
+
+  float* red = reinterpret_cast<float*>(&rows_s[0][0]);
+  flush_slab<4>(s1, s2, g.stats, g.C, g.CVS, g.PXL, 0, brow, g.rows_used, p, cg, true, red);
+  float* wrow = g.ws + (long)brow * g.C * 9;
+  const int cw = g.CVS * 4;
+#pragma unroll
+  for (int t0 = 0; t0 < 9; t0 += 3) {
+    __syncthreads();
+#pragma unroll
+    for (int tt = 0; tt < 3; ++tt)
+      *reinterpret_cast<float4*>(red + tid * 12 + tt * 4) = make_float4(dwa[t0 + tt][0], dwa[t0 + tt][1], dwa[t0 + tt][2], dwa[t0 + tt][3]);
+    __syncthreads();
+    for (int i = tid; i < cw * 3; i += NT) {
+      const int c = i / 3, tt = i - c * 3;
+      const int cgc = c >> 2, j = c & 3;
+      if (c < g.C) {
+        float sum = 0.f;
+        for (int q = 0; q < g.PXL; ++q) sum += red[(q * g.CVS + cgc) * 12 + tt * 4 + j];
+        wrow[(long)c * 9 + t0 + tt] = sum;
+      }
+    }
+  }
+  float* tred = reinterpret_cast<float*>(tiles);
+#pragma unroll
+  for (int i = 0; i < 2; ++i)
+#pragma unroll
+    for (int j = 0; j < 2; ++j)
+#pragma unroll
+      for (int r = 0; r < 4; ++r) tred[(wave * 32 + i * 16 + fq * 4 + r) * 32 + j * 16 + fr] = acc[i][j][r];
+  if (fq == 0) {
+    tred[4 * 32 * 32 + wave * 32 + fr] = accP[0][0];
+    tred[4 * 32 * 32 + wave * 32 + 16 + fr] = accP[1][0];
+  }
+  __syncthreads();
+  float* trow = t.rows + (long)brow * ROWF;
+  for (int i = tid; i < ROWF; i += NT) {
+    float s;
+    if (i < 2 * N * KP) {
+      const int which = i / (N * KP), r = i - which * N * KP;
+      const int n = r / KP, kk = r - n * KP;
+      const float* q = tred + (which * 32 + n) * 32 + kk;
+      s = q[0] + q[2 * 32 * 32];
+    } else {
+      const float* q = tred + 4 * 32 * 32 + (i - 2 * N * KP);
+      s = q[0] + q[32] + q[64] + q[96];
+    }
+    trow[i] = s;
+  }
+}
+
+struct FinishArgs { tss_bn_bwd_job job; const float* rows; int nrows; const float* mean; float* dw; int K; };
+
+__global__ __launch_bounds__(tss_fin::FIN_NT) void stem_tail_finish_kernel(const FinishArgs a) {
+  constexpr int CH = tss_fin::FIN_CH;
+  constexpr int NV = 2 * CH * KP / 4 + KP / 4;
+  constexpr int U = 16;
+  static_assert(NV <= tss_fin::FIN_NT / 2 && CH * KP <= tss_fin::FIN_NT, "two row groups of NV lanes; one lane per (n, j)");
+  __shared__ double part[2][NV * 4];
+  const int blk = (int)blockIdx.x, tid = threadIdx.x;
+  tss_fin::bn_bwd_finalize_block(a.job, blk);
+  const int col = tid & 127, rg = tid >> 7;
+  if (col < NV) {
+    const int off = col < CH * KP / 4 ? blk * CH * KP + 4 * col
+                  : (col < 2 * CH * KP / 4 ? N * KP + blk * CH * KP + 4 * (col - CH * KP / 4) : 2 * N * KP + 4 * (col - 2 * CH * KP / 4));
+    const float* src = a.rows + off;
+    double s0 = 0.0, s1 = 0.0, s2 = 0.0, s3 = 0.0;
+    for (int r0 = rg; r0 < a.nrows; r0 += 2 * U) {
+      float4 v[U];
+#pragma unroll
+      for (int u = 0; u < U; ++u) {
+        const int r = r0 + 2 * u;
+        v[u] = r < a.nrows ? *reinterpret_cast<const float4*>(src + (long)r * ROWF) : make_float4(0.f, 0.f, 0.f, 0.f);
+      }
+#pragma unroll
+      for (int u = 0; u < U; ++u) { s0 += (double)v[u].x; s1 += (double)v[u].y; s2 += (double)v[u].z; s3 += (double)v[u].w; }
+    }
+    part[rg][4 * col + 0] = s0; part[rg][4 * col + 1] = s1; part[rg][4 * col + 2] = s2; part[rg][4 * col + 3] = s3;
+  }
+  __threadfence_block();
+  __syncthreads();
+  if (tid < CH * KP) {
+    const int nl = tid / KP, j = tid - nl * KP;
+    const int n = blk * CH + nl;
+    if (n < a.job.C && j < a.K) {
+      const double A = part[0][tid] + part[1][tid];
+      const double Y = part[0][CH * KP + tid] + part[1][CH * KP + tid];
+      const double P = part[0][2 * CH * KP + j] + part[1][2 * CH * KP + j];
+      const volatile float* ga = a.job.ga; const volatile float* gb = a.job.gb; const volatile float* gce = a.job.gce;
+      const double v = (double)ga[n] * (A - (double)gce[n] * P) + (double)gb[n] * (Y - (double)a.mean[n] * P);
+      a.dw[n * a.K + j] += (float)v;
+    }
+  }
+}
+
+}
+
+extern "C" {
+
+int tss_stem_tail_supported(int C, int Cin, int Hi, int Wi, int dtype) {
+  const char* sw = getenv("TSS_STEM_TAIL");
+  const bool on = sw && atoi(sw) != 0;
+  return on && dtype == TSS_BF16 && C == N && Cin >= 1 && Cin <= 3 && Hi >= 1 && Wi >= 1 &&
+         (long)Cin * Hi * Wi * 4 < (1l << 31) && tss::dwroll_bwd_fused_supported(C, 2, 1, dtype);
+}
+
+int tss_stem_tail_row_floats(void) { return ROWF; }
+
+int tss_stem_tail_bwd_sweep(const void* e, long lde, const void* yraw, long ldyr,
+                            const float* ga, const float* gb, const float* gce, const float* gmu, const float* w,
+                            const void* x, long ldx, const float* in_mean, const float* in_scale, const float* in_bias, int in_relu,
+                            const void* image, int image_f32, int Cin, int Hi, int Wi,
+                            double* bstats, float* ws, float* tail_rows,
+                            int B, int C, int dtype, int grid_cap, void* stream, int* rows_out) {
+  TSS_REQUIRE(tss_stem_tail_supported(C, Cin, Hi, Wi, dtype), TSS_ERR_SHAPE);
+  TSS_REQUIRE(e && yraw && ga && gb && gce && gmu && w && x && in_mean && in_scale && in_bias && image && bstats && ws && tail_rows &&
+              rows_out && B >= 1 && grid_cap >= 0, TSS_ERR_SHAPE);
+  TSS_REQUIRE((lde % 8) == 0 && lde >= C && (ldyr % 8) == 0 && ldyr >= C && (ldx % 8) == 0 && ldx >= C, TSS_ERR_SHAPE);
+  TSS_REQUIRE(tss::aligned16(e) && tss::aligned16(yraw) && tss::aligned16(x) && tss::aligned16(tail_rows), TSS_ERR_ALIGN);
+  RollBwdArgs g = {};
+  g.e = (const bf16_t*)e; g.lde = lde; g.yr = (const bf16_t*)yraw; g.ldyr = ldyr; g.ga = ga; g.gb = gb; g.gce = gce; g.gmu = gmu;
+  g.w = w; g.x = (const bf16_t*)x; g.ldx = ldx; g.xm = in_mean; g.xs = in_scale; g.xb = in_bias; g.x_relu = in_relu;
+  g.x_mask = 1; g.stats = bstats; g.ws = ws;
+  g.B = B; g.H = (Hi - 1) / 2 + 1; g.W = (Wi - 1) / 2 + 1; g.C = C;
+  const int Ho = (g.H - 1) / 2 + 1, Wo = (g.W - 1) / 2 + 1;
+  TSS_REQUIRE((long)g.W * ldx < (1l << 30) && (long)Wo * (lde > ldyr ? lde : ldyr) < (1l << 30), TSS_ERR_SHAPE);
+  plan_bwd(g, 2, Ho, Wo, 1, grid_cap);
+  TailArgs t = {};
+  t.img = image; t.Cin = Cin; t.Hi = Hi; t.Wi = Wi; t.rows = tail_rows;
+  const long Ps = (long)B * g.H * g.W, Po = (long)B * Ho * Wo;
+  const hipStream_t st = (hipStream_t)stream;
+  static tss::DevOnce once;
+  if (once.first()) {
+    (void)hipFuncSetAttribute(reinterpret_cast<const void*>(stem_tail_sweep_kernel<true, float>), hipFuncAttributeMaxDynamicSharedMemorySize, SMEM_BYTES);
+    (void)hipFuncSetAttribute(reinterpret_cast<const void*>(stem_tail_sweep_kernel<false, float>), hipFuncAttributeMaxDynamicSharedMemorySize, SMEM_BYTES);
+    (void)hipFuncSetAttribute(reinterpret_cast<const void*>(stem_tail_sweep_kernel<false, bf16_t>), hipFuncAttributeMaxDynamicSharedMemorySize, SMEM_BYTES);
+  }
+  {
+    tss::ProfScope prof(TSS_K_STEM_TAIL_BWD_SWEEP, st,
+                        (double)Po * 2 * C * 2 + (double)Ps * C * 2 + (double)B * Cin * Hi * Wi * (image_f32 ? 4 : 2),
+                        36.0 * Po * C + 4.0 * Ps * C * Cin * 9);
+    if (image_f32 && Wi >= 4) hipLaunchKernelGGL((stem_tail_sweep_kernel<true, float>), dim3(g.rows_used), dim3(NT), SMEM_BYTES, st, g, t, Ho, Wo);
+    else if (image_f32) hipLaunchKernelGGL((stem_tail_sweep_kernel<false, float>), dim3(g.rows_used), dim3(NT), SMEM_BYTES, st, g, t, Ho, Wo);
+    else hipLaunchKernelGGL((stem_tail_sweep_kernel<false, bf16_t>), dim3(g.rows_used), dim3(NT), SMEM_BYTES, st, g, t, Ho, Wo);
+  }
+  *rows_out = g.rows_used;
+  return tss::check_last("stem_tail_bwd_sweep");
+}
+
+int tss_stem_tail_bwd_finish(const double* bstats, double count, const float* invstd, const float* gamma, int accumulate,
+                             float* dgamma, float* dbeta, float* ga, float* gb, float* gce, const float* mean,
+                             const float* tail_rows, int rows, float* dw, int Cin, int C, void* stream) {
+  TSS_REQUIRE(C == N && Cin >= 1 && Cin <= 3 && rows >= 1 && rows <= TSS_STAT_SLABS, TSS_ERR_SHAPE);
+  TSS_REQUIRE(bstats && invstd && ga && gb && gce && mean && tail_rows && dw, TSS_ERR_SHAPE);
+  TSS_REQUIRE(tss::aligned16(tail_rows), TSS_ERR_ALIGN);
+  FinishArgs a = {};
+  a.job.bstats = bstats; a.job.count = count; a.job.invstd = invstd; a.job.gamma = gamma; a.job.training = 1;
+  a.job.accumulate = accumulate; a.job.dgamma = dgamma; a.job.dbeta = dbeta; a.job.ga = ga; a.job.gb = gb; a.job.gce = gce; a.job.C = C;
+  a.rows = tail_rows; a.nrows = rows; a.mean = mean; a.dw = dw; a.K = Cin * 9;
+  tss::ProfScope prof(TSS_K_STEM_TAIL_BWD_FINISH, (hipStream_t)stream, (double)rows * ROWF * 4 + (double)TSS_STAT_SLABS * 2 * C * 8, 0.0);
+  hipLaunchKernelGGL(stem_tail_finish_kernel, dim3(tss_fin::fin_blocks(C)), dim3(tss_fin::FIN_NT), 0, (hipStream_t)stream, a);
+  return tss::check_last("stem_tail_bwd_finish");
+}
+
+}
diff --git a/torch_semantic_segmentation_amd/csrc/stemtaps.h b/torch_semantic_segmentation_amd/csrc/stemtaps.h
--- /dev/null
+++ b/torch_semantic_segmentation_amd/csrc/stemtaps.h
@@ -0,0 +1,59 @@
+#pragma once
+#include "common.h"
+
+namespace tss_stem {
+
+struct __attribute__((packed, aligned(4))) F4u { float x, y, z, w; };
+__device__ __forceinline__ int window_base(int ox, int Win, int* shift, int width = 4) {
+  const int ix0 = 2 * ox - 1;
+  const int base = ix0 < 0 ? 0 : (ix0 > Win - width ? Win - width : ix0);
+  *shift = ix0 - base;
+  return base;
+}
+__device__ __forceinline__ void window_taps(float fx, float fy, float fz, float fw, int shift, int ox, int Win, bool row_ok,
+                                            float* v3) {
+  const int ix0 = 2 * ox - 1;
+#pragma unroll
+  for (int kx = 0; kx < 3; ++kx) {
+    const int idx = kx + shift;
+    const float t = idx <= 0 ? fx : (idx == 1 ? fy : (idx == 2 ? fz : fw));
+    v3[kx] = (row_ok && idx >= 0 && ix0 + kx < Win) ? t : 0.f;
+  }
+}
+
+template <typename TX>
+__device__ __forceinline__ void stem_taps(const TX* x, long b, int oy, int ox, bool in, int Cin, int Hin, int Win,
+                                          int stride, long plane, float v[27]) {
+  if (sizeof(TX) == 4 && stride == 2 && Win >= 4) {
+    int sh;
+    const int base = window_base(ox, Win, &sh);
+#pragma unroll
+    for (int c = 0; c < 3; ++c)
+#pragma unroll
+      for (int ky = 0; ky < 3; ++ky) {
+        const int iy = 2 * oy + ky - 1;
+        const bool vy = in && c < Cin && iy >= 0 && iy < Hin;
+        const float* row = reinterpret_cast<const float*>(x) + (b * Cin + (c < Cin ? c : 0)) * plane + (long)(vy ? iy : 0) * Win + base;
+        const F4u f = *reinterpret_cast<const F4u*>(row);
+        window_taps(f.x, f.y, f.z, f.w, sh, ox, Win, vy, v + c * 9 + ky * 3);
+      }
+    return;
+  }
+#pragma unroll
+  for (int c = 0; c < 3; ++c)
+#pragma unroll
+    for (int ky = 0; ky < 3; ++ky) {
+      const int iy = oy * stride + ky - 1;
+      const bool vy = iy >= 0 && iy < Hin;
+#pragma unroll
+      for (int kx = 0; kx < 3; ++kx) {
+        const int ix = ox * stride + kx - 1;
+        const bool ok = in && c < Cin && vy && ix >= 0 && ix < Win;
+        const long off = (b * Cin + (c < Cin ? c : 0)) * plane + (vy ? iy : 0) * (long)Win + (ix < 0 ? 0 : (ix >= Win ? Win - 1 : ix));
+        const float t = (float)x[off];
+        v[c * 9 + ky * 3 + kx] = ok ? t : 0.f;
+      }
+    }
+}
+
+}
diff --git a/torch_semantic_segmentation_amd/ops.py b/torch_semantic_segmentation_amd/ops.py
--- a/torch_semantic_segmentation_amd/ops.py
+++ b/torch_semantic_segmentation_amd/ops.py
@@ -566,7 +566,7 @@
 
 class BNLink:
     __slots__ = ('C', 'count', 'training', 'gamma', 'beta', 'vec', 'scale', 'mean', 'invstd',
-                 'ga', 'gb', 'gce', 'stats', 'bstats', 'consumed', 'sync')
+                 'ga', 'gb', 'gce', 'stats', 'bstats', 'consumed', 'sync', 'stem', 'tail')
 
     def __init__(self, C, count, training, gamma, beta, device, slabs=True):
         self.C, self.count, self.training, self.gamma, self.beta = C, count, training, gamma, beta
@@ -579,6 +579,8 @@
             self.stats = self.bstats = None
         self.consumed = False
         self.sync = None
+        self.stem = None
+        self.tail = None
 
 
 class Deferred:
@@ -1288,9 +1290,61 @@
 
 
 
+def _stem_tail_ok(c):
+    cfg, il = c.cfg, c.il
+    if il is None or il.stem is None or c.y is None or N.fast_paths_disabled():
+        return False
+    image, cin, _, stem_stride, stem_weight = il.stem
+    return bool(c.s == 2 and c.d == 1 and c.Cout == 32 and c.dt == N.TSS_BF16 and stem_stride == 2
+                and il.training and il.sync is None and il.beta is not None and cfg.in_relu
+                and cfg.res_fork is None and cfg.stash_fork is None and c.need_dx and c.side is None
+                and not getattr(c.x, '_backward_hooks', None) and not c.x.retains_grad
+                and not _param_observed(c.p_weight) and not _param_observed(stem_weight)
+                and N.lib().tss_stem_tail_supported(c.Cout, cin, image.shape[2], image.shape[3], c.dt))
+
+
+def _bwd_dw_stem_tail(c, ws):
+    il = c.il
+    image, cin, image_f32 = il.stem[:3]
+    rows = ctypes.c_int(0)
+    trows = torch.empty((N.stat_slabs(), N.lib().tss_stem_tail_row_floats()), dtype=torch.float32, device=c.dev)
+    call('tss_stem_tail_bwd_sweep', *c.gargs, ptr(c.weight), *c.xargs, ptr(image), int(image_f32), cin, image.shape[2], image.shape[3],
+         c.bst, ptr(ws), ptr(trows), c.B, c.Cout, c.dt, 0, c.st, ctypes.byref(rows))
+    _add_rows(ws, c.dw, c.Cout * 9, rows.value, c.p_weight, c.dw_ret)
+    e_in = torch.empty(1, dtype=c.e.dtype, device=c.dev).expand(c.B, c.Cin, c.Hin, c.Win)
+    il.tail = (e_in, trows, rows.value)
+    return e_in
+
+
+def _bwd_stem_tail_finish(ctx, cfg, tail):
+    x, weight, y, _ = ctx.saved_tensors
+    link, (_, trows, rows) = cfg.out_link, tail
+    if ctx.needs_input_grad[0]:
+        raise NotImplementedError('HIP path: gradient with respect to the input image is not implemented')
+    p_weight, p_gamma, p_beta, _ = cfg.params
+    Cout = cfg.cout
+    dgamma = dbeta = None
+    acc = 0
+    if ctx.has_affine:
+        dgamma, dbeta = _direct_target(p_gamma), _direct_target(p_beta)
+        if dgamma is not None and dbeta is not None:
+            acc = 1
+        else:
+            dgb = torch.empty((2, Cout), dtype=torch.float32, device=x.device)
+            dgamma, dbeta = dgb[0], dgb[1]
+    dw, dw_ret = _grad_target(p_weight, weight)
+    call('tss_stem_tail_bwd_finish', ptr(link.bstats), float(link.count), ptr(link.invstd), ptr(link.gamma), acc, ptr(dgamma), ptr(dbeta),
+         ptr(link.ga), ptr(link.gb), ptr(link.gce), ptr(link.mean), ptr(trows), rows, ptr(dw), cfg.cin, Cout, stream())
+    if acc:
+        dgamma = dbeta = None
+    return None, dw_ret, dgamma, dbeta, None, None
+
+
 def _bwd_dw(c):
     weight, B, Hin, Win, Cout, s, d, dt, st = c.weight, c.B, c.Hin, c.Win, c.Cout, c.s, c.d, c.dt, c.st
     ws = c.tmp((N.stat_slabs(), Cout * 9))
+    if _stem_tail_ok(c):
+        return _bwd_dw_stem_tail(c, ws), _NO_EXTRAS
     defer = 1 if (c.need_dx and c.side is None) else 0
     fused = bool(defer and ((fuse_dw_backward and N.lib().tss_dwconv3x3_bwd_fused_supported(Cout, s, d, dt))
                             or N.lib().tss_dwconv3x3_bwd_fused_preferred(Cout, s, d, dt)))
@@ -1469,6 +1523,8 @@
         mask = _FWD[cfg.kind](_FwdArgs(cfg, x, weight, bias, y, _aff(cfg.in_link), stats, B, Hin, Win, Cout, P, s, d, dt, dev, st))
         if link is not None:
             _finalize_forward(link, cfg.bn, cfg.training, P, Cout, gamma, st)
+            if cfg.kind == 'stem':
+                link.stem = (x, cfg.cin, bool(cfg.image_f32), s, cfg.params[0])
         cfg.out_link = link
         ctx.cfg = cfg
         ctx.save_for_backward(x, weight, y if link is not None else None, mask)
@@ -1479,6 +1535,11 @@
     @staticmethod
     def backward(ctx, e):
         cfg = ctx.cfg
+        if cfg.kind == 'stem' and cfg.out_link is not None and cfg.out_link.tail is not None:
+            tail, cfg.out_link.tail = cfg.out_link.tail, None
+            if e.data_ptr() != tail[0].data_ptr():
+                raise RuntimeError('HIP path: the stem received a gradient other than the one its consumer left for it')
+            return _bwd_stem_tail_finish(ctx, cfg, tail)
         c = _Bwd()
         c.cfg, c.temps = cfg, []
         x, weight, y, drop_mask = ctx.saved_tensors
```

Result: no change. 1731 images/sec, median of 2 (-0.0%).
